# kiva12138/MIMRL

Hardware: AMD Instinct MI355X
Metric: two-stage train iters/sec (higher is better)
Workload: dtype bf16

## Files before the change

### include/mimrl.h

```cpp
#ifndef MIMRL_H_
#define MIMRL_H_

#include <stdint.h>

#ifdef __cplusplus
extern "C" {
#endif

#define MIMRL_ABI_VERSION 6
#define MIMRL_MAX_BLOCKS 4
#define MIMRL_MAX_BATCH 2048
#define MIMRL_MAX_BATCH_CONCAT 1024
#define MIMRL_MAX_CLASSES 8

enum { MIMRL_OK = 0, MIMRL_ERR_ARG = -1, MIMRL_ERR_HIP = -2, MIMRL_ERR_STATE = -3, MIMRL_ERR_NODEVICE = -4 };
enum { MIMRL_GROUP_MAIN = 0, MIMRL_GROUP_CRITIC = 1 };
enum { MIMRL_CRITIC_SEPARATE = 0, MIMRL_CRITIC_CONCAT = 1 };
enum { MIMRL_BOUND_INFONCE = 0, MIMRL_BOUND_NWJ, MIMRL_BOUND_TUBA, MIMRL_BOUND_DV, MIMRL_BOUND_JS_FGAN,
       MIMRL_BOUND_JS, MIMRL_BOUND_SMILE, MIMRL_BOUND_MINE, MIMRL_BOUND_INTERPOLATE };
enum { MIMRL_ACT_NONE = 0, MIMRL_ACT_RELU = 1, MIMRL_ACT_GELU = 2, MIMRL_ACT_TANH = 3 };
enum { MIMRL_PREC_FP32 = 0, MIMRL_PREC_BF16_GEMM_FWD = 1, MIMRL_PREC_BF16_GEMM_BWD = 2, MIMRL_PREC_BF16_GRU_FWD = 4,
       MIMRL_PREC_BF16_GRU_BWD = 8, MIMRL_PREC_BF16 = 15 };

enum { MIMRL_BASELINE_CONSTANT = 0, MIMRL_BASELINE_GAUSSAIN = 1, MIMRL_BASELINE_UNNORMALIZED = 2 };
// ... 115 lines not shown
int mimrl_op_gemm_wgrad_group(void* stream, int n, const float* const* A, const float* const* B, float* const* C, const int32_t* dims,
                              const int64_t* strides, int precision);
int64_t mimrl_op_gru_saved_floats(int B, int T);
int mimrl_op_gru_forward(void* stream, const float* gx_f, const float* gx_r, const float* whh_f, const float* whh_r,
                         const float* bhh_f, const float* bhh_r, const int32_t* lens, float* out, float* saved_f,
                         float* saved_r, int B, int T, int precision);
int mimrl_op_gru_backward(void* stream, const float* whh_f, const float* whh_r, const float* saved_f,
                          const float* saved_r, const int32_t* lens, const float* out, const float* dout, float* dg_f,
                          float* dg_r, float* hprev_f, float* hprev_r, int B, int T, int precision);
int mimrl_op_recur_btv(int B, int nmod);
int mimrl_op_lstm_forward(void* stream, const float* gx_f, const float* gx_r, const float* whh_f, const float* whh_r,
                          const float* bhh_f, const float* bhh_r, const int32_t* lens, float* out, float* saved_f,
                          float* saved_r, int B, int T, int kernel);
int mimrl_op_lstm_backward(void* stream, const float* whh_f, const float* whh_r, const float* saved_f,
                           const float* saved_r, const int32_t* lens, const float* out, const float* dout, float* dg_f,
                           float* dg_r, float* hprev_f, float* hprev_r, int B, int T, int kernel);
int mimrl_op_concat_dw(void* stream, const void* dz2, const void* a1, float* dw2, const void* dz1, const void* a0, float* dw1, int E, int64_t rows,
                       int64_t dw_stride, const float* ds, const void* a2h, float* dw3, const uint32_t* m2, const float* w3, const float* P,
                       const float* Q, int B);
int mimrl_op_gru_wgrad(void* stream, const void* const* dg, const void* const* x, const void* const* hp, float* const* dw_ih,
                       float* const* dw_hh, int64_t rows, int kp);
int mimrl_op_mi_bound(void* stream, const float* scores, float* dscores, float* mi, const float* gscale, int E, int B,
                      int bound);
int mimrl_op_mi_bound_ex(void* stream, const float* scores, float* dscores, float* mi, float* mi_loss, const float* gscale,
                         int E, int B, int bound, uint32_t lossform);
#define MIMRL_NCE_WS_FLOATS 2064
int mimrl_op_mi_infonce_rows(void* stream, const float* scores, float* dscores, float* mi, float* mi_loss, const float* gscale,
                             int E, int B, float* ws);
int mimrl_op_mi_bound_baseline(void* stream, float* scores, float* dscores, float* mi, const float* gscale, const float* lb,
                               float* dlb, int E, int B, int bound);
int mimrl_op_mi_sep_infonce(void* stream, const float* tout, float* dtout, float* mi, float* mi_loss, const float* gscale, int E,
                            int B, int tiled);
int mimrl_op_knn(void* stream, const float* Z, int dz, int N, const int32_t* anchors, int m, int k, int32_t* idx_out);
int mimrl_op_sample_anchors(void* stream, int32_t* anchors_out, int ncall, int m, int N, uint64_t seed, const int32_t* step,
                            uint32_t stream_id, int step_add);
int mimrl_knn_r1_host(const float* z, int N, const int32_t* anchors, int m, int k, int32_t* idx_out);
int mimrl_set_knn_override_mask(mimrl_handle* h, int stage, unsigned call_mask);
int mimrl_op_cmi_loss(void* stream, const float* logits, float* dlogits, float* bce, float* cmi, const float* g_bce,
                      const float* g_cmi, int E, int n, int hardtanh);
int mimrl_op_task_loss(void* stream, int kind, const float* pred, const float* y, float* dpred, float* loss, int B);
int mimrl_op_class_loss(void* stream, int kind, const float* logits, const float* y, float* dlogits, float* loss, int B, int C);
int mimrl_op_mlp_stack_forward(void* stream, int nb, int rows, int brows, int nl, const int32_t* dims, const float* const* W,
                               const float* const* b, int64_t pstride, const float* in, float* const* act, float* out);
int mimrl_op_mlp_stack_backward(void* stream, int nb, int rows, int brows, int nl, const int32_t* dims, const float* const* W,
                                int64_t pstride, const float* const* act, const float* dout, float* const* dz, float* din,
                                float* const* db);
int mimrl_probe_cube(mimrl_handle* h, const float* x, float* out, const float* dout, float* dx);
int mimrl_probe_encoders(mimrl_handle* h, float* cube_x, const float* dcube, const float* dmean);
int mimrl_probe_mi(mimrl_handle* h, int stage, float* mi, float* scores, float* dtin_out);
int mimrl_probe_cmi(mimrl_handle* h, int stage, const float* cmi_in, float* logits, float* vals, float* dcin_out);
int mimrl_probe_knn(mimrl_handle* h, int stage, int32_t* idx_out);
int mimrl_op_adam(void* stream, float* p, float* g, float* m, float* v, int64_t n, const float* lr, const int32_t* step,
                  float beta1, float beta2, float eps, float weight_decay, float clip);

#ifdef __cplusplus
}
#endif
#endif
```

### mimrl_amd/_lib.py

```python
from __future__ import annotations

import ctypes as C
import os
from typing import List, Tuple

_HERE = os.path.dirname(os.path.abspath(__file__))
DETERMINISTIC = os.environ.get("MIMRL_DETERMINISTIC", "0") not in ("", "0")
LIB_PATH = os.environ.get("MIMRL_LIB_PATH") or os.path.join(_HERE, "libmimrl_hip_det.so" if DETERMINISTIC else "libmimrl_hip.so")
MAX_BLOCKS = 4
MAX_BATCH = 2048
MAX_BATCH_CONCAT = 1024
NCE_WS_FLOATS = 2064
NSCALARS = 64
MAX_CLASSES = 8
PHASES = ["gemm_misc", "gru_fwd", "gru_bwd", "cube_fwd", "cube_bwd", "est_fwd", "est_bwd", "opt", "model_misc"]
S1_LOSS, S1_MIS, S1_LOSSES, S2_LOSS, S2_TASK, S2_MIS, S2_LOSSES = 0, 1, 12, 32, 33, 34, 42

BOUNDS = {"infonce": 0, "nwj": 1, "tuba": 2, "dv": 3, "js_fgan": 4, "js": 5, "smile": 6, "mine": 7, "interpolate": 8}
ACTS = {"none": 0, "relu": 1, "gelu": 2, "tanh": 3}
PREC = {"fp32": 0, "bf16": 15, "bf16_gemm_fwd": 1, "bf16_gemm_bwd": 2, "bf16_gemm": 3, "bf16_gru": 12, "bf16_nogemmbwd": 13}


class MimrlError(RuntimeError):
    pass
# ... 29 lines not shown
        "main_p", "main_g", "main_m", "main_v", "crit_p", "crit_g", "crit_m", "crit_v",
        "text", "audio", "video", "labels", "bank_c", "bank_f", "bank_t", "bank_a", "bank_v",
        "anchors", "lr_main", "lr_critic", "pred", "feats", "scalars", "knn_override", "counters")]


_lib = None


def load() -> C.CDLL:
    global _lib
    if _lib is not None:
        return _lib
    if not os.path.exists(LIB_PATH):
        raise MimrlError(f"{LIB_PATH} is missing: build it with `python -c 'import __graft_entry__ as g; g.build()'` "
                         f"or `make -C mimrl_amd/csrc` (hipcc --offload-arch=gfx950). There is no CPU fallback.")
    try:
        import torch
    except ImportError:
        pass
    lib = C.CDLL(LIB_PATH)
    if os.environ.get("MIMRL_LIB_PATH"):
        class _Partial:
            def __init__(self, lib):
                object.__setattr__(self, "_lib", lib)

            def __getattr__(self, name):
                try:
                    return getattr(self._lib, name)
                except AttributeError:
                    return type("_Missing", (), {})()
        real, lib = lib, _Partial(lib)
    lib.mimrl_last_error.restype = C.c_char_p
    lib.mimrl_bucket_floats.restype = C.c_int64
    lib.mimrl_workspace_bytes.restype = C.c_int64
    lib.mimrl_op_gru_saved_floats.restype = C.c_int64
    lib.mimrl_destroy.restype = None
    lib.mimrl_op_gemm.argtypes = [_FP, _FP, _FP, _FP, C.c_int, C.c_int, C.c_int, C.c_int, C.POINTER(C.c_int64), _FP, _FP,
                                  C.c_float, C.c_float, C.c_int, C.c_int]
    lib.mimrl_op_gemm_ex.argtypes = [_FP, _FP, _FP, _FP, C.c_int, C.c_int, C.c_int, C.c_int, C.POINTER(C.c_int64), _FP, _FP, C.c_int,
                                     C.POINTER(C.c_int64), C.c_int, C.c_int, _FP, _FP, _FP, C.c_int, C.c_int]
    lib.mimrl_comm_unique_id.argtypes = [_FP]
    lib.mimrl_set_comm.argtypes = [_FP, _FP, C.c_int, C.c_int]
    lib.mimrl_set_comm_critic_bf16.argtypes = [_FP, C.c_int]
    lib.mimrl_set_task_loss.argtypes = [_FP, C.c_int]
    lib.mimrl_op_task_loss.argtypes = [_FP, C.c_int, _FP, _FP, _FP, _FP, C.c_int]
    lib.mimrl_set_class_loss.argtypes = [_FP, C.c_int]
    lib.mimrl_op_class_loss.argtypes = [_FP, C.c_int, _FP, _FP, _FP, _FP, C.c_int, C.c_int]
    lib.mimrl_main_late_offset.argtypes = [_FP]
    lib.mimrl_main_late_offset.restype = C.c_int64
    lib.mimrl_op_gemm16.argtypes = [_FP, _FP, _FP, _FP, C.c_int, C.c_int, C.c_int, C.c_int, C.POINTER(C.c_int64), _FP, _FP, C.c_int,
                                    C.POINTER(C.c_int64), C.c_int, C.POINTER(C.c_int64), _FP, C.c_int]
    lib.mimrl_op_gemm_wgrad_group.argtypes = [_FP, C.c_int, C.POINTER(C.c_void_p), C.POINTER(C.c_void_p), C.POINTER(C.c_void_p),
                                              C.POINTER(C.c_int32), C.POINTER(C.c_int64), C.c_int]
    lib.mimrl_op_adam.argtypes = [_FP, _FP, _FP, _FP, _FP, C.c_int64, _FP, _FP, C.c_float, C.c_float, C.c_float,
                                  C.c_float, C.c_float]
    lib.mimrl_op_gru_forward.argtypes = [_FP] * 11 + [C.c_int, C.c_int, C.c_int]
    lib.mimrl_op_gru_backward.argtypes = [_FP] * 12 + [C.c_int, C.c_int, C.c_int]
    lib.mimrl_op_lstm_forward.argtypes = [_FP] * 11 + [C.c_int, C.c_int, C.c_int]
    lib.mimrl_op_lstm_backward.argtypes = [_FP] * 12 + [C.c_int, C.c_int, C.c_int]
    lib.mimrl_op_recur_btv.argtypes = [C.c_int, C.c_int]
    lib.mimrl_op_concat_dw.argtypes = [C.c_void_p] * 7 + [C.c_int, C.c_int64, C.c_int64] + [C.c_void_p] * 7 + [C.c_int]
    lib.mimrl_op_gru_wgrad.argtypes = [C.c_void_p] + [C.POINTER(C.c_void_p)] * 5 + [C.c_int64, C.c_int]
    lib.mimrl_op_mi_bound.argtypes = [_FP] * 5 + [C.c_int, C.c_int, C.c_int]
    lib.mimrl_op_mi_bound_ex.argtypes = [_FP] * 6 + [C.c_int, C.c_int, C.c_int, C.c_uint32]
    lib.mimrl_op_mi_infonce_rows.argtypes = [_FP] * 6 + [C.c_int, C.c_int, _FP]
    lib.mimrl_op_mi_sep_infonce.argtypes = [_FP] * 6 + [C.c_int, C.c_int, C.c_int]
    lib.mimrl_op_mi_bound_baseline.argtypes = [_FP] * 7 + [C.c_int, C.c_int, C.c_int]
    lib.mimrl_op_knn.argtypes = [_FP, _FP, C.c_int, C.c_int, _FP, C.c_int, C.c_int, _FP]
    lib.mimrl_op_cmi_loss.argtypes = [_FP] * 7 + [C.c_int, C.c_int, C.c_int]
    lib.mimrl_op_sample_anchors.argtypes = [_FP, _FP, C.c_int, C.c_int, C.c_int, C.c_uint64, _FP, C.c_uint32, C.c_int]
    lib.mimrl_create.argtypes = [C.POINTER(Cfg), _FP, C.POINTER(_FP)]
    lib.mimrl_bind.argtypes = [_FP, C.POINTER(Buffers)]
    lib.mimrl_profile_read.argtypes = [_FP, C.POINTER(C.c_float), C.POINTER(C.c_int32)]
    lib.mimrl_profile_read_gemm.argtypes = [_FP, C.POINTER(C.c_double)]
    for fn in ("mimrl_set_bank_rows", "mimrl_stage_grads", "mimrl_stage_grads_part", "mimrl_stage_apply", "mimrl_estimate", "mimrl_profile_enable", "mimrl_set_stage2_prefetch"):
        getattr(lib, fn).argtypes = [_FP, C.c_int]
    lib.mimrl_set_grad_scale.argtypes = [_FP, C.c_float]
    lib.mimrl_stage_grads_part.argtypes = [_FP, C.c_int, C.c_int]
    lib.mimrl_set_inputs.argtypes = [_FP, C.c_int, _FP, _FP, _FP, _FP]
    lib.mimrl_knn_r1_host.argtypes = [_FP, C.c_int, _FP, C.c_int, C.c_int, _FP]
    lib.mimrl_set_knn_override_mask.argtypes = [_FP, C.c_int, C.c_uint]
    for fn in ("mimrl_stage1_step", "mimrl_stage2_step", "mimrl_two_stage_step", "mimrl_destroy", "mimrl_workspace_bytes", "mimrl_params_changed",
               "mimrl_stage2_forward_tail"):
        getattr(lib, fn).argtypes = [_FP]
    lib.mimrl_forward.argtypes = [_FP, C.c_int, C.c_int]
    lib.mimrl_set_kernel_stamps.argtypes = [_FP, _FP, C.c_int]
    lib.mimrl_probe_cube.argtypes = [_FP] * 5
    lib.mimrl_probe_mi.argtypes = [_FP, C.c_int, _FP, _FP, _FP]
    lib.mimrl_probe_cmi.argtypes = [_FP, C.c_int, _FP, _FP, _FP, _FP]
    lib.mimrl_probe_knn.argtypes = [_FP, C.c_int, _FP]
    lib.mimrl_probe_encoders.argtypes = [_FP] * 4
    lib.mimrl_layout_count.argtypes = [C.POINTER(Cfg)]
    lib.mimrl_layout_entry_dim2.argtypes = [C.POINTER(Cfg), C.c_int]
    lib.mimrl_bucket_floats.argtypes = [C.POINTER(Cfg), C.c_int]
    lib.mimrl_layout_entry.argtypes = [C.POINTER(Cfg), C.c_int, C.c_char_p, C.c_int, C.POINTER(C.c_int),
                                       C.POINTER(C.c_int64), C.POINTER(C.c_int), C.POINTER(C.c_int), C.POINTER(C.c_int)]
    if os.environ.get("MIMRL_LIB_PATH"):
        lib = real
    _lib = lib
    return lib


ENCODERS = {"gru": 0, "conv": 1, "lstm": 2}
BASELINES = {"constant": 0, "gaussain": 1, "unnormalized": 2}

EXPORTS = [
    "mimrl_last_error", "mimrl_abi_version", "mimrl_deterministic", "mimrl_device_check", "mimrl_layout_count", "mimrl_layout_entry", "mimrl_layout_entry_dim2",
    "mimrl_bucket_floats", "mimrl_create", "mimrl_bind", "mimrl_set_bank_rows", "mimrl_set_inputs", "mimrl_stage1_step", "mimrl_stage2_step", "mimrl_two_stage_step",
    "mimrl_stage_grads", "mimrl_stage_grads_part", "mimrl_stage_apply", "mimrl_forward", "mimrl_estimate", "mimrl_profile_enable", "mimrl_profile_read", "mimrl_profile_read_gemm",
    "mimrl_workspace_bytes", "mimrl_params_changed", "mimrl_set_stage2_prefetch", "mimrl_stage2_forward_tail", "mimrl_set_grad_scale", "mimrl_destroy", "mimrl_op_gemm", "mimrl_op_gemm_ex", "mimrl_op_gemm16", "mimrl_op_gemm_wgrad_group",
    "mimrl_op_gru_saved_floats", "mimrl_op_gru_forward", "mimrl_op_gru_backward", "mimrl_op_gru_wgrad", "mimrl_op_concat_dw", "mimrl_op_mi_bound", "mimrl_op_mi_bound_ex", "mimrl_op_mi_bound_baseline", "mimrl_op_mi_sep_infonce", "mimrl_op_knn",
    "mimrl_op_cmi_loss", "mimrl_op_sample_anchors", "mimrl_knn_r1_host", "mimrl_set_knn_override_mask", "mimrl_op_mlp_stack_forward", "mimrl_op_mlp_stack_backward", "mimrl_op_adam",
    "mimrl_probe_cube", "mimrl_probe_mi", "mimrl_probe_cmi", "mimrl_probe_knn", "mimrl_probe_encoders", "mimrl_set_kernel_stamps", "mimrl_comm_unique_id", "mimrl_set_comm", "mimrl_main_late_offset", "mimrl_set_comm_critic_bf16",
    "mimrl_stage1_pipe_prime", "mimrl_stage1_pipe", "mimrl_set_task_loss", "mimrl_op_task_loss", "mimrl_set_class_loss", "mimrl_op_class_loss",
    "mimrl_op_mi_infonce_rows", "mimrl_op_lstm_forward", "mimrl_op_lstm_backward", "mimrl_op_recur_btv",
]

TASK_LOSSES = {"MAE": 0, "MSE": 1, "RMSE": 2, "SIMSE": 3, "CCC": 4}
BATCH_COUPLED_LOSSES = ("RMSE", "SIMSE", "CCC")
CLASS_LOSSES = {"CE": 5, "Focal": 6, "BCE": 7}


def task_loss_code(opt, world: int = 1) -> int:
    loss = getattr(opt, "loss", "MAE")
    task = getattr(opt, "task", "regression")
    ncls = int(getattr(opt, "num_class", 1))
    if loss in CLASS_LOSSES:
        if task != "classification":
            raise NotImplementedError(f"--loss {loss} is a classification loss: it needs --task classification (and --num_class)")
        if loss == "BCE" and ncls not in (1, 2):
            raise NotImplementedError(f"--loss BCE needs --num_class 1 or 2, got {ncls} (Solver.py:327-337)")
        if loss != "BCE" and not 2 <= ncls <= MAX_CLASSES:
            raise NotImplementedError(f"--loss {loss} needs 2 <= --num_class <= {MAX_CLASSES}, got {ncls}")
        if int(world) > 1 and loss == "Focal":
            raise NotImplementedError(f"--loss {loss} couples the whole batch: with {int(world)} ranks each would see only its shard, not the "
                                      f"reference's global batch; run it on one rank, or use CE / BCE")
        return CLASS_LOSSES[loss]
    if loss not in TASK_LOSSES:
        raise NotImplementedError(f"--loss {loss}: unknown task loss (choose one of {', '.join(list(TASK_LOSSES) + list(CLASS_LOSSES))})")
    if task == "classification" or ncls > 1:
        raise NotImplementedError(f"--loss {loss} is a regression loss: --task classification / --num_class {ncls} need one of "
                                  f"{', '.join(CLASS_LOSSES)}")
    if int(world) > 1 and loss in BATCH_COUPLED_LOSSES:
        raise NotImplementedError(f"--loss {loss} couples the whole batch: with {int(world)} ranks each would see only its shard, not the "
                                  f"reference's global batch; run it on one rank, or use MAE / MSE")
    return TASK_LOSSES[loss]


def check(rc: int) -> int:
    if rc < 0:
        raise MimrlError(f"libmimrl_hip error {rc}: {load().mimrl_last_error().decode()}")
    return rc


def make_cfg(opt, d_t: int, d_a: int, d_v: int, seq_len: int = None, bank_capacity: int = 0, precision: str = "fp32",
             use_graph: bool = False, seed: int = 0, device_anchors: bool = False, batch: int = None) -> Cfg:
    c = Cfg()
    c.batch = int(batch if batch is not None else opt.batch_size)
    c.time_len = int(opt.time_len)
    c.seq_len = int(seq_len if seq_len is not None else opt.time_len)
    c.d_t, c.d_a, c.d_v, c.d_common = int(d_t), int(d_a), int(d_v), int(opt.d_common)
    enc = getattr(opt, "encoders", "gru")
    if enc not in ENCODERS:
        raise MimrlError(f"--encoders {enc}: choose gru, conv or lstm (Model.py:237)")
    c.encoder = ENCODERS[enc]
    nb = len(opt.d_hiddens)
    if nb > MAX_BLOCKS or len(opt.d_outs) != nb or len(opt.res_project) != nb:
        raise MimrlError("d_hiddens / d_outs / res_project must have the same length (<= 4)")
# ... 78 lines not shown
```

### mimrl_amd/csrc/cube_bwd_fused.h

```cpp
#pragma once
#include "common.h"
#include "model_ops.h"

namespace mimrl {

struct LAxisBwdArgs {
  const float *dz, *y, *mean, *rstd, *gamma;
  const float* u;
  const float *w2, *w1, *wr;
  float *dy, *du, *dx;
  float *db2, *db1;
  int B, il, hl, ol, C, act;
};
bool laxis_bwd_supported(int il, int hl, int ol, int C);
int laxis_bwd_fused(hipStream_t s, const LAxisBwdArgs& a);

struct DAxisBwdArgs {
  const float *dz, *y, *mean, *rstd, *gamma;
  const float* u;
  const __bf16 *w2t, *w1t, *wrt;
  float *dy, *du, *dx;
  long R;
  int act;
  float *dgamma, *dbeta, *db2, *db1;
};
bool daxis_bwd_supported(int id, int hd, int od);
int daxis_bwd_fused(hipStream_t s, const DAxisBwdArgs& a);

struct WtTransposeArgs { const float* src[12]; __bf16* dst[12]; int n; };
int wt_transpose_bf16(hipStream_t s, const WtTransposeArgs& a);

int daxis_param_grads(hipStream_t s, const float* y, const float* mean, const float* rstd, const float* dz, const float* dy,
                      const float* du, float* dgamma, float* dbeta, float* db2, float* db1, long R);

#ifdef MIMRL_PHASE_PROBE
int cube_bwd_read_phases(long long* out);
#endif

}
```

### mimrl_amd/csrc/cube_bwd_fused.hip

```cpp
#include "cube_bwd_fused.h"
#include "kmix_device.h"

namespace mimrl {

namespace {

#ifdef MIMRL_PHASE_PROBE
__device__ long long g_cbwd_phase[64];
#define BPHASE(base, i) do { if (blockIdx.x == 0 && blockIdx.y == 0 && threadIdx.x == 0) g_cbwd_phase[(base) + (i)] = (long long)wall_clock64(); } while (0)
#else
#define BPHASE(base, i) do { } while (0)
#endif

constexpr int CT = 128;
constexpr int KP = 64 + 8;


template <bool LONG = false>
__global__ __launch_bounds__(256, LONG ? 2 : 1) void laxis_bwd_kernel(LAxisBwdArgs a) {
  __shared__ __attribute__((aligned(16))) __bf16 sdyu[2][CT][KP];
  auto& sdy = sdyu[0];
  auto& sdu = sdyu[1];
  __shared__ __attribute__((aligned(16))) __bf16 wts[3][64][KP];
  float (*red)[2][CT] = reinterpret_cast<float (*)[2][CT]>(&sdu[0][0]);
  __shared__ float acc_l[3][64];
  __shared__ LdsAcc acc_h[64];
  __shared__ float sgam[64];
  const int tid = threadIdx.x, lane = tid & 63, wave = tid >> 6, lr = lane & 31, lh = lane >> 5;
  const int b = blockIdx.y, c0 = blockIdx.x * CT;
  const int il = a.il, hl = a.hl, ol = a.ol, C = a.C;
  const int pb = ol > 32 ? 16 : 0;
  BPHASE(pb, 0);

  float uu[2][16];
  {
    const int ccu = c0 + wave * 32 + lr;
#pragma unroll
    for (int mt = 0; mt < 2; ++mt)
#pragma unroll
      for (int r = 0; r < 16; ++r) {
        const int h = min(mt * 32 + (r & 3) + 8 * (r >> 2) + 4 * lh, hl - 1);
        uu[mt][r] = a.u[((long)b * hl + h) * C + ccu];
      }
  }
  {
    uint4* z = reinterpret_cast<uint4*>(&wts[0][0][0]);
    for (int i = tid; i < 3 * 64 * KP * 2 / 16; i += 256) z[i] = make_uint4(0u, 0u, 0u, 0u);
    if (tid < 64) { acc_l[0][tid] = 0.f; acc_l[1][tid] = 0.f; acc_l[2][tid] = 0.f; acc_h[tid].zero(); sgam[tid] = a.gamma[tid < ol ? tid : ol - 1]; }
  }
  __syncthreads();
  BPHASE(pb, 1);
  {
    const int n2 = ol * hl, n1 = hl * il, nr = ol * il;
    float wv[3][16];
#pragma unroll
    for (int j = 0; j < 16; ++j) {
      const int idx = tid + 256 * j;
      wv[0][j] = a.w2[idx < n2 ? idx : n2 - 1];
      if constexpr (!LONG) {
        wv[1][j] = a.w1[idx < n1 ? idx : n1 - 1];
        wv[2][j] = a.wr[idx < nr ? idx : nr - 1];
      }
    }
#pragma unroll
    for (int j = 0; j < 16; ++j) {
      const int idx = tid + 256 * j;
      if (idx < n2) { const int o = idx / hl, h = idx - o * hl; wts[0][h][o] = to_bf16(wv[0][j]); }
      if constexpr (!LONG) {
        if (idx < n1) { const int h = idx / il, i = idx - h * il; wts[1][i][h] = to_bf16(wv[1][j]); }
        if (idx < nr) { const int o = idx / il, i = idx - o * il; wts[2][i][o] = to_bf16(wv[2][j]); }
      }
    }
  }

  BPHASE(pb, 2);
  const int col = tid & (CT - 1), half = tid >> 7;
  const long cidx = (long)b * C + c0 + col;
  const float mu = a.mean[cidx], rs = a.rstd[cidx];
  const float* __restrict__ dzb = a.dz + (long)b * ol * C + c0 + col;
  const float* __restrict__ yb = a.y + (long)b * ol * C + c0 + col;
  float* __restrict__ dyb = a.dy + (long)b * ol * C + c0 + col;
  float gq[32], xq[32];
#pragma unroll
  for (int j = 0; j < 32; ++j) {
    const int l = min(half + 2 * j, ol - 1);
    gq[j] = dzb[(long)l * C]; xq[j] = yb[(long)l * C];
  }
  float s1 = 0.f, s2 = 0.f;
#pragma unroll
  for (int j = 0; j < 32; ++j) {
    const int l = half + 2 * j;
    xq[j] = (xq[j] - mu) * rs;
    gq[j] = l < ol ? gq[j] * sgam[min(l, 63)] : 0.f;
    s1 += gq[j]; s2 += gq[j] * xq[j];
  }
  BPHASE(pb, 3);
  red[0][half][col] = s1;
  red[1][half][col] = s2;
  __syncthreads();
  s1 = (red[0][0][col] + red[0][1][col]) / ol;
  s2 = (red[1][0][col] + red[1][1][col]) / ol;
#pragma unroll
  for (int j = 0; j < 32; ++j) {
    const int l = half + 2 * j;
    if (l < ol) {
      const float v = rs * (gq[j] - s1 - xq[j] * s2);
      dyb[(long)l * C] = v;
      sdy[col][l] = to_bf16(v);
    }
  }
  for (int l = ol + ((half ^ ol) & 1); l < 64; l += 2) sdy[col][l] = to_bf16(0.f);
  __syncthreads();

  if (a.db2 && tid >= 192 && tid - 192 < ol) {
    float t = 0.f;
    for (int c = 0; c < CT; ++c) t += (float)sdy[(c + tid) & (CT - 1)][tid - 192];
    acc_l[2][tid - 192] = t;
  }
  BPHASE(pb, 4);
  const int nt = wave;
  const int cc = c0 + nt * 32 + lr;
  {
    f32x16 acc0, acc1;
#pragma unroll
    for (int r = 0; r < 16; ++r) { acc0[r] = 0.f; acc1[r] = 0.f; }
#pragma unroll
    for (int ks = 0; ks < 4; ++ks) {
      const bf16x8 bf = *reinterpret_cast<const bf16x8*>(&sdy[nt * 32 + lr][ks * 16 + 8 * lh]);
      const bf16x8 a0 = *reinterpret_cast<const bf16x8*>(&wts[0][lr][ks * 16 + 8 * lh]);
      acc0 = __builtin_amdgcn_mfma_f32_32x32x16_bf16(a0, bf, acc0, 0, 0, 0);
      const bf16x8 a1 = *reinterpret_cast<const bf16x8*>(&wts[0][32 + lr][ks * 16 + 8 * lh]);
      acc1 = __builtin_amdgcn_mfma_f32_32x32x16_bf16(a1, bf, acc1, 0, 0, 0);
    }
    act_dispatch(a.act, [&](auto AT) __attribute__((always_inline)) {
#pragma unroll
    for (int mt = 0; mt < 2; ++mt)
#pragma unroll
      for (int r = 0; r < 16; ++r) {
        const int h = mt * 32 + (r & 3) + 8 * (r >> 2) + 4 * lh;
        float v = 0.f;
        if (h < hl) {
          const long ui = ((long)b * hl + h) * C + cc;
          v = (mt == 0 ? acc0[r] : acc1[r]) * act_grad_c<decltype(AT)::value>(a.act, uu[mt][r]);
          a.du[ui] = v;
        }
        sdu[nt * 32 + lr][h] = to_bf16(v);
        if (a.db1) {
          const float t = half_sum_hi(v);
          if (lr == 16 && h < hl) acc_h[h].add(t);
        }
      }
    });
  }
  __syncthreads();
  BPHASE(pb, 5);
  if constexpr (LONG) {
    float w1v[16], wrv[16];
    auto wreq = [&](int i0) __attribute__((always_inline)) {
      const int i = min(i0 + (tid & 63), il - 1);
#pragma unroll
      for (int j = 0; j < 16; ++j) {
        const int r = 16 * (tid >> 6) + j;
        w1v[j] = a.w1[(long)min(r, hl - 1) * il + i];
        wrv[j] = a.wr[(long)min(r, ol - 1) * il + i];
      }
    };
    wreq(0);
    for (int i0 = 0; i0 < il; i0 += 64) {
      __syncthreads();
      {
        const int ii = tid & 63, r0 = 16 * (tid >> 6);
        const bool iok = i0 + ii < il;
        bf16x8 p1[2], p2[2];
#pragma unroll
        for (int j = 0; j < 16; ++j) {
          p1[j >> 3][j & 7] = to_bf16(iok && r0 + j < hl ? w1v[j] : 0.f);
          p2[j >> 3][j & 7] = to_bf16(iok && r0 + j < ol ? wrv[j] : 0.f);
        }
        *reinterpret_cast<bf16x8*>(&wts[1][ii][r0]) = p1[0]; *reinterpret_cast<bf16x8*>(&wts[1][ii][r0 + 8]) = p1[1];
        *reinterpret_cast<bf16x8*>(&wts[2][ii][r0]) = p2[0]; *reinterpret_cast<bf16x8*>(&wts[2][ii][r0 + 8]) = p2[1];
      }
      __syncthreads();
      wreq(i0 + 64 < il ? i0 + 64 : i0);
      f32x16 acc0, acc1;
#pragma unroll
      for (int r = 0; r < 16; ++r) { acc0[r] = 0.f; acc1[r] = 0.f; }
#pragma unroll
      for (int ks = 0; ks < 8; ++ks) {
        const bool first = ks < 4;
        const int kk = (first ? ks : ks - 4) * 16 + 8 * lh;
        const bf16x8 bf = *reinterpret_cast<const bf16x8*>(first ? &sdu[nt * 32 + lr][kk] : &sdy[nt * 32 + lr][kk]);
        const bf16x8 a0 = *reinterpret_cast<const bf16x8*>(&wts[first ? 1 : 2][lr][kk]);
        acc0 = __builtin_amdgcn_mfma_f32_32x32x16_bf16(a0, bf, acc0, 0, 0, 0);
        const bf16x8 a1 = *reinterpret_cast<const bf16x8*>(&wts[first ? 1 : 2][32 + lr][kk]);
        acc1 = __builtin_amdgcn_mfma_f32_32x32x16_bf16(a1, bf, acc1, 0, 0, 0);
      }
      {
#pragma unroll
        for (int mt = 0; mt < 2; ++mt)
#pragma unroll
          for (int r = 0; r < 16; ++r) {
            const int i = i0 + mt * 32 + (r & 3) + 8 * (r >> 2) + 4 * lh;
            if (i < il) a.dx[((long)b * il + i) * C + cc] = mt == 0 ? acc0[r] : acc1[r];
          }
      }
    }
  } else {
    f32x16 acc0, acc1;
#pragma unroll
    for (int r = 0; r < 16; ++r) { acc0[r] = 0.f; acc1[r] = 0.f; }
#pragma unroll
    for (int ks = 0; ks < 8; ++ks) {
      const bool first = ks < 4;
      const int kk = (first ? ks : ks - 4) * 16 + 8 * lh;
      const bf16x8 bf = *reinterpret_cast<const bf16x8*>(first ? &sdu[nt * 32 + lr][kk] : &sdy[nt * 32 + lr][kk]);
      const bf16x8 a0 = *reinterpret_cast<const bf16x8*>(&wts[first ? 1 : 2][lr][kk]);
      acc0 = __builtin_amdgcn_mfma_f32_32x32x16_bf16(a0, bf, acc0, 0, 0, 0);
      const bf16x8 a1 = *reinterpret_cast<const bf16x8*>(&wts[first ? 1 : 2][32 + lr][kk]);
      acc1 = __builtin_amdgcn_mfma_f32_32x32x16_bf16(a1, bf, acc1, 0, 0, 0);
    }
    {
#pragma unroll
      for (int mt = 0; mt < 2; ++mt)
#pragma unroll
        for (int r = 0; r < 16; ++r) {
          const int i = mt * 32 + (r & 3) + 8 * (r >> 2) + 4 * lh;
          if (i < il) a.dx[((long)b * il + i) * C + cc] = mt == 0 ? acc0[r] : acc1[r];
        }
    }
  }
  __syncthreads();
  BPHASE(pb, 6);
  if (a.db2 && tid < ol) acc_add(&a.db2[tid], acc_l[2][tid]);
  if (a.db1 && tid >= 64 && tid - 64 < hl) acc_add(&a.db1[tid - 64], acc_h[tid - 64].get());
  BPHASE(pb, 7);
}

}

#ifdef MIMRL_PHASE_PROBE
int cube_bwd_read_phases(long long* out) { return hipMemcpyFromSymbol(out, HIP_SYMBOL(g_cbwd_phase), sizeof(long long) * 64) == hipSuccess ? 0 : 1; }
#endif

bool laxis_bwd_supported(int il, int hl, int ol, int C) {
  return il >= 1 && hl >= 1 && ol >= 1 && hl <= 64 && ol <= 64 && C % CT == 0;
}

int laxis_bwd_fused(hipStream_t s, const LAxisBwdArgs& a) {
  if (!laxis_bwd_supported(a.il, a.hl, a.ol, a.C)) return set_error(MIMRL_ERR_ARG, "laxis_bwd_fused: unsupported shape");
  if (!a.wr) return set_error(MIMRL_ERR_ARG, "laxis_bwd_fused: needs the residual projection");
  if (a.il > 64) hipLaunchKernelGGL(laxis_bwd_kernel<true>, dim3(a.C / CT, a.B), dim3(256), 0, s, a);
  else hipLaunchKernelGGL(laxis_bwd_kernel<false>, dim3(a.C / CT, a.B), dim3(256), 0, s, a);
  LAUNCH_CHECK();
  return MIMRL_OK;
}

namespace {

constexpr int DR = 32;
constexpr int DP = 128 + 8;

__global__ __launch_bounds__(256) void daxis_bwd_kernel(DAxisBwdArgs a) {
  __shared__ __attribute__((aligned(16))) __bf16 sdy[DR][DP];
  __shared__ __attribute__((aligned(16))) __bf16 sdu[DR][DP];
  __shared__ LdsAcc spg[3][128];
  const int tid = threadIdx.x, lane = tid & 63, wave = tid >> 6, lr = lane & 31, lh = lane >> 5;
  const long r0 = (long)blockIdx.x * DR;
  const bool pg = a.dgamma != nullptr;
  const int pb = gridDim.x <= 200 ? 32 : 48;
  BPHASE(pb, 0);
  if (pg) for (int i = tid; i < 3 * 128; i += 256) (&spg[0][0])[i].zero();
  const int row1 = tid >> 3, part1 = tid & 7;
  const long r1 = r0 + row1;
  const bool ok1 = r1 < a.R;
  const long rc1 = ok1 ? r1 : a.R - 1;
  const float mu1 = a.mean[rc1], rs1 = a.rstd[rc1];
  float4 gz4[4], yv4[4];
#pragma unroll
  for (int q = 0; q < 4; ++q) {
    gz4[q] = *reinterpret_cast<const float4*>(a.dz + rc1 * 128 + part1 * 16 + q * 4);
    yv4[q] = *reinterpret_cast<const float4*>(a.y + rc1 * 128 + part1 * 16 + q * 4);
  }
  const int n = wave * 32 + lr;
  bf16x8 bw2[8], bw1[8], bwr[8];
#pragma unroll
  for (int ks = 0; ks < 8; ++ks) {
    bw2[ks] = *reinterpret_cast<const bf16x8*>(a.w2t + n * 128 + ks * 16 + 8 * lh);
    bw1[ks] = *reinterpret_cast<const bf16x8*>(a.w1t + n * 128 + ks * 16 + 8 * lh);
    bwr[ks] = *reinterpret_cast<const bf16x8*>(a.wrt + n * 128 + ks * 16 + 8 * lh);
  }
  float uu[16];
#pragma unroll
  for (int r = 0; r < 16; ++r) {
    const long row = min(r0 + (r & 3) + 8 * (r >> 2) + 4 * lh, a.R - 1);
    uu[r] = a.u[row * 128 + n];
  }
  BPHASE(pb, 1);
  {
    const int row = row1, part = part1;
    const long r = r1;
    const bool ok = ok1;
    float g[16], xh[16], dyk[16];
    float s1 = 0.f, s2 = 0.f;
    const float mu = mu1, rs = rs1;
#pragma unroll
    for (int q = 0; q < 4; ++q) {
      const float4 gz = gz4[q];
      const float4 yv = yv4[q];
      const float gg[4] = {gz.x, gz.y, gz.z, gz.w}, yy[4] = {yv.x, yv.y, yv.z, yv.w};
#pragma unroll
      for (int j = 0; j < 4; ++j) {
        g[q * 4 + j] = gg[j];
        xh[q * 4 + j] = (yy[j] - mu) * rs;
        const float dxh = gg[j] * a.gamma[part * 16 + q * 4 + j];
        s1 += dxh; s2 += dxh * xh[q * 4 + j];
      }
    }
    s1 = group_sum<8>(s1); s2 = group_sum<8>(s2);
    s1 *= (1.f / 128.f); s2 *= (1.f / 128.f);
#pragma unroll
    for (int q = 0; q < 4; ++q) {
      float v[4];
#pragma unroll
      for (int j = 0; j < 4; ++j) {
        const int c = part * 16 + q * 4 + j;
        v[j] = rs * (g[q * 4 + j] * a.gamma[c] - s1 - xh[q * 4 + j] * s2);
      }
      if (ok) *reinterpret_cast<float4*>(a.dy + r * 128 + part * 16 + q * 4) = make_float4(v[0], v[1], v[2], v[3]);
      bf16x4 p; p[0] = to_bf16(v[0]); p[1] = to_bf16(v[1]); p[2] = to_bf16(v[2]); p[3] = to_bf16(v[3]);
      *reinterpret_cast<bf16x4*>(&sdy[row][part * 16 + q * 4]) = p;
      if (pg) {
#pragma unroll
        for (int j = 0; j < 4; ++j) { const float gz = ok ? g[q * 4 + j] : 0.f; xh[q * 4 + j] *= gz; g[q * 4 + j] = gz; v[j] = ok ? v[j] : 0.f; }
        dyk[q * 4 + 0] = v[0]; dyk[q * 4 + 1] = v[1]; dyk[q * 4 + 2] = v[2]; dyk[q * 4 + 3] = v[3];
      }
    }
    if (pg) {
      __syncthreads();
#pragma unroll
      for (int j = 0; j < 16; ++j) {
        float sa = xh[j], sb = g[j], sc = dyk[j];
#pragma unroll
        for (int o = 8; o < 64; o <<= 1) { sa += __shfl_xor(sa, o, 64); sb += __shfl_xor(sb, o, 64); sc += __shfl_xor(sc, o, 64); }
        if (lane < 8) { spg[0][part * 16 + j].add(sa); spg[1][part * 16 + j].add(sb); spg[2][part * 16 + j].add(sc); }
      }
    }
  }
  __syncthreads();
  BPHASE(pb, 2);
  {
    f32x16 acc;
#pragma unroll
    for (int r = 0; r < 16; ++r) acc[r] = 0.f;
#pragma unroll
    for (int ks = 0; ks < 8; ++ks) {
      const bf16x8 af = *reinterpret_cast<const bf16x8*>(&sdy[lr][ks * 16 + 8 * lh]);
      acc = __builtin_amdgcn_mfma_f32_32x32x16_bf16(af, bw2[ks], acc, 0, 0, 0);
    }
    float csum = 0.f;
    act_dispatch(a.act, [&](auto AT) __attribute__((always_inline)) {
#pragma unroll
    for (int r = 0; r < 16; ++r) {
      const int m = (r & 3) + 8 * (r >> 2) + 4 * lh;
      const long row = r0 + m;
      float v = 0.f;
      if (row < a.R) {
        v = acc[r] * act_grad_c<decltype(AT)::value>(a.act, uu[r]);
        a.du[row * 128 + n] = v;
      }
      sdu[m][n] = to_bf16(v);
      csum += v;
    }
    });
    if (pg) {
      csum += __shfl_xor(csum, 32, 64);
      if (lh == 0) acc_add(&a.db1[n], csum);
    }
  }
  __syncthreads();
  BPHASE(pb, 3);
  if (pg && tid < 128) {
    acc_add(&a.dgamma[tid], spg[0][tid].get());
    acc_add(&a.dbeta[tid], spg[1][tid].get());
    acc_add(&a.db2[tid], spg[2][tid].get());
  }
  {
    f32x16 acc;
#pragma unroll
    for (int r = 0; r < 16; ++r) acc[r] = 0.f;
#pragma unroll
    for (int ks = 0; ks < 8; ++ks) {
      const bf16x8 a1 = *reinterpret_cast<const bf16x8*>(&sdu[lr][ks * 16 + 8 * lh]);
      acc = __builtin_amdgcn_mfma_f32_32x32x16_bf16(a1, bw1[ks], acc, 0, 0, 0);
      const bf16x8 a2 = *reinterpret_cast<const bf16x8*>(&sdy[lr][ks * 16 + 8 * lh]);
      acc = __builtin_amdgcn_mfma_f32_32x32x16_bf16(a2, bwr[ks], acc, 0, 0, 0);
    }
#pragma unroll
    for (int r = 0; r < 16; ++r) {
      const long row = r0 + (r & 3) + 8 * (r >> 2) + 4 * lh;
      if (row < a.R) a.dx[row * 128 + n] = acc[r];
    }
  }
  BPHASE(pb, 4);
}

__global__ void wt_transpose_kernel(WtTransposeArgs a) {
  __shared__ float t[32][33];
  const float* __restrict__ src = a.src[blockIdx.z];
  __bf16* __restrict__ dst = a.dst[blockIdx.z];
  const int k0 = blockIdx.y * 32, n0 = blockIdx.x * 32, tx = threadIdx.x & 31, ty = threadIdx.x >> 5;
  for (int j = ty; j < 32; j += 8) t[j][tx] = src[(k0 + j) * 128 + n0 + tx];
  __syncthreads();
  for (int j = ty; j < 32; j += 8) dst[(n0 + j) * 128 + k0 + tx] = to_bf16(t[tx][j]);
}

__global__ __launch_bounds__(256) void daxis_param_grads_kernel(const float* __restrict__ y, const float* __restrict__ mean,
                                                                const float* __restrict__ rstd, const float* __restrict__ dz,
                                                                const float* __restrict__ dy, const float* __restrict__ du,
                                                                float* __restrict__ dgamma, float* __restrict__ dbeta,
                                                                float* __restrict__ db2, float* __restrict__ db1, long R) {
  __shared__ float4 red[4][8][32];
  const int cq = threadIdx.x & 31, rl = threadIdx.x >> 5;
  const long r0 = (long)blockIdx.x * 64;
  float4 a0 = make_float4(0.f, 0.f, 0.f, 0.f), a1 = a0, a2 = a0, a3 = a0;
#pragma unroll
  for (int i = 0; i < 8; ++i) {
    const long r = r0 + rl + 8 * i;
    const long rc = r < R ? r : R - 1;
    const float m = r < R ? 1.f : 0.f;
    const float mu = mean[rc], rs = rstd[rc] * m;
    const float4 g = *reinterpret_cast<const float4*>(dz + rc * 128 + cq * 4);
    const float4 yv = *reinterpret_cast<const float4*>(y + rc * 128 + cq * 4);
    const float4 v = *reinterpret_cast<const float4*>(dy + rc * 128 + cq * 4);
    const float4 u = *reinterpret_cast<const float4*>(du + rc * 128 + cq * 4);
    a0.x += g.x * (yv.x - mu) * rs; a0.y += g.y * (yv.y - mu) * rs; a0.z += g.z * (yv.z - mu) * rs; a0.w += g.w * (yv.w - mu) * rs;
    a1.x += g.x * m; a1.y += g.y * m; a1.z += g.z * m; a1.w += g.w * m;
    a2.x += v.x * m; a2.y += v.y * m; a2.z += v.z * m; a2.w += v.w * m;
    a3.x += u.x * m; a3.y += u.y * m; a3.z += u.z * m; a3.w += u.w * m;
  }
  red[0][rl][cq] = a0; red[1][rl][cq] = a1; red[2][rl][cq] = a2; red[3][rl][cq] = a3;
  __syncthreads();
#pragma unroll
  for (int h = 0; h < 2; ++h) {
    const int idx = threadIdx.x + 256 * h, q = idx >> 7, c = idx & 127;
    const float* base = reinterpret_cast<const float*>(&red[q][0][0]);
    float sum = 0.f;
#pragma unroll
    for (int j = 0; j < 8; ++j) sum += base[j * 128 + c];
    float* dst = q == 0 ? dgamma : (q == 1 ? dbeta : (q == 2 ? db2 : db1));
    if (dst) acc_add(&dst[c], sum);
  }
}

}

int daxis_param_grads(hipStream_t s, const float* y, const float* mean, const float* rstd, const float* dz, const float* dy,
                      const float* du, float* dgamma, float* dbeta, float* db2, float* db1, long R) {
  if (R <= 0) return MIMRL_OK;
  hipLaunchKernelGGL(daxis_param_grads_kernel, dim3((unsigned)((R + 63) / 64)), dim3(256), 0, s, y, mean, rstd, dz, dy, du, dgamma, dbeta,
                     db2, db1, R);
  LAUNCH_CHECK();
  return MIMRL_OK;
}

bool daxis_bwd_supported(int id, int hd, int od) { return id == 128 && hd == 128 && od == 128; }

int daxis_bwd_fused(hipStream_t s, const DAxisBwdArgs& a) {
  if (!a.w2t || !a.w1t || !a.wrt) return set_error(MIMRL_ERR_ARG, "daxis_bwd_fused: needs the transposed weight images");
  if ((a.dgamma || a.dbeta || a.db2 || a.db1) && !(a.dgamma && a.dbeta && a.db2 && a.db1))
    return set_error(MIMRL_ERR_ARG, "daxis_bwd_fused: the four parameter-gradient outputs come together");
  hipLaunchKernelGGL(daxis_bwd_kernel, dim3((unsigned)((a.R + DR - 1) / DR)), dim3(256), 0, s, a);
  LAUNCH_CHECK();
  return MIMRL_OK;
}

int wt_transpose_bf16(hipStream_t s, const WtTransposeArgs& a) {
  if (a.n < 1 || a.n > 12) return set_error(MIMRL_ERR_ARG, "wt_transpose_bf16: 1..12 matrices");
  hipLaunchKernelGGL(wt_transpose_kernel, dim3(4, 4, a.n), dim3(256), 0, s, a);
  LAUNCH_CHECK();
  return MIMRL_OK;
}

}
```

### mimrl_amd/csrc/cube_fused.h

```cpp
#pragma once
#include "common.h"
#include "model_ops.h"

namespace mimrl {

struct CubePre {
  const float* tx_raw;
  const float* h2[2];
  const float *gamma[2], *beta[2];
  float p[3];
  float* feats;
  float* cube; float *mean[2], *rstd[2];
  int T;
  RngKey key;
};
struct CubeHead { const float *w, *bias; float *ff, *pred; float scale; int C; };

struct CubeFusedArgs {
  const float* x;
  const float *l_w1, *l_b1, *l_w2, *l_b2, *l_wr, *l_g, *l_be;
  KMixW kw;
  const float *d_w1, *d_b1, *d_w2, *d_b2, *d_wr, *d_g, *d_be;
  float *l_u, *l_h, *l_y, *l_z, *l_mean, *l_rstd;
  float* k_z;
  float *d_u, *d_h, *d_y, *d_mean, *d_rstd;
  float* d_z;
  int B, il, hl, ol, K, act, save;
  int dbg_phase;
  int pre_on, head_on;
  CubePre pre; CubeHead head;
};

bool cube_fused_supported(int il, int hl, int ol, int ik, int hk, int ok, int id, int hd, int od, bool ln_first,
                          bool res_project, bool bias, const float* dropout_mlp);
int cube_block_fwd_fused(hipStream_t s, const CubeFusedArgs& a);

#ifdef MIMRL_PHASE_PROBE
int cube_fwd_read_phases(long long* out);
#endif

}
```

### mimrl_amd/csrc/cube_fused.hip

```cpp
#include "cube_fused.h"

#include "cube_bookends.h"

#include <type_traits>

namespace mimrl {

namespace {

constexpr int D = 128;
constexpr int ILD = 72;
constexpr int IMG = 64 * ILD;
constexpr int CTL = 68, CTD = 132;

typedef _Float16 bf;

#ifdef MIMRL_PHASE_PROBE
__device__ long long g_cube_phase[128];
#define CPHASE(i) do { if (blockIdx.x == 0 && threadIdx.x == 0) g_cube_phase[(SAVE ? 64 : 0) + (NMT - 1) * 16 + (i)] = (long long)wall_clock64(); } while (0)
#else
#define CPHASE(i) do { } while (0)
#endif

__device__ __forceinline__ void mma64(f32x16& acc, const bf* A, const bf* B, int wm, int wn, int lane) {
// ... 32 lines not shown
  *reinterpret_cast<f16x8*>(img + n * ILD + kc + 8) = hi;
}
__device__ __forceinline__ void stage_weight(bf* img, const float* __restrict__ W, int ld, int n0, int k0, int N, int K, int tid) {
  stage_weight_commit(img, stage_weight_request(W, ld, n0, k0, N, K, tid), n0, k0, N, K, tid);
}
struct WImg { float4 q0, q1, q2, q3; };
__device__ __forceinline__ WImg load_weight128(const float* __restrict__ W, int n0, int k0, int tid) {
  const int n = tid >> 2, kc = (tid & 3) * 16;
  const float4* src = reinterpret_cast<const float4*>(W + (long)(n0 + n) * D + k0 + kc);
  return WImg{src[0], src[1], src[2], src[3]};
}
__device__ __forceinline__ void commit_weight128(bf* img, const WImg& w, int tid) {
  const int n = tid >> 2, kc = (tid & 3) * 16;
  f16x8 lo, hi;
  lo[0] = to_f16(w.q0.x); lo[1] = to_f16(w.q0.y); lo[2] = to_f16(w.q0.z); lo[3] = to_f16(w.q0.w);
  lo[4] = to_f16(w.q1.x); lo[5] = to_f16(w.q1.y); lo[6] = to_f16(w.q1.z); lo[7] = to_f16(w.q1.w);
  hi[0] = to_f16(w.q2.x); hi[1] = to_f16(w.q2.y); hi[2] = to_f16(w.q2.z); hi[3] = to_f16(w.q2.w);
  hi[4] = to_f16(w.q3.x); hi[5] = to_f16(w.q3.y); hi[6] = to_f16(w.q3.z); hi[7] = to_f16(w.q3.w);
  *reinterpret_cast<f16x8*>(img + n * ILD + kc) = lo;
  *reinterpret_cast<f16x8*>(img + n * ILD + kc + 8) = hi;
}

struct Carve {
  int xm, aw, bx, bh, ctl, red, ksw, prm;
  int bw, ctd, dprm, az, ah;
  int total;
};
__host__ __device__ inline Carve carve(int K, int nmt, int G) {
  Carve c;
  const int C = K * D, XP = C + 8;
  const int xm_bytes = 64 * XP * 2;
  c.xm = 0;
  c.aw = xm_bytes;
  c.bx = c.aw + 3 * IMG * 2;
  c.bh = c.bx + G * IMG * 2;
  c.ctl = c.bh + G * IMG * 2;
  c.red = c.ctl + G * 64 * CTL * 4;
  c.ksw = c.red + G * 2 * 4 * 64 * 4;
  c.prm = c.ksw + 256 * 4;
  const int l_end = c.prm + 4 * 64 * 4;
  c.bw = 0;
  c.dprm = c.bw + 2 * G * IMG * 2;
  int after = c.dprm + 2 * D * 4;
  if (after < xm_bytes) after = xm_bytes;
  c.az = (after + 15) & ~15;
  c.ah = c.az + nmt * 2 * IMG * 2;
  const int ah_bytes = nmt * 2 * IMG * 2, ctd_bytes = 64 * CTD * 4;
  c.ctd = c.ah;
  const int d_end = c.ah + (ah_bytes > ctd_bytes ? ah_bytes : ctd_bytes);
  c.total = l_end > d_end ? l_end : d_end;
  return c;
}

template <bool SAVE, int NMT, int G, bool PRE, bool HEAD>
__device__ __forceinline__ void cube_fwd_fused_body(const CubeFusedArgs& a) {
  static_assert(!(PRE || HEAD) || G == 2, "PRE / HEAD: 8 waves (12 time-phase streams on 8 waves; head_fwd_kernel's 512-thread shape)");
  static_assert(!HEAD || NMT == 1, "HEAD: every row of the block output in the one LDS tile");
  extern __shared__ __attribute__((aligned(16))) char smem[];
  constexpr int NT = 256 * G;
  const int tid = threadIdx.x, grp = tid >> 8, t = tid & 255, lane = t & 63, wave = t >> 6, wm = wave >> 1, wn = wave & 1;
  const int b = blockIdx.x;
  const int K = a.K, C = K * D, XP = C + 8, il = a.il, hl = a.hl, ol = a.ol;
  const Carve cv = carve(K, NMT, G);
  bf* Xm = reinterpret_cast<bf*>(smem + cv.xm);
  bf* Aw = reinterpret_cast<bf*>(smem + cv.aw);
  bf* Bx = reinterpret_cast<bf*>(smem + cv.bx) + grp * IMG;
  bf* Bh = reinterpret_cast<bf*>(smem + cv.bh) + grp * IMG;
  float* CtL = reinterpret_cast<float*>(smem + cv.ctl) + grp * 64 * CTL;
  float* red = reinterpret_cast<float*>(smem + cv.red) + grp * 2 * 4 * 64;
  float* ksw = reinterpret_cast<float*>(smem + cv.ksw);
  float* prm = reinterpret_cast<float*>(smem + cv.prm);

  CPHASE(0);
  {
    const bool g0 = G == 1 || grp == 0;
    const WReq w0 = stage_weight_request(g0 ? a.l_w1 : a.l_w2, g0 ? il : hl, 0, 0, g0 ? hl : ol, g0 ? il : hl, t);
    const WReq w1 = stage_weight_request(a.l_wr, il, 0, 0, ol, il, t);
    WReq w2;
    if (G == 1) w2 = stage_weight_request(a.l_w2, hl, 0, 0, ol, hl, t);
    float pr[4] = {0.f, 0.f, 0.f, 0.f};
    if (tid < 64) {
      pr[0] = (tid < hl && a.l_b1) ? a.l_b1[tid] : 0.f;
      pr[1] = (tid < ol && a.l_b2) ? a.l_b2[tid] : 0.f;
      pr[2] = tid < ol ? a.l_g[tid] : 0.f;
      pr[3] = tid < ol ? a.l_be[tid] : 0.f;
    }
    CPHASE(13);
    if constexpr (PRE) {
      const CubePre& pp = a.pre;
      const int T = pp.T, w8 = tid >> 6, ph = w8 & 3, ln64 = tid & 63;
      const bool audio = w8 >= 4;
      const int m = audio ? 0 : 1, slot = 1 + m;
      const uint32_t rstep = (uint32_t)(*pp.key.step + pp.key.add);
      const float* __restrict__ txb = pp.tx_raw + (long)b * T * D;
      const float* __restrict__ h2 = (audio ? pp.h2[0] : pp.h2[1]) + (long)b * T * 2 * D;
      const float* __restrict__ gam = audio ? pp.gamma[0] : pp.gamma[1];
      const float* __restrict__ bet = audio ? pp.beta[0] : pp.beta[1];
      float* __restrict__ lmean = audio ? pp.mean[0] : pp.mean[1];
      float* __restrict__ lrstd = audio ? pp.rstd[0] : pp.rstd[1];
      const float ga0 = gam[ln64], ga1 = gam[ln64 + 64], be0 = bet[ln64], be1 = bet[ln64 + 64];
      const float pdrop = audio ? pp.p[1] : pp.p[2];
      const bool wr = pp.cube != nullptr;
      float xt[16][2], v[8][2];
#pragma unroll
      for (int q = 0; q < 16; ++q) {
        const int tt = ph + 4 * q < T ? ph + 4 * q : T - 1;
        xt[q][0] = txb[(long)tt * D + ln64]; xt[q][1] = txb[(long)tt * D + ln64 + 64];
      }
// ... 82 lines not shown
          *reinterpret_cast<f16x4*>(Xm + l * XP + c4) = p;
        }
      }
    }
    }
    CPHASE(14);
    if (tid < 64) { prm[0 * 64 + tid] = pr[0]; prm[1 * 64 + tid] = pr[1]; prm[2 * 64 + tid] = pr[2]; prm[3 * 64 + tid] = pr[3]; }
    stage_weight_commit(g0 ? Aw + 0 * IMG : Aw + 1 * IMG, w0, 0, 0, g0 ? hl : ol, g0 ? il : hl, t);
    if (g0) stage_weight_commit(Aw + 2 * IMG, w1, 0, 0, ol, il, t);
    if (G == 1) stage_weight_commit(Aw + 1 * IMG, w2, 0, 0, ol, hl, t);
  }
  __syncthreads();
  CPHASE(1);
  if constexpr (PRE) {
    if (tid < 3 * D) {
      const float* fp = reinterpret_cast<const float*>(smem + cv.ctl) + (tid >> 7) * 4 * D + (tid & 127);
      a.pre.feats[((long)(tid >> 7) * a.B + b) * D + (tid & 127)] = pre_mean(fp[0], fp[D], fp[2 * D], fp[3 * D], a.pre.T);
    }
  }
  if (a.dbg_phase == 1) return;

  for (int nb = 0; nb < C; nb += 64 * G) {
    const int n0 = nb + 64 * grp;
    const bool on = n0 < C;
    if (on) {
      const int n = t & 63, kg = (t >> 6) * 16;
      f16x8 lo, hi;
#pragma unroll
      for (int j = 0; j < 8; ++j) { lo[j] = Xm[(kg + j) * XP + n0 + n]; hi[j] = Xm[(kg + 8 + j) * XP + n0 + n]; }
      *reinterpret_cast<f16x8*>(Bx + n * ILD + kg) = lo;
      *reinterpret_cast<f16x8*>(Bx + n * ILD + kg + 8) = hi;
    }
    __syncthreads();
    if (nb == 0) CPHASE(8);
    f32x16 acc;
#pragma unroll
    for (int i = 0; i < 16; ++i) acc[i] = 0.f;
    if (on) {
      mma64(acc, Aw + 0 * IMG, Bx, wm, wn, lane);
      const int n = wn * 32 + (lane & 31);
      act_dispatch(a.act, [&](auto AT) __attribute__((always_inline)) {
#pragma unroll
        for (int g = 0; g < 4; ++g) {
          f16x4 p;
#pragma unroll
          for (int q = 0; q < 4; ++q) {
            const int m = acc_row(4 * g + q, wm, lane);
            float h = 0.f;
            if (m < hl) {
              const float u = acc[4 * g + q] + prm[m];
              h = act_apply_c<decltype(AT)::value>(a.act, u);
              if (SAVE) {
                a.l_u[((long)b * hl + m) * C + n0 + n] = u;
                a.l_h[((long)b * hl + m) * C + n0 + n] = h;
              }
            }
            p[q] = to_f16(h);
          }
          *reinterpret_cast<f16x4*>(Bh + n * ILD + wm * 32 + 8 * g + 4 * (lane >> 5)) = p;
        }
      });
    }
    __syncthreads();
    if (nb == 0) CPHASE(9);
    if (on) {
#pragma unroll
      for (int i = 0; i < 16; ++i) acc[i] = 0.f;
      mma64(acc, Aw + 1 * IMG, Bh, wm, wn, lane);
      mma64(acc, Aw + 2 * IMG, Bx, wm, wn, lane);
      const int n = wn * 32 + (lane & 31);
#pragma unroll
      for (int r = 0; r < 16; ++r) {
        const int m = acc_row(r, wm, lane);
        CtL[m * CTL + n] = acc[r] + prm[64 + m];
      }
    }
    __syncthreads();
    if (nb == 0) CPHASE(10);
    {
      const int n = t & 63, q = t >> 6;
      float yv[16];
      float s = 0.f;
      if (on) {
#pragma unroll
        for (int j = 0; j < 16; ++j) {
          const int m = q + 4 * j;
          yv[j] = m < ol ? CtL[m * CTL + n] : 0.f;
          s += yv[j];
        }
        red[q * 64 + n] = s;
      }
      __syncthreads();
      float mu = 0.f;
      if (on) {
        mu = (red[n] + red[64 + n] + red[128 + n] + red[192 + n]) / ol;
        float v = 0.f;
#pragma unroll
        for (int j = 0; j < 16; ++j) { const float c = (q + 4 * j < ol) ? yv[j] - mu : 0.f; v += c * c; }
        red[256 + q * 64 + n] = v;
      }
      __syncthreads();
      if (on) {
        const float rs = rsqrtf((red[256 + n] + red[320 + n] + red[384 + n] + red[448 + n]) / ol + LN_EPS);
#pragma unroll
        for (int j = 0; j < 16; ++j) {
          const int m = q + 4 * j;
          if (m < ol) {
            const float z = (yv[j] - mu) * rs * prm[128 + m] + prm[192 + m];
            const bf zb = to_f16(z);
            Xm[m * XP + n0 + n] = zb;
            if (SAVE) {
              a.l_y[((long)b * ol + m) * C + n0 + n] = yv[j];
              a.l_z[((long)b * ol + m) * C + n0 + n] = (float)zb;
            }
          }
        }
        if (SAVE && q == 0) { a.l_mean[(long)b * C + n0 + n] = mu; a.l_rstd[(long)b * C + n0 + n] = rs; }
      }
    }
    __syncthreads();
    if (nb == 0) CPHASE(11);
  }

  CPHASE(2);
  if (a.dbg_phase == 2) return;
  WImg wnext;
  if constexpr (!SAVE) wnext = load_weight128(a.d_w1, (G == 1 ? 0 : grp) * 64, 0, t);
  kmix_stage_weights(a.kw, ksw);
  {
    auto phase_k = [&](auto NKc) __attribute__((always_inline)) {
      constexpr int NK = decltype(NKc)::value;
      act_dispatch(a.kw.act, [&](auto AT) __attribute__((always_inline)) {
      KMixRegs<NK> kq;
      kq.load(ksw);
#pragma unroll 2
      for (int i = tid; i < ol * D; i += NT) {
        const int l = i >> 7, d = i & 127;
        KMixVals<NK> v;
#pragma unroll
        for (int k = 0; k < NK; ++k) { v.x[k] = (float)Xm[l * XP + k * D + d]; v.sc[k] = 1.f; }
        kmix_forward_regs<NK, decltype(AT)::value>(a.kw, kq, v);
        float out[NK];
        ln_small<NK>(v.y, NK, kq.g, kq.be, out, v.xh, v.mu, v.rs);
#pragma unroll
        for (int o = 0; o < NK; ++o) {
          const bf ob = to_f16(out[o]);
          Xm[l * XP + o * D + d] = ob;
          if (SAVE) a.k_z[(((long)b * ol + l) * NK + o) * D + d] = (float)ob;
        }
      }
      });
    };
    if (K == 3) phase_k(std::integral_constant<int, 3>{});
    else if (K == 1) phase_k(std::integral_constant<int, 1>{});
    else if (K == 2) phase_k(std::integral_constant<int, 2>{});
    else phase_k(std::integral_constant<int, 4>{});
  }
  __syncthreads();

  CPHASE(3);
  if (a.dbg_phase == 3) return;
  const int R = ol * K;
  float* CtD = reinterpret_cast<float*>(smem + cv.ctd);
  float* dgam = reinterpret_cast<float*>(smem + cv.dprm);
  float* dbet = dgam + D;
  bf* Az = reinterpret_cast<bf*>(smem + cv.az);
  bf* Ah = reinterpret_cast<bf*>(smem + cv.ah);
  for (int c = tid; c < NMT * 64 * 16; c += NT) {
    const int r = c >> 4, ch = c & 15;
    f16x8 v;
#pragma unroll
    for (int j = 0; j < 8; ++j) v[j] = to_f16(0.f);
    if (r < R) {
      const int l = r / K, kk = r - l * K;
      v = *reinterpret_cast<const f16x8*>(Xm + l * XP + kk * D + ch * 8);
    }
    *reinterpret_cast<f16x8*>(Az + ((r >> 6) * 2 + (ch >> 3)) * IMG + (r & 63) * ILD + (ch & 7) * 8) = v;
  }
  __syncthreads();
  CPHASE(4);
  if (tid < D) { dgam[tid] = a.d_g[tid]; dbet[tid] = a.d_be[tid]; }
  constexpr int NTW = 2 / G, NI1 = 2 * NTW;
  const int nt0 = G == 1 ? 0 : grp;
  float b1v[NTW], b2v[NTW];
#pragma unroll
  for (int q = 0; q < NTW; ++q) {
    const int col = (nt0 + q) * 64 + wn * 32 + (lane & 31);
    b1v[q] = a.d_b1 ? a.d_b1[col] : 0.f;
    b2v[q] = a.d_b2 ? a.d_b2[col] : 0.f;
  }

  f32x16 acc[NMT][NTW];
#pragma unroll
  for (int mt = 0; mt < NMT; ++mt)
#pragma unroll
    for (int q = 0; q < NTW; ++q)
#pragma unroll
      for (int i = 0; i < 16; ++i) acc[mt][q][i] = 0.f;
  auto wload = [&](int i) -> WImg {
    const float* W = i < NI1 ? a.d_w1 : (i < 2 * NI1 ? a.d_w2 : a.d_wr);
    const int j = i % NI1;
    return load_weight128(W, (nt0 + (j >> 1)) * 64, (j & 1) * 64, t);
  };
  bf* Bw2[2] = {reinterpret_cast<bf*>(smem + cv.bw) + (2 * grp) * IMG, reinterpret_cast<bf*>(smem + cv.bw) + (2 * grp + 1) * IMG};
  if constexpr (SAVE) wnext = wload(0);
#pragma unroll
  for (int i = 0; i < NI1; ++i) {
    const int q = i >> 1, kh = i & 1;
    commit_weight128(Bw2[i & 1], wnext, t);
    wnext = wload(i + 1);
    __syncthreads();
#pragma unroll
    for (int mt = 0; mt < NMT; ++mt) mma64(acc[mt][q], Az + (mt * 2 + kh) * IMG, Bw2[i & 1], wm, wn, lane);
  }
  CPHASE(12);
  act_dispatch(a.act, [&](auto AT) __attribute__((always_inline)) {
#pragma unroll
  for (int mt = 0; mt < NMT; ++mt)
#pragma unroll
    for (int q = 0; q < NTW; ++q) {
      const int nt = nt0 + q, n = wn * 32 + (lane & 31), col = nt * 64 + n;
      const float b1 = b1v[q];
#pragma unroll
      for (int r = 0; r < 16; ++r) {
        const int m = acc_row(r, wm, lane), row = mt * 64 + m;
        float h = 0.f;
        if (row < R) {
          const float u = acc[mt][q][r] + b1;
          h = act_apply_c<decltype(AT)::value>(a.act, u);
          if (SAVE) {
            a.d_u[((long)b * R + row) * D + col] = u;
            a.d_h[((long)b * R + row) * D + col] = h;
          }
        }
        Ah[(mt * 2 + nt) * IMG + m * ILD + n] = to_f16(h);
        acc[mt][q][r] = 0.f;
      }
    }
  });
  __syncthreads();
  CPHASE(5);
  if (a.dbg_phase == 4) return;
#pragma unroll
  for (int i = NI1; i < 3 * NI1; ++i) {
    const int which = i >= 2 * NI1, q = (i % NI1) >> 1, kh = i & 1;
    commit_weight128(Bw2[i & 1], wnext, t);
    if (i + 1 < 3 * NI1) wnext = wload(i + 1);
    __syncthreads();
    const bf* Asrc = which == 0 ? Ah : Az;
#pragma unroll
    for (int mt = 0; mt < NMT; ++mt) mma64(acc[mt][q], Asrc + (mt * 2 + kh) * IMG, Bw2[i & 1], wm, wn, lane);
  }
  __syncthreads();
  CPHASE(6);
  if (a.dbg_phase == 5) return;
#pragma unroll
  for (int mt = 0; mt < NMT; ++mt) {
#pragma unroll
    for (int q = 0; q < NTW; ++q) {
      const int n = wn * 32 + (lane & 31), col = (nt0 + q) * 64 + n;
      const float b2 = b2v[q];
#pragma unroll
      for (int r = 0; r < 16; ++r) CtD[acc_row(r, wm, lane) * CTD + col] = acc[mt][q][r] + b2;
    }
    __syncthreads();
    {
      constexpr int TPR = 4 * G, CW = 32 / G;
      const int m = tid / TPR, part = tid % TPR, row = mt * 64 + m;
      float yv[CW];
      float s0 = 0.f;
#pragma unroll
      for (int j = 0; j < CW / 4; ++j) {
        const float4 q = *reinterpret_cast<const float4*>(&CtD[m * CTD + part * CW + 4 * j]);
        yv[4 * j] = q.x; yv[4 * j + 1] = q.y; yv[4 * j + 2] = q.z; yv[4 * j + 3] = q.w;
        s0 += (q.x + q.y) + (q.z + q.w);
      }
      s0 = group_sum<TPR>(s0);
      const float mu = s0 * (1.f / D);
      float v0 = 0.f;
#pragma unroll
      for (int j = 0; j < CW; ++j) { const float c = yv[j] - mu; v0 += c * c; }
      v0 = group_sum<TPR>(v0);
      const float rs = rsqrtf(v0 * (1.f / D) + LN_EPS);
      if (row < R) {
        const long o = ((long)b * R + row) * D + part * CW;
#pragma unroll
        for (int j = 0; j < CW / 4; ++j) {
          const int c = part * CW + 4 * j;
          float4 z;
          z.x = (yv[4 * j] - mu) * rs * dgam[c] + dbet[c];
          z.y = (yv[4 * j + 1] - mu) * rs * dgam[c + 1] + dbet[c + 1];
          z.z = (yv[4 * j + 2] - mu) * rs * dgam[c + 2] + dbet[c + 2];
          z.w = (yv[4 * j + 3] - mu) * rs * dgam[c + 3] + dbet[c + 3];
          *reinterpret_cast<float4*>(a.d_z + o + 4 * j) = z;
          if constexpr (HEAD) *reinterpret_cast<float4*>(&CtD[m * CTD + c]) = z;
          if (SAVE) *reinterpret_cast<float4*>(a.d_y + o + 4 * j) = make_float4(yv[4 * j], yv[4 * j + 1], yv[4 * j + 2], yv[4 * j + 3]);
        }
        if (SAVE && part == 0) { a.d_mean[(long)b * R + row] = mu; a.d_rstd[(long)b * R + row] = rs; }
      }
    }
    __syncthreads();
  }
  if constexpr (HEAD) {
    float (*hph)[128] = reinterpret_cast<float (*)[128]>(smem + cv.bw);
    float* hred = reinterpret_cast<float*>(smem + cv.bw) + 4 * 128;
    hph[tid >> 7][tid & 127] = head_phase_sum(CtD + (tid & 127), CTD, tid >> 7, R);
    __syncthreads();
    head_finish(hph, a.head.w, a.head.bias, a.head.ff + (long)b * D, a.head.pred + (long)b * a.head.C, a.head.scale, hred, a.head.C);
  }
  CPHASE(7);
}

template <bool SAVE, int NMT, int G>
__global__ __launch_bounds__(256 * G) void cube_fwd_fused_kernel(CubeFusedArgs a) { cube_fwd_fused_body<SAVE, NMT, G, false, false>(a); }
template <bool SAVE, int NMT, bool PRE, bool HEAD>
__global__ __launch_bounds__(512) void cube_fwd_bookends_kernel(CubeFusedArgs a) { cube_fwd_fused_body<SAVE, NMT, 2, PRE, HEAD>(a); }

}

#ifdef MIMRL_PHASE_PROBE
int cube_fwd_read_phases(long long* out) { return hipMemcpyFromSymbol(out, HIP_SYMBOL(g_cube_phase), sizeof(long long) * 128) == hipSuccess ? 0 : 1; }
#endif

bool cube_fused_supported(int il, int hl, int ol, int ik, int hk, int ok, int id, int hd, int od, bool ln_first,
                          bool res_project, bool bias, const float* dropout_mlp) {
  (void)bias;
  if (ln_first || !res_project) return false;
  if (dropout_mlp[0] > 0.f || dropout_mlp[1] > 0.f || dropout_mlp[2] > 0.f) return false;
  if (id != D || hd != D || od != D) return false;
  if (il > 64 || hl > 64 || ol > 64 || il < 1 || hl < 1 || ol < 1) return false;
  if (ik != hk || ik != ok || ik < 1 || ik > 4) return false;
  if (ol * ok > 192) return false;
  return true;
}

int cube_block_fwd_fused(hipStream_t s, const CubeFusedArgs& a) {
  const int R = a.ol * a.K;
  const int nmt = (R + 63) / 64;
  if (nmt < 1 || nmt > 3) return set_error(MIMRL_ERR_ARG, "cube_fused: unsupported row count %d", R);
  constexpr int groups = 2;
  const int G = groups == 1 ? 1 : 2;
  const Carve cv = carve(a.K, nmt, G);
  if (cv.total > 160 * 1024) return set_error(MIMRL_ERR_ARG, "cube_fused: LDS budget exceeded (%d B)", cv.total);
  if ((a.pre_on || a.head_on) && G != 2) return set_error(MIMRL_ERR_ARG, "cube_fused: the PRE / HEAD modes need two wave groups");
  if (a.pre_on && (a.K != 3 || a.pre.T < 1 || a.pre.T > a.il)) return set_error(MIMRL_ERR_ARG, "cube_fused: PRE mode needs K = 3 and 1 <= T <= il (T %d, il %d, K %d)", a.pre.T, a.il, a.K);
  if (a.head_on && nmt != 1) return set_error(MIMRL_ERR_ARG, "cube_fused: HEAD mode needs ol * K <= 64 (got %d)", R);
#define LAUNCH_KERN(KERN, GG)                                                                                      \
  do {                                                                                                             \
    auto kern = KERN;                                                                                              \
    HIPX(hipFuncSetAttribute(reinterpret_cast<const void*>(kern), hipFuncAttributeMaxDynamicSharedMemorySize, cv.total)); \
    hipLaunchKernelGGL(kern, dim3(a.B), dim3(256 * GG), cv.total, s, a);                                           \
  } while (0)
#define LAUNCH_PLAIN(SAVE, GG)                                                                                     \
  do {                                                                                                             \
    if (nmt == 1) LAUNCH_KERN((cube_fwd_fused_kernel<SAVE, 1, GG>), GG);                                           \
    else if (nmt == 2) LAUNCH_KERN((cube_fwd_fused_kernel<SAVE, 2, GG>), GG);                                      \
    else LAUNCH_KERN((cube_fwd_fused_kernel<SAVE, 3, GG>), GG);                                                    \
  } while (0)
#define LAUNCH_PRE(SAVE)                                                                                           \
  do {                                                                                                             \
    if (nmt == 1) LAUNCH_KERN((cube_fwd_bookends_kernel<SAVE, 1, true, false>), 2);                                \
    else if (nmt == 2) LAUNCH_KERN((cube_fwd_bookends_kernel<SAVE, 2, true, false>), 2);                           \
    else LAUNCH_KERN((cube_fwd_bookends_kernel<SAVE, 3, true, false>), 2);                                         \
  } while (0)
#define LAUNCH_MODE(SAVE)                                                                                          \
  do {                                                                                                             \
    if (G == 1) LAUNCH_PLAIN(SAVE, 1);                                                                             \
    else if (a.head_on && a.pre_on) LAUNCH_KERN((cube_fwd_bookends_kernel<SAVE, 1, true, true>), 2);               \
    else if (a.head_on) LAUNCH_KERN((cube_fwd_bookends_kernel<SAVE, 1, false, true>), 2);                          \
    else if (a.pre_on) LAUNCH_PRE(SAVE);                                                                           \
    else LAUNCH_PLAIN(SAVE, 2);                                                                                    \
  } while (0)
  if (a.save) LAUNCH_MODE(true); else LAUNCH_MODE(false);
#undef LAUNCH_MODE
#undef LAUNCH_PRE
#undef LAUNCH_PLAIN
#undef LAUNCH_KERN
  LAUNCH_CHECK();
  return MIMRL_OK;
}

}
```

### mimrl_amd/csrc/engine.h

```cpp
#pragma once
#include <cstdio>
#include <cstdlib>
#include <cstring>
#include <algorithm>
#include <vector>
#include <dlfcn.h>

#include "cube_fused.h"
#include "mlp_fused.h"
#include "concat_fused.h"
#include "cube_bwd_fused.h"
#include "cube_long.h"
#include "estimator_ops.h"
#include "gemm.h"
#include "gru.h"
#include "gru_wgrad.h"
#include "concat_dw.h"
#include "lstm.h"
#include "layout.h"
#include "comm.h"
#include "model_ops.h"
#include "scoped.h"

namespace mimrl {
// ... 342 lines not shown
  void retire(hipGraphExec_t& ex) { if (ex) { retired.push_back(ex); ex = nullptr; } }
  void drop_graphs(int set = -1) {
    for (int q = 0; q < 2; ++q)
      if (set < 0 || q == set)
        for (CachedGraph& c : gsets[q].all) retire(c.exec);
  }
  template <typename Body>
  int replay_or_capture(CachedGraph& slot, Body&& body, bool postprocess = false);
  float* P(long off) const { return bufs.main_p + off; }
  float* Gm(long off) const { return bufs.main_g + off; }
  float* CP(long off) const { return bufs.crit_p + off; }
  float* CG(long off) const { return bufs.crit_g + off; }
  long conv_w[2] = {0, 0}, conv_b[2] = {0, 0};
  int encoders_forward(bool save, int knn_stage);
  int conv_forward(int knn_stage);
  int conv_backward();
  int lstm_encoders_forward(bool save, int knn_stage);
  int lstm_encoders_backward();
  int rng_add = 0;
  RngKey key() const { return RngKey{(uint32_t)cfg.seed, (uint32_t)(cfg.seed >> 32), d_ints, rng_add}; }
  const float* coef1() const { return d_consts; }
  const float* coef2() const { return d_consts + 11; }
  const float* gs_mi(int stage) const { return d_consts + 19 + (stage - 1) * 5; }
  const float* g_bce(int stage) const { return d_consts + 29 + (stage - 1) * 6; }
  const float* g_cmi(int stage) const { return d_consts + 41 + (stage - 1) * 6; }
  int nprod() const { return (cfg.batch / cfg.k_neighbor) * cfg.k_neighbor; }
  int m_anchor() const { return cfg.batch / cfg.k_neighbor; }

  int resolve();
  int alloc_workspace();
  template <typename T>
  int take(T** p, size_t count) {
    const size_t bytes = (count * sizeof(T) + 255) / 256 * 256;
    if (ws) {
      if (ws_used + bytes > ws_bytes) return set_error(MIMRL_ERR_STATE, "workspace overflow");
      *p = reinterpret_cast<T*>(ws + ws_used);
    }
    ws_used += bytes;
    return MIMRL_OK;
  }
  int carve();

  int G_(const GemmDesc& d) { return G_on(stream, d); }
  struct Deferred { int kind; int side; GemmDesc g; const float* src; long n0, n1, n2, n3; float* dst;
                    const float *p1 = nullptr, *p2 = nullptr, *p3 = nullptr; float* dst2 = nullptr; KMixW kw = KMixW();
                    const float *p4 = nullptr, *p5 = nullptr; float *dst3 = nullptr, *dst4 = nullptr; };
  std::vector<Deferred> deferred;
  int flush_deferred(int only_side = 0);
  int wg_helper = -1;
  int dbg_delay(hipStream_t st, int tag);
  int model_forward(bool train, bool save, int knn_stage = 0, int part = 0);
  int cube_forward(bool train, bool save, const CubePre* pre = nullptr, const CubeHead* head = nullptr);
  bool cube_block_fused(int i, bool train) const;
  int cube_backward(int cur_in, int* cur_out);
  int wt_images(hipStream_t st, bool bwd_bf16, bool launch, bool* d_fused);
  int model_backward();
  int encoders_backward(float* dcube);
  int gru_layer_backward(int l);
  int knn_launch(int stage, hipStream_t st);
  bool pipe_primed = false; int fwd_parity = 0, pipe_set = 0;
  int pipe_forward_body(bool other_inputs);
  int run_stage1_pipe_prime();
  int run_stage1_pipe(bool next_valid);
  int mi_forward(int stage, bool want_grad);
  int cmi_forward(int stage, bool want_grad);
  int mi_backward(int stage);
  int cmi_backward(int stage);
  int route_feature_grads();
  GatherSum head_gather;
  bool head_gather_on = false;
  hipEvent_t ev_dmean = nullptr;
  int estimators_all(int stage, bool want_grad, bool backward);
  int mlp_stack_forward(int nb, int rows, int brows, long p0, long pstride, int nl, const long (*l_off)[2], const int* dims,
                        const float* in, float* const* act, float* out);
  int mlp_stack_backward(int nb, int rows, int brows, long p0, long pstride, int nl, const long (*l_off)[2],
                         const int* dims, const float* in, float* const* act, float* dout, float* const* dtmp, float* din,
                         bool wgrad);
  int enqueue_grads(int stage, bool skip_zero = false);
  int enqueue_apply(int stage);
  int run(int stage, int kind);
  int run_step();
  bool keep_events = false;
  bool fuse_boundary = false;
  bool imgT_valid = false;
  bool skip_imgT_refresh = false;
  bool wtT_prebuilt = false;
  bool wtT_built = false;
};
```

### mimrl_amd/csrc/engine_abi.hip

```cpp
#include "engine.h"

extern "C" {

const char* mimrl_last_error(void) { return mimrl::last_error_slot().c_str(); }
#ifdef MIMRL_PHASE_PROBE
int mimrl_dbg_cube_phases(long long* out) { return mimrl::cube_fwd_read_phases(out); }
int mimrl_dbg_cube_bwd_phases(long long* out) { return mimrl::cube_bwd_read_phases(out); }
int mimrl_dbg_kmix_phases(long long* out) { return mimrl::kmix_bwd_read_phases(out); }
int mimrl_dbg_nce_phases(long long* out) { return mimrl::nce_read_phases(out); }
int mimrl_dbg_model_ops_phases(long long* out) { return mimrl::model_ops_read_phases(out); }
int mimrl_dbg_gru_bwd_phases(long long* out) { return mimrl::gru_bwd_read_phases(out); }
int mimrl_dbg_concat_bwd_phases(long long* out) { return mimrl::concat_bwd_read_phases(out); }
#endif
int mimrl_abi_version(void) { return MIMRL_ABI_VERSION; }

int mimrl_device_check(void) {
  int n = 0;
  if (hipGetDeviceCount(&n) != hipSuccess || n <= 0) return set_error(MIMRL_ERR_NODEVICE, "no HIP device visible");
  int dev = 0;
  if (hipGetDevice(&dev) != hipSuccess) return set_error(MIMRL_ERR_NODEVICE, "hipGetDevice failed");
  hipDeviceProp_t p;
  if (hipGetDeviceProperties(&p, dev) != hipSuccess) return set_error(MIMRL_ERR_NODEVICE, "hipGetDeviceProperties failed");
  if (std::strncmp(p.gcnArchName, "gfx950", 6) != 0)
    return set_error(MIMRL_ERR_NODEVICE, "device %d is %s; this library is built for gfx950 (MI355X) only", dev, p.gcnArchName);
// ... 513 lines not shown
                     const float* A2, const float* B2, int K2, const int64_t st2[6], int a_gap_at, int a_gap_rows, const float* bias_n,
                     const float* gradact_u, float* colsum, int act, int precision) {
  if (!st || (A2 && !st2)) return set_error(MIMRL_ERR_ARG, "null strides");
  GemmDesc d;
  d.A = A; d.B = B; d.C = C; d.M = M; d.N = N; d.K = K; d.batch = batch;
  d.sa_m = st[0]; d.sa_k = st[1]; d.sa_b = st[2]; d.sb_k = st[3]; d.sb_n = st[4]; d.sb_b = st[5];
  d.sc_m = st[6]; d.sc_n = st[7]; d.sc_b = st[8];
  if (A2) {
    d.A2 = A2; d.B2 = B2; d.K2 = K2;
    d.sa2_m = st2[0]; d.sa2_k = st2[1]; d.sa2_b = st2[2]; d.sb2_k = st2[3]; d.sb2_n = st2[4]; d.sb2_b = st2[5];
  }
  d.a_gap_at = a_gap_at; d.a_gap_rows = a_gap_rows;
  d.bias_n = bias_n; d.gradact_u = gradact_u; d.colsum = colsum; d.act = act & 0xff; d.atomic = (act >> 8) & 1;
  return gemm(reinterpret_cast<hipStream_t>(stream), d, (precision & 1) != 0);
}

int mimrl_op_gemm16(void* stream, const void* A, const void* B, void* C, int M, int N, int K, int batch, const int64_t st[9],
                    const void* A2, const void* B2, int K2, const int64_t st2[6], int batch_in, const int64_t st_bo[5],
                    const float* bias_n, int flags) {
  if (!st || (A2 && !st2) || (batch_in > 0 && !st_bo)) return set_error(MIMRL_ERR_ARG, "null strides");
  if (batch_in < 0 || (batch_in > 0 && batch % batch_in != 0)) return set_error(MIMRL_ERR_ARG, "batch_in must divide batch");
  GemmDesc d;
  d.A = static_cast<const float*>(A); d.B = static_cast<const float*>(B); d.C = static_cast<float*>(C);
  d.M = M; d.N = N; d.K = K; d.batch = batch;
  d.sa_m = st[0]; d.sa_k = st[1]; d.sa_b = st[2]; d.sb_k = st[3]; d.sb_n = st[4]; d.sb_b = st[5];
  d.sc_m = st[6]; d.sc_n = st[7]; d.sc_b = st[8];
  if (A2) {
    d.A2 = static_cast<const float*>(A2); d.B2 = static_cast<const float*>(B2); d.K2 = K2;
    d.sa2_m = st2[0]; d.sa2_k = st2[1]; d.sa2_b = st2[2]; d.sb2_k = st2[3]; d.sb2_n = st2[4]; d.sb2_b = st2[5];
  }
  if (batch_in > 0) { d.batch_in = batch_in; d.sa_bo = st_bo[0]; d.sb_bo = st_bo[1]; d.sc_bo = st_bo[2]; d.bias_n_bo = st_bo[3]; }
  if (st_bo) d.bias_n_b = st_bo[4];
  d.bias_n = bias_n;
  d.a_bf16 = flags & 1; d.b_bf16 = (flags >> 1) & 1; d.f16 = (flags >> 2) & 1; d.c_f16 = (flags >> 3) & 1; d.atomic = (flags >> 4) & 1;
  if (flags >> 8) { d.a_gap_at = (flags >> 8) & 0xfff; d.a_gap_rows = (flags >> 20) & 0xfff; }
  return gemm(reinterpret_cast<hipStream_t>(stream), d, true);
}

int mimrl_op_gemm_wgrad_group(void* stream, int n, const float* const* A, const float* const* B, float* const* C, const int32_t* dims,
                              const int64_t* st, int precision) {
  if (n <= 0 || n > 12 || !A || !B || !C || !dims || !st) return set_error(MIMRL_ERR_ARG, "gemm_wgrad_group: 1..12 problems");
  GemmDesc d[12];
  for (int i = 0; i < n; ++i) {
    d[i].A = A[i]; d[i].B = B[i]; d[i].C = C[i];
    d[i].M = dims[4 * i]; d[i].N = dims[4 * i + 1]; d[i].K = dims[4 * i + 2]; d[i].batch = dims[4 * i + 3];
    const int64_t* q = st + 9 * i;
    d[i].sa_m = q[0]; d[i].sa_k = q[1]; d[i].sa_b = q[2]; d[i].sb_k = q[3]; d[i].sb_n = q[4]; d[i].sb_b = q[5];
    d[i].sc_m = q[6]; d[i].sc_n = q[7]; d[i].sc_b = q[8];
    d[i].atomic = 1;
  }
  return gemm_group_splitk(reinterpret_cast<hipStream_t>(stream), d, n, (precision & 1) != 0);
}

int64_t mimrl_op_gru_saved_floats(int B, int T) { return gru_saved_floats(B, T); }

int mimrl_op_gru_forward(void* stream, const float* gx_f, const float* gx_r, const float* whh_f, const float* whh_r,
                         const float* bhh_f, const float* bhh_r, const int32_t* lens, float* out, float* saved_f,
                         float* saved_r, int B, int T, int precision) {
  GruFwdArgs a;
  std::memset(&a, 0, sizeof a);
  a.B = B; a.T = T; a.out_ld = 2 * H; a.nmod = 1; a.btv = gru_pick_btv(B, 1);
  a.lens[0] = lens; a.lens[1] = lens;
  a.seq[0][0] = GruSeq{gx_f, whh_f, bhh_f, out, saved_f};
  a.seq[0][1] = GruSeq{gx_r, whh_r, bhh_r, out, saved_r};
  return gru_forward(reinterpret_cast<hipStream_t>(stream), a, (precision & 1) != 0);
}

int mimrl_op_gru_backward(void* stream, const float* whh_f, const float* whh_r, const float* saved_f,
                          const float* saved_r, const int32_t* lens, const float* out, const float* dout, float* dg_f,
                          float* dg_r, float* hprev_f, float* hprev_r, int B, int T, int precision) {
  GruBwdArgs a;
  std::memset(&a, 0, sizeof a);
  a.B = B; a.T = T; a.out_ld = 2 * H; a.dout_ld = 2 * H; a.dout_off = H; a.nmod = 1; a.btv = gru_pick_btv(B, 1);
  a.lens[0] = lens; a.lens[1] = lens;
  a.seq[0][0] = GruSeqBwd{whh_f, saved_f, out, dout, dg_f, hprev_f, nullptr, nullptr};
  a.seq[0][1] = GruSeqBwd{whh_r, saved_r, out, dout, dg_r, hprev_r, nullptr, nullptr};
  return gru_backward(reinterpret_cast<hipStream_t>(stream), a, (precision & 1) != 0);
}

int mimrl_op_recur_btv(int B, int nmod) {
  if (B < 1 || nmod < 1 || nmod > 2) return set_error(MIMRL_ERR_ARG, "mimrl_op_recur_btv: B >= 1, nmod 1 or 2");
  const int g = gru_pick_btv(B, nmod), l = lstm_btv(B, nmod);
  if (g != l) return set_error(MIMRL_ERR_STATE, "mimrl_op_recur_btv: the GRU (%d) and LSTM (%d) picks differ: give this entry point an encoder argument", g, l);
  return g;
}

int mimrl_op_lstm_forward(void* stream, const float* gx_f, const float* gx_r, const float* whh_f, const float* whh_r,
                          const float* bhh_f, const float* bhh_r, const int32_t* lens, float* out, float* saved_f,
                          float* saved_r, int B, int T, int kernel) {
  if (!gx_f || !gx_r || !whh_f || !whh_r || !bhh_f || !bhh_r || !lens || !out) return set_error(MIMRL_ERR_ARG, "mimrl_op_lstm_forward: null argument");
  if ((saved_f != nullptr) != (saved_r != nullptr)) return set_error(MIMRL_ERR_ARG, "mimrl_op_lstm_forward: both saved records or neither");
  LstmFwdArgs a;
  std::memset(&a, 0, sizeof a);
  a.B = B; a.T = T; a.out_ld = 2 * H; a.nmod = 1;
  a.lens[0] = lens; a.lens[1] = lens;
  a.seq[0][0] = LstmSeq{gx_f, whh_f, bhh_f, out, saved_f};
  a.seq[0][1] = LstmSeq{gx_r, whh_r, bhh_r, out, saved_r};
  return lstm_forward_kernels(reinterpret_cast<hipStream_t>(stream), a, kernel);
}

int mimrl_op_lstm_backward(void* stream, const float* whh_f, const float* whh_r, const float* saved_f,
                           const float* saved_r, const int32_t* lens, const float* out, const float* dout, float* dg_f,
                           float* dg_r, float* hprev_f, float* hprev_r, int B, int T, int kernel) {
  if (!whh_f || !whh_r || !saved_f || !saved_r || !lens || !out || !dout || !dg_f || !dg_r || !hprev_f || !hprev_r)
    return set_error(MIMRL_ERR_ARG, "mimrl_op_lstm_backward: null argument");
  LstmBwdArgs a;
// ... 152 lines not shown
```

### mimrl_amd/csrc/engine_backward.hip

```cpp
#include "engine.h"

int mimrl_handle::cube_backward(int cur_in, int* cur_out) {
  const int B = cfg.batch;
  int dims[MIMRL_MAX_BLOCKS + 1][3];
  dims[0][0] = cfg.time_len; dims[0][1] = 3; dims[0][2] = cfg.d_common;
  for (int i = 0; i < cfg.n_blocks; ++i)
    for (int ax = 0; ax < 3; ++ax) dims[i + 1][ax] = cfg.d_outs[i][ax];
  const int per_block = 7 + (cfg.dropout_mlp[0] > 0.f) + (cfg.dropout_mlp[2] > 0.f);
  const bool defer = multi_stream && !cfg.ln_first && per_block * cfg.n_blocks + 1 <= NGBUF;
  const int npool = defer ? NGBUF : 4;
  int used[NGBUF] = {0};
  used[cur_in] = 1;
  int cur = cur_in;
  auto grab = [&]() { for (int q = 0; q < npool; ++q) if (!used[q]) { used[q] = 1; return q; } return -1; };
  auto release = [&](int q) { if (!defer) used[q] = 0; };
  auto W_gemm = [&](int sd, const GemmDesc& g) -> int {
    if (defer) { deferred.push_back(Deferred{0, sd, g, nullptr, 0, 0, 0, 0, nullptr}); return MIMRL_OK; }
    return G_on(S(sd), g);
  };
  auto W_colsum = [&](int sd, const float* src, long rows, int cols, int ld, float* dst) -> int {
    if (defer) { deferred.push_back(Deferred{1, sd, GemmDesc(), src, rows, cols, ld, 0, dst}); return MIMRL_OK; }
    return colsum(S(sd), src, rows, cols, ld, dst);
  };
  auto W_rowsum = [&](int sd, const float* src, int nb, int rows, int cols, float* dst) -> int {
    if (defer) { deferred.push_back(Deferred{2, sd, GemmDesc(), src, nb, rows, cols, 0, dst}); return MIMRL_OK; }
    return rowsum_batched(S(sd), src, nb, rows, cols, dst);
  };
  auto W_lnpar = [&](int sd, const float* y, const float* mean, const float* rstd, const float* dz, float* dgam, float* dbet,
                     int nb, int n, int cols) -> int {
    if (defer) {
      Deferred d{3, sd, GemmDesc(), y, nb, n, cols, 0, dgam};
      d.p1 = mean; d.p2 = rstd; d.p3 = dz; d.dst2 = dbet;
      deferred.push_back(d);
      return MIMRL_OK;
    }
    return colln_param_grads(S(sd), y, mean, rstd, dz, dgam, dbet, nb, n, cols);
  };
  auto W_dpg = [&](int sd, const float* y, const float* mean, const float* rstd, const float* dz, const float* dy, const float* du,
                   float* dgam, float* dbet, float* db2, float* db1, long rows) -> int {
    if (defer) {
      Deferred d{6, sd, GemmDesc(), y, rows, 0, 0, 0, dgam};
      d.p1 = mean; d.p2 = rstd; d.p3 = dz; d.p4 = dy; d.p5 = du; d.dst2 = dbet; d.dst3 = db2; d.dst4 = db1;
      deferred.push_back(d);
      return MIMRL_OK;
    }
    return daxis_param_grads(S(sd), y, mean, rstd, dz, dy, du, dgam, dbet, db2, db1, rows);
  };
  auto W_fork = [&](int lo, int hi) -> int { return defer ? MIMRL_OK : fork(lo, hi); };
  bool d_fused[MIMRL_MAX_BLOCKS] = {};
  MX(wt_images(stream, bf16, !(wtT_prebuilt && wtT_built), d_fused));
  auto W_join = [&](int lo, int hi) -> int { return defer ? MIMRL_OK : join(lo, hi); };
#define GRAB(var)                                                                                   \
  const int var = grab();                                                                           \
  if (var < 0) return set_error(MIMRL_ERR_STATE, "cube_backward: out of gradient buffers (line %d)", __LINE__)

  for (int i = cfg.n_blocks - 1; i >= 0; --i) {
    const BlockW& w = blk[i];
    BlockBuf& b = bb[i];
    const int il = dims[i][0], ik = dims[i][1], id = dims[i][2];
    const int hl = w.ax[0].hid, ol = w.ax[0].out, hk = w.ax[1].hid, ok = w.ax[1].out, hd = w.ax[2].hid, od = w.ax[2].out;
    const float* xblk = i == 0 ? cube0 : bb[i - 1].d.z;
    const float pl = cfg.dropout_mlp[0], pk = cfg.dropout_mlp[1], pd = cfg.dropout_mlp[2];
    if (d_fused[i]) {
      const AxisW& a = w.ax[2];
      const long R2 = (long)B * ol * ok;
      GRAB(i_dy); GRAB(i_du); GRAB(i_dx);
      DAxisBwdArgs fa;
      fa.dz = gbuf[cur]; fa.y = b.d.y; fa.mean = b.d.mean; fa.rstd = b.d.rstd; fa.gamma = P(a.ln_g); fa.u = b.d.u;
      fa.w2t = wtT[i][0]; fa.w1t = wtT[i][1]; fa.wrt = wtT[i][2];
      fa.dy = gbuf[i_dy]; fa.du = gbuf[i_du]; fa.dx = gbuf[i_dx];
      fa.R = R2; fa.act = cfg.activation;
      fa.dgamma = fa.dbeta = fa.db2 = fa.db1 = nullptr;
      MX(daxis_bwd_fused(stream, fa));
      MX(W_fork(1, 3));
      MX(W_dpg(2, b.d.y, b.d.mean, b.d.rstd, gbuf[cur], gbuf[i_dy], gbuf[i_du], Gm(a.ln_g), Gm(a.ln_b),
               a.fc2.b >= 0 ? Gm(a.fc2.b) : nullptr, a.fc1.b >= 0 ? Gm(a.fc1.b) : nullptr, R2));
      { GemmDesc g = gemm_tn(gbuf[i_dy], od, b.d.h, hd, Gm(a.fc2.w), hd, od, hd, (int)R2); g.atomic = 1; MX(W_gemm(1, g)); }
      { GemmDesc g = gemm_tn(gbuf[i_dy], od, b.k.z, id, Gm(a.res), id, od, id, (int)R2); g.atomic = 1; MX(W_gemm(2, g)); }
      { GemmDesc g = gemm_tn(gbuf[i_du], hd, b.k.z, id, Gm(a.fc1.w), id, hd, id, (int)R2); g.atomic = 1; MX(W_gemm(3, g)); }
      MX(W_join(1, 3));
      release(cur); release(i_dy); release(i_du);
      cur = i_dx;
    } else {
      const AxisW& a = w.ax[2];
      const long R2 = (long)B * ol * ok;
      const float* xin = b.k.z;
      const float* xmlp = cfg.ln_first ? b.d.xn : b.k.z;
      int i_dy = cur;
      if (!cfg.ln_first) {
        GRAB(q);
        MX(rowln_bwd(stream, b.d.y, P(a.ln_g), b.d.mean, b.d.rstd, gbuf[cur], gbuf[q], Gm(a.ln_g), Gm(a.ln_b), R2, od));
        release(cur);
        i_dy = q;
      }
      const float* dy = gbuf[i_dy];
      int i_dym = i_dy;
      if (pd > 0.f) {
        GRAB(q);
        HIPX(hipMemcpyAsync(gbuf[q], dy, sizeof(float) * R2 * od, hipMemcpyDeviceToDevice, stream));
        MX(dropout_inplace(stream, gbuf[q], R2 * od, pd, key(), 12 + 3 * i));
        i_dym = q;
      }
      const float* dym = gbuf[i_dym];
      MX(W_fork(1, 2));
      { GemmDesc g = gemm_tn(dym, od, b.d.h, hd, Gm(a.fc2.w), hd, od, hd, (int)R2); g.atomic = 1; MX(W_gemm(1, g)); }
      if (a.fc2.b >= 0) MX(W_colsum(1, dym, R2, od, od, Gm(a.fc2.b)));
      if (a.res >= 0) { GemmDesc g = gemm_tn(dy, od, xin, id, Gm(a.res), id, od, id, (int)R2); g.atomic = 1; MX(W_gemm(2, g)); }
      GRAB(i_du);
      { GemmDesc g = gemm_nn(dym, od, P(a.fc2.w), hd, gbuf[i_du], hd, (int)R2, hd, od); g.act = cfg.activation; g.gradact_u = b.d.u;
        if (a.fc1.b >= 0) g.colsum = Gm(a.fc1.b);
        MX(G_(g)); }
      MX(W_fork(3, 3));
      { GemmDesc g = gemm_tn(gbuf[i_du], hd, xmlp, id, Gm(a.fc1.w), id, hd, id, (int)R2); g.atomic = 1; MX(W_gemm(3, g)); }
      GRAB(i_dx0);
      int i_dx = i_dx0;
      const bool fuse_dx = a.res >= 0 && !cfg.ln_first;
      { GemmDesc g = gemm_nn(gbuf[i_du], hd, P(a.fc1.w), id, gbuf[i_dx], id, (int)R2, id, hd);
        if (fuse_dx) { g.A2 = dy; g.sa2_m = od; g.sa2_k = 1; g.B2 = P(a.res); g.sb2_k = id; g.sb2_n = 1; g.K2 = od; }
        MX(G_(g)); }
      if (cfg.ln_first) {
        MX(join(3, 3));
        MX(rowln_bwd(stream, b.k.z, P(a.ln_g), b.d.xn_mean, b.d.xn_rstd, gbuf[i_dx], gbuf[i_du], Gm(a.ln_g), Gm(a.ln_b), R2, id));
        release(i_dx);
        i_dx = i_du;
      } else {
        release(i_du);
      }
      if (!fuse_dx) {
        if (a.res >= 0) { GemmDesc g = gemm_nn(dy, od, P(a.res), id, gbuf[i_dx], id, (int)R2, id, od); g.beta = 1.f; MX(G_(g)); }
        else MX(add_inplace(stream, gbuf[i_dx], dy, R2 * id));
      }
      MX(W_join(1, 3));
      if (i_dym != i_dy) release(i_dym);
      release(i_dy);
      cur = i_dx;
    }
    {
      const AxisW& a = w.ax[1];
      KMixW kw;
      std::memset(&kw, 0, sizeof kw);
      kw.w1 = P(a.fc1.w); kw.b1 = a.fc1.b >= 0 ? P(a.fc1.b) : nullptr;
      kw.w2 = P(a.fc2.w); kw.b2 = a.fc2.b >= 0 ? P(a.fc2.b) : nullptr;
      kw.wr = a.res >= 0 ? P(a.res) : nullptr; kw.g = P(a.ln_g); kw.be = P(a.ln_b);
      kw.dw1 = Gm(a.fc1.w); kw.db1 = a.fc1.b >= 0 ? Gm(a.fc1.b) : nullptr;
      kw.dw2 = Gm(a.fc2.w); kw.db2 = a.fc2.b >= 0 ? Gm(a.fc2.b) : nullptr;
      kw.dwr = a.res >= 0 ? Gm(a.res) : nullptr; kw.dg = Gm(a.ln_g); kw.dbe = Gm(a.ln_b);
      kw.ik = ik; kw.hk = hk; kw.ok = ok; kw.act = cfg.activation; kw.ln_first = cfg.ln_first;
      kw.drop_p = pk; kw.key = key(); kw.stream_id = 11 + 3 * i;
      GRAB(q);
      static const int kmix_inchain = dbg_env("MIMRL_KMIX_PG_INCHAIN") ? atoi(dbg_env("MIMRL_KMIX_PG_INCHAIN")) : 1;
      if (defer && kmix_inchain) {
        MX(kmix_bwd(stream, b.l.z, gbuf[cur], gbuf[q], kw, (long)B * ol, id));
      } else if (defer) {
        MX(kmix_bwd_part(stream, b.l.z, gbuf[cur], gbuf[q], kw, (long)B * ol, id, 1));
        static const int kdbg = dbg_env("MIMRL_DBG_KMIX") ? atoi(dbg_env("MIMRL_DBG_KMIX")) : 0;
        static const bool kmix_park = dbg_env("MIMRL_KMIX_PG_PARKED") != nullptr;
        if (kmix_park) {
          Deferred d{5, 2, GemmDesc(), b.l.z, (long)B * ol, id, 0, 0, nullptr};
          d.p3 = gbuf[cur]; d.kw = kw; d.kw.dbg = kdbg;
          deferred.push_back(d);
        } else {
          KMixW kp = kw; kp.dbg = kdbg;
          MX(fork(3, 3));
          MX(kmix_bwd_part(S(3), b.l.z, gbuf[cur], nullptr, kp, (long)B * ol, id, 2));
          kmix_pg_on_side3 = true;
        }
      } else {
        MX(kmix_bwd(stream, b.l.z, gbuf[cur], gbuf[q], kw, (long)B * ol, id));
      }
      release(cur);
      cur = q;
    }
    if (bf16 && fused_cube_bwd && !cfg.ln_first && pl <= 0.f && w.ax[0].res >= 0 && laxis_bwd_supported(il, hl, ol, ik * id) &&
        (il <= 64 || laxis_bwd_long_on)) {
      const AxisW& a = w.ax[0];
      const long C = (long)ik * id;
      GRAB(i_dy); GRAB(i_du); GRAB(i_dx);
      LAxisBwdArgs fa;
      fa.dz = gbuf[cur]; fa.y = b.l.y; fa.mean = b.l.mean; fa.rstd = b.l.rstd; fa.gamma = P(a.ln_g); fa.u = b.l.u;
      fa.w2 = P(a.fc2.w); fa.w1 = P(a.fc1.w); fa.wr = P(a.res);
      fa.dy = gbuf[i_dy]; fa.du = gbuf[i_du]; fa.dx = gbuf[i_dx];
      fa.db2 = a.fc2.b >= 0 ? Gm(a.fc2.b) : nullptr; fa.db1 = a.fc1.b >= 0 ? Gm(a.fc1.b) : nullptr;
      fa.B = B; fa.il = il; fa.hl = hl; fa.ol = ol; fa.C = (int)C; fa.act = cfg.activation;
      MX(laxis_bwd_fused(stream, fa));
      MX(W_fork(1, 3));
      MX(W_lnpar(1, b.l.y, b.l.mean, b.l.rstd, gbuf[cur], Gm(a.ln_g), Gm(a.ln_b), B, ol, (int)C));
      release(cur);
      { GemmDesc g; g.A = gbuf[i_dy]; g.sa_m = C; g.sa_k = 1; g.sa_b = (long)ol * C;
        g.B = b.l.h; g.sb_k = 1; g.sb_n = C; g.sb_b = (long)hl * C;
        g.C = Gm(a.fc2.w); g.sc_m = hl; g.sc_n = 1; g.sc_b = 0; g.M = ol; g.N = hl; g.K = (int)C; g.batch = B; g.atomic = 1;
        MX(W_gemm(1, g)); }
      { GemmDesc g; g.A = gbuf[i_dy]; g.sa_m = C; g.sa_k = 1; g.sa_b = (long)ol * C;
        g.B = xblk; g.sb_k = 1; g.sb_n = C; g.sb_b = (long)il * C;
        g.C = Gm(a.res); g.sc_m = il; g.sc_n = 1; g.sc_b = 0; g.M = ol; g.N = il; g.K = (int)C; g.batch = B; g.atomic = 1;
        MX(W_gemm(2, g)); }
      { GemmDesc g; g.A = gbuf[i_du]; g.sa_m = C; g.sa_k = 1; g.sa_b = (long)hl * C;
        g.B = xblk; g.sb_k = 1; g.sb_n = C; g.sb_b = (long)il * C;
        g.C = Gm(a.fc1.w); g.sc_m = il; g.sc_n = 1; g.sc_b = 0; g.M = hl; g.N = il; g.K = (int)C; g.batch = B; g.atomic = 1;
        MX(W_gemm(3, g)); }
      MX(W_join(1, 3));
      release(i_dy); release(i_du);
      cur = i_dx;
    } else {
      const AxisW& a = w.ax[0];
      const long C = (long)ik * id;
      const float* xmlp = cfg.ln_first ? b.l.xn : xblk;
      int i_dy = cur;
      if (!cfg.ln_first) {
        GRAB(q);
        MX(colln_bwd(stream, b.l.y, P(a.ln_g), b.l.mean, b.l.rstd, gbuf[cur], gbuf[q], Gm(a.ln_g), Gm(a.ln_b), B, ol, (int)C));
        release(cur);
        i_dy = q;
      }
      const float* dy = gbuf[i_dy];
      int i_dym = i_dy;
      if (pl > 0.f) {
        GRAB(q);
        HIPX(hipMemcpyAsync(gbuf[q], dy, sizeof(float) * B * ol * C, hipMemcpyDeviceToDevice, stream));
        MX(dropout_inplace(stream, gbuf[q], (long)B * ol * C, pl, key(), 10 + 3 * i));
        i_dym = q;
      }
      const float* dym = gbuf[i_dym];
      MX(W_fork(1, 2));
      { GemmDesc g; g.A = dym; g.sa_m = C; g.sa_k = 1; g.sa_b = (long)ol * C;
        g.B = b.l.h; g.sb_k = 1; g.sb_n = C; g.sb_b = (long)hl * C;
        g.C = Gm(a.fc2.w); g.sc_m = hl; g.sc_n = 1; g.sc_b = 0; g.M = ol; g.N = hl; g.K = (int)C; g.batch = B; g.atomic = 1;
        MX(W_gemm(1, g)); }
      if (a.fc2.b >= 0) MX(W_rowsum(1, dym, B, ol, (int)C, Gm(a.fc2.b)));
      if (a.res >= 0) {
        GemmDesc g; g.A = dy; g.sa_m = C; g.sa_k = 1; g.sa_b = (long)ol * C;
        g.B = xblk; g.sb_k = 1; g.sb_n = C; g.sb_b = (long)il * C;
        g.C = Gm(a.res); g.sc_m = il; g.sc_n = 1; g.sc_b = 0; g.M = ol; g.N = il; g.K = (int)C; g.batch = B; g.atomic = 1;
        MX(W_gemm(2, g));
      }
      GRAB(i_du);
      { GemmDesc g; g.A = P(a.fc2.w); g.sa_m = 1; g.sa_k = hl; g.sa_b = 0;
        if (bf16 && w2p[i] && w2p_valid[i] && hl % 4 != 0) { g.A = w2p[i]; g.sa_k = (hl + 3) & ~3; g.a_pad4 = 1; }
        g.B = dym; g.sb_k = C; g.sb_n = 1; g.sb_b = (long)ol * C;
        g.C = gbuf[i_du]; g.sc_m = C; g.sc_n = 1; g.sc_b = (long)hl * C; g.M = hl; g.N = (int)C; g.K = ol; g.batch = B;
        g.act = cfg.activation; g.gradact_u = b.l.u;
        MX(G_(g)); }
      MX(W_fork(3, 3));
      { GemmDesc g; g.A = gbuf[i_du]; g.sa_m = C; g.sa_k = 1; g.sa_b = (long)hl * C;
        g.B = xmlp; g.sb_k = 1; g.sb_n = C; g.sb_b = (long)il * C;
        g.C = Gm(a.fc1.w); g.sc_m = il; g.sc_n = 1; g.sc_b = 0; g.M = hl; g.N = il; g.K = (int)C; g.batch = B; g.atomic = 1;
        MX(W_gemm(3, g)); }
      if (a.fc1.b >= 0) MX(W_rowsum(3, gbuf[i_du], B, hl, (int)C, Gm(a.fc1.b)));
      GRAB(i_dx0);
      int i_dx = i_dx0;
      { GemmDesc g; g.A = P(a.fc1.w); g.sa_m = 1; g.sa_k = il; g.sa_b = 0;
        g.B = gbuf[i_du]; g.sb_k = C; g.sb_n = 1; g.sb_b = (long)hl * C;
        g.C = gbuf[i_dx]; g.sc_m = C; g.sc_n = 1; g.sc_b = (long)il * C; g.M = il; g.N = (int)C; g.K = hl; g.batch = B;
        if (a.res >= 0 && !cfg.ln_first) {
          g.A2 = P(a.res); g.sa2_m = 1; g.sa2_k = il; g.sa2_b = 0;
          g.B2 = dy; g.sb2_k = C; g.sb2_n = 1; g.sb2_b = (long)ol * C; g.K2 = ol;
        }
        MX(G_(g)); }
      if (cfg.ln_first) {
        MX(join(3, 3));
        MX(colln_bwd(stream, xblk, P(a.ln_g), b.l.xn_mean, b.l.xn_rstd, gbuf[i_dx], gbuf[i_du], Gm(a.ln_g), Gm(a.ln_b), B, il, (int)C));
        release(i_dx);
        i_dx = i_du;
      } else {
        release(i_du);
      }
      if (a.res >= 0 && !cfg.ln_first) {
      } else if (a.res >= 0) {
        GemmDesc g; g.A = P(a.res); g.sa_m = 1; g.sa_k = il; g.sa_b = 0;
        g.B = dy; g.sb_k = C; g.sb_n = 1; g.sb_b = (long)ol * C;
        g.C = gbuf[i_dx]; g.sc_m = C; g.sc_n = 1; g.sc_b = (long)il * C; g.M = il; g.N = (int)C; g.K = ol; g.batch = B; g.beta = 1.f;
        MX(G_(g));
      } else {
        MX(add_inplace(stream, gbuf[i_dx], dy, (long)B * il * C));
      }
      MX(W_join(1, 3));
      if (i_dym != i_dy) release(i_dym);
      release(i_dy);
      cur = i_dx;
    }
    static const int early = dbg_env("MIMRL_EARLY_FLUSH") ? atoi(dbg_env("MIMRL_EARLY_FLUSH")) : 2;
    if (defer && (early == 2 || (early == 1 && i == cfg.n_blocks - 1))) MX(flush_deferred(1));
  }
#undef GRAB
  *cur_out = cur;
  return MIMRL_OK;
}

__global__ void dbg_spin_kernel(long ticks) {
  const long t0 = wall_clock64();
  while (wall_clock64() - t0 < ticks) __builtin_amdgcn_s_sleep(16);
}
int mimrl_handle::dbg_delay(hipStream_t st, int tag) {
  static const char* spec = knob("MIMRL_DBG_DELAY_TAG");
  static const int want = spec ? atoi(spec) : -1;
  static const int us = spec && strchr(spec, ':') ? atoi(strchr(spec, ':') + 1) : 50;
  if (tag != want) return MIMRL_OK;
  hipLaunchKernelGGL(dbg_spin_kernel, dim3(1), dim3(64), 0, st, (long)us * 100);
  LAUNCH_CHECK();
  return MIMRL_OK;
}

int mimrl_handle::flush_deferred(int only_side) {
  if (deferred.empty()) return MIMRL_OK;
  if (only_side > 0) MX(fork(only_side, only_side)); else MX(fork(1, 3));
  for (int q = 1; q <= 3; ++q) MX(dbg_delay(S(q), 9));
  constexpr int wg_sides = 3;
  static const int dbg_skip_kinds = dbg_env("MIMRL_DBG_SKIP_DEFERRED") ? atoi(dbg_env("MIMRL_DBG_SKIP_DEFERRED")) : 0;
  const bool groupk = !prof_on && bf16 && !((dbg_skip_kinds >> 0) & 1) && cfg.seq_len <= 128;
  if (groupk) {
    std::vector<GemmDesc> cls[2];
    for (const Deferred& d : deferred) if (d.kind == 0) cls[d.g.sa_k == 1 ? 0 : 1].push_back(d.g);
    for (int c = 0; c < 2; ++c) {
      hipStream_t st = only_side > 0 ? S(only_side) : S(1 + c % wg_sides);
      for (size_t i = 0; i < cls[c].size(); i += 12) MX(gemm_group_splitk(st, cls[c].data() + i, (int)std::min<size_t>(12, cls[c].size() - i), bf16));
    }
  }
  int rr = 2;
  for (const Deferred& d : deferred) {
    if ((dbg_skip_kinds >> d.kind) & 1) continue;
    if (groupk && d.kind == 0) continue;
    static const bool dbg_defer_main = dbg_env("MIMRL_DBG_DEFER_MAIN") != nullptr;
    hipStream_t st = dbg_defer_main ? stream : only_side > 0 ? S(only_side) : S(1 + (groupk ? rr++ : d.side - 1) % wg_sides);
    if (d.kind == 0) MX(G_on(st, d.g));
    else if (d.kind == 1) MX(colsum(st, d.src, d.n0, (int)d.n1, (int)d.n2, d.dst));
    else if (d.kind == 2) MX(rowsum_batched(st, d.src, (int)d.n0, (int)d.n1, (int)d.n2, d.dst));
    else if (d.kind == 3) MX(colln_param_grads(st, d.src, d.p1, d.p2, d.p3, d.dst, d.dst2, (int)d.n0, (int)d.n1, (int)d.n2));
    else if (d.kind == 6) MX(daxis_param_grads(st, d.src, d.p1, d.p2, d.p3, d.p4, d.p5, d.dst, d.dst2, d.dst3, d.dst4, d.n0));
    else MX(kmix_bwd_part(st, d.src, d.p3, nullptr, d.kw, d.n0, (int)d.n1, 2));
  }
  deferred.clear();
  return MIMRL_OK;
}

int mimrl_handle::model_backward() {
  Range rg("mimrl.model_backward");
  DetDefer det_defer(stream, &det_ranges);
  const int B = cfg.batch, T = cfg.seq_len, L = cfg.time_len, D = cfg.d_common;
  const long BT_ = (long)B * T;
  const int nb = cfg.n_blocks;
  const int ol = cfg.d_outs[nb - 1][0], ok = cfg.d_outs[nb - 1][1], od = cfg.d_outs[nb - 1][2];
  MX(head_bwd(stream, dfeat, dpred, P(cls_w), bufs.feats, gbuf[0], Gm(cls_w), Gm(cls_b), B, ol, ok, od,
              cfg.compose_t_sum, cfg.compose_k_sum, head_gather_on ? &head_gather : nullptr, ncls()));
  int ci = 0;
  deferred.clear();
  { Scope sc(this, MIMRL_PH_CUBE_BWD); MX(cube_backward(0, &ci)); }
  MX(dbg_delay(stream, 7));
  return encoders_backward(gbuf[ci]);
}

int mimrl_handle::encoders_backward(float* dcube) {
  const int B = cfg.batch, T = cfg.seq_len, L = cfg.time_len, D = cfg.d_common;
  const long BT_ = (long)B * T;
  const float* dmean = dfeat + (size_t)B * D;
  if (head_gather_on && ev_dmean) { HIPX(hipStreamWaitEvent(stream, ev_dmean, 0)); ev_dmean = nullptr; }
  {
    LnSide2 sd[2];
    for (int m = 0; m < 2; ++m)
      sd[m] = LnSide2{h1[m], P(ln_g[m]), P(ln_b[m]), ln_mean[m], ln_rstd[m], ds[m], Gm(ln_g[m]), Gm(ln_b[m]), 1 + m,
                      cfg.dropout[1 + m], (uint32_t)(1 + m)};
    ds_bf16_live = rec16_on && cfg.encoder == MIMRL_ENCODER_GRU && dg_bf16 && (prec & MIMRL_PREC_BF16_GRU_BWD) != 0 && gru_bwd_io16_ok(0);
    MX(ln_relu_drop_bwd2(stream, sd[0], sd[1], dcube, B, T, L, 3, D, key(), dmean + (size_t)B * D, dmean + 2 * (size_t)B * D, ds_bf16_live ? 1 : 0));
  }
  MX(fork(0, 0));
  MX(text_post_bwd(S(0), dcube, dtx, B, T, L, 3, D, 0, cfg.dropout[0], key(), 0, dmean));
  { GemmDesc g = gemm_tn(dtx, D, bufs.text, cfg.d_t, Gm(w_t), cfg.d_t, D, cfg.d_t, (int)BT_); g.atomic = 1; MX(G_on(S(0), g)); }
  static const int dbg_join_at = dbg_env("MIMRL_DBG_JOIN_AT") ? atoi(dbg_env("MIMRL_DBG_JOIN_AT")) : 0;
  MX(flush_deferred());
  if (dbg_join_at == 1) MX(join(1, 3));
  if (cfg.encoder != MIMRL_ENCODER_GRU) kmix_pg_on_side3 = false;
  if (cfg.encoder == MIMRL_ENCODER_CONV) {
    MX(conv_backward());
    MX(join(0, 5));
    return MIMRL_OK;
  }
  if (cfg.encoder == MIMRL_ENCODER_LSTM) {
    MX(lstm_encoders_backward());
    MX(join(0, 5));
    return MIMRL_OK;
  }
  if (kmix_pg_on_side3) { MX(join(3, 3)); kmix_pg_on_side3 = false; }
// ... 158 lines not shown
```

### mimrl_amd/csrc/engine_forward.hip

```cpp
#include "engine.h"

int mimrl_handle::encoders_forward(bool save, int knn_stage) {
  if (cfg.encoder == MIMRL_ENCODER_CONV) return conv_forward(knn_stage);
  if (cfg.encoder == MIMRL_ENCODER_LSTM) return lstm_encoders_forward(save, knn_stage);
  const int B = cfg.batch, T = cfg.seq_len;
  const long BT_ = (long)B * T;
  const float* xin[2] = {bufs.audio, bufs.video};
  const int dmod[2] = {cfg.d_a, cfg.d_v};
  if (!ev_lens) MX(seq_lengths2(S(4), xin[0], dmod[0], lens[0], xin[1], dmod[1], lens[1], B, T));
  const bool use_h16 = h16_on && l0_packed && bf16 && fwd_f16 && (prec & MIMRL_PREC_BF16_GRU_FWD) && h0h[0] && w1h;
  if (save) { h16_live = use_h16; hp16_live = false; }
  for (int l = 0; l < 2; ++l) {
    GruFwdArgs a;
    a.B = B; a.T = T; a.out_ld = 2 * H; a.nmod = 2;
    a.btv = gru_pick_btv(B, 2);
    a.gx_f16 = gx_f16 ? 1 : 0;
    a.stamp = kstamp; a.stamp.id = l;
    if (l == 1) MX(fork(1, 3));
    if (l == 0 && !l0_packed && l0_bwd_pack && save) {
      L0Pack pk;
      for (int m = 0; m < 2; ++m) { pk.x[m] = xin[m]; pk.d[m] = dmod[m]; for (int d = 0; d < 2; ++d) { pk.w_ih[m][d] = nullptr; pk.b_ih[m][d] = nullptr; } }
      pk.xpack = xpack; pk.wpack = wpack; pk.bpack = bpack; pk.rows = BT_; pk.KP = KP();
      MX(l0_pack(S(0), pk, true, false));
    }
// ... 198 lines not shown
    if (save || keep_cube0) {
      cpre.cube = cube0;
      for (int m = 0; m < 2; ++m) { cpre.mean[m] = ln_mean[m]; cpre.rstd[m] = ln_rstd[m]; }
    }
  } else if (!pre_done) {
    LnSide2 sd[2];
    for (int m = 0; m < 2; ++m)
      sd[m] = LnSide2{h1[m], P(ln_g[m]), P(ln_b[m]), ln_mean[m], ln_rstd[m], nullptr, nullptr, nullptr, 1 + m, pdrop[1 + m],
                      (uint32_t)(1 + m)};
    if (fused_pre) {
      MX(tail_pre_fwd(stream, tx_raw, pdrop[0], sd[0], sd[1], cube0, bufs.feats + (size_t)B * D, B, T, L, 3, D, key()));
    } else {
      MX(ln_relu_drop_fwd2(stream, sd[0], sd[1], cube0, B, T, L, 3, D, key()));
      MX(feat_mean_fwd(stream, cube0, bufs.feats + (size_t)B * D, B, T, L, 3, D));
    }
  }
  const BlockBuf& last = bb[cfg.n_blocks - 1];
  const int ol = cfg.d_outs[cfg.n_blocks - 1][0], ok = cfg.d_outs[cfg.n_blocks - 1][1], od = cfg.d_outs[cfg.n_blocks - 1][2];
  if (od != D) return set_error(MIMRL_ERR_ARG, "last block d_out must equal d_common (features feed 128-wide estimators)");
  CubeHead chead;
  chead.w = P(cls_w); chead.bias = P(cls_b); chead.ff = bufs.feats; chead.pred = bufs.pred; chead.C = ncls();
  chead.scale = (cfg.compose_t_sum ? 1.f : 1.f / ol) * (cfg.compose_k_sum ? 1.f : 1.f / ok);
  { Scope sc(this, MIMRL_PH_CUBE_FWD); MX(cube_forward(train, save, fold_pre ? &cpre : nullptr, fold_head ? &chead : nullptr)); }
  MX(dbg_delay(stream, save ? 2 : 13));
  if (!fold_head)
    MX(head_fwd(stream, last.d.z, P(cls_w), P(cls_b), bufs.feats, bufs.pred, B, ol, ok, od, cfg.compose_t_sum,
                cfg.compose_k_sum, ncls()));
  (void)ff;
  return MIMRL_OK;
}

int mimrl_handle::dual_tail_pre() {
  const int B = cfg.batch, T = cfg.seq_len, L = cfg.time_len, D = cfg.d_common;
  float* const cubes[2] = {cube0, alt.cube0};
  float* const feats[2] = {bufs.feats + (size_t)B * D, alt.feats + (size_t)B * D};
  const int add[2] = {1, 0};
  if (T < L)
    for (int o = 0; o < 2; ++o) HIPX(hipMemsetAsync(cubes[o], 0, sizeof(float) * (size_t)B * L * 3 * D, stream));
  LnSide2 sd[2];
  for (int m = 0; m < 2; ++m)
    sd[m] = LnSide2{h1[m], P(ln_g[m]), P(ln_b[m]), ln_mean[m], ln_rstd[m], nullptr, nullptr, nullptr, 1 + m, cfg.dropout[1 + m], (uint32_t)(1 + m)};
  MX(tail_pre2_fwd(stream, tx_raw, cfg.dropout[0], sd[0], sd[1], cubes, feats, add, tailp_part, B, T, L, 3, D, key()));
  return MIMRL_OK;
}

bool mimrl_handle::cube_block_fused(int i, bool train) const {
  if (!bf16 || !fused_cube || i < 0 || i >= cfg.n_blocks) return false;
  int il = cfg.time_len, ik = 3, id = cfg.d_common;
  for (int j = 0; j < i; ++j) { il = blk[j].ax[0].out; ik = blk[j].ax[1].out; id = blk[j].ax[2].out; }
  const BlockW& w = blk[i];
  const float pmlp[3] = {train ? cfg.dropout_mlp[0] : 0.f, train ? cfg.dropout_mlp[1] : 0.f, train ? cfg.dropout_mlp[2] : 0.f};
  return cube_fused_supported(il, w.ax[0].hid, w.ax[0].out, ik, w.ax[1].hid, w.ax[1].out, id, w.ax[2].hid, w.ax[2].out, cfg.ln_first != 0,
                              cfg.res_project[i] != 0, cfg.bias != 0, pmlp);
}

int mimrl_handle::cube_forward(bool train, bool save, const CubePre* pre, const CubeHead* head) {
  const int B = cfg.batch;
  const float* x = cube0;
  int il = cfg.time_len, ik = 3, id = cfg.d_common;
  const bool no_fused = !fused_cube;
  for (int i = 0; i < cfg.n_blocks; ++i) {
    const BlockW& w = blk[i];
    BlockBuf& b = bb[i];
    const int hl = w.ax[0].hid, ol = w.ax[0].out, hk = w.ax[1].hid, ok = w.ax[1].out, hd = w.ax[2].hid, od = w.ax[2].out;
    const float pl = train ? cfg.dropout_mlp[0] : 0.f, pk = train ? cfg.dropout_mlp[1] : 0.f,
                pd = train ? cfg.dropout_mlp[2] : 0.f;
    const float pmlp[3] = {pl, pk, pd};
    if (bf16 && !no_fused &&
        cube_fused_supported(il, hl, ol, ik, hk, ok, id, hd, od, cfg.ln_first != 0, cfg.res_project[i] != 0, cfg.bias != 0, pmlp)) {
      CubeFusedArgs fa;
      std::memset(&fa, 0, sizeof fa);
      auto PB = [&](long off) -> const float* { return off >= 0 ? P(off) : nullptr; };
      fa.x = x;
      fa.l_w1 = P(w.ax[0].fc1.w); fa.l_b1 = PB(w.ax[0].fc1.b); fa.l_w2 = P(w.ax[0].fc2.w); fa.l_b2 = PB(w.ax[0].fc2.b);
      fa.l_wr = P(w.ax[0].res); fa.l_g = P(w.ax[0].ln_g); fa.l_be = P(w.ax[0].ln_b);
      fa.kw.w1 = P(w.ax[1].fc1.w); fa.kw.b1 = PB(w.ax[1].fc1.b); fa.kw.w2 = P(w.ax[1].fc2.w); fa.kw.b2 = PB(w.ax[1].fc2.b);
      fa.kw.wr = P(w.ax[1].res); fa.kw.g = P(w.ax[1].ln_g); fa.kw.be = P(w.ax[1].ln_b);
      fa.kw.ik = ik; fa.kw.hk = hk; fa.kw.ok = ok; fa.kw.act = cfg.activation; fa.kw.ln_first = 0; fa.kw.drop_p = 0.f;
      fa.kw.key = key(); fa.kw.stream_id = 0;
      fa.d_w1 = P(w.ax[2].fc1.w); fa.d_b1 = PB(w.ax[2].fc1.b); fa.d_w2 = P(w.ax[2].fc2.w); fa.d_b2 = PB(w.ax[2].fc2.b);
      fa.d_wr = P(w.ax[2].res); fa.d_g = P(w.ax[2].ln_g); fa.d_be = P(w.ax[2].ln_b);
      if (save) {
        fa.l_u = b.l.u; fa.l_h = b.l.h; fa.l_y = b.l.y; fa.l_z = b.l.z; fa.l_mean = b.l.mean; fa.l_rstd = b.l.rstd;
        fa.k_z = b.k.z;
        fa.d_u = b.d.u; fa.d_h = b.d.h; fa.d_y = b.d.y; fa.d_mean = b.d.mean; fa.d_rstd = b.d.rstd;
      }
      fa.d_z = b.d.z;
      fa.dbg_phase = dbg_env("MIMRL_CUBE_PHASE") ? atoi(dbg_env("MIMRL_CUBE_PHASE")) : 0;
      fa.B = B; fa.il = il; fa.hl = hl; fa.ol = ol; fa.K = ik; fa.act = cfg.activation; fa.save = save ? 1 : 0;
      if (fa.dbg_phase == 100) { fa.save = 0; fa.dbg_phase = 0; }
      if (pre && i == 0) { fa.pre_on = 1; fa.pre = *pre; }
      if (head && i == cfg.n_blocks - 1) { fa.head_on = 1; fa.head = *head; }
      MX(cube_block_fwd_fused(stream, fa));
      x = b.d.z;
      il = ol; ik = ok; id = od;
      continue;
    }
    {
      const AxisW& a = w.ax[0];
      const long C = (long)ik * id;
      const float* xi = x;
      const bool long_l = bf16 && laxis_long_on && !cfg.ln_first && pl <= 0.f && a.res >= 0 && laxis_fwd_long_supported(il, hl, ol, (int)C);
      if (long_l) {
        if (w2p[i] && hl % 4 != 0) {
          MX(pad_rows(stream, P(a.fc2.w), w2p[i], ol, hl, (hl + 3) & ~3));
          w2p_valid[i] = true;
        }
        LAxisLongArgs la;
        la.x = x; la.w1 = P(a.fc1.w); la.b1 = a.fc1.b >= 0 ? P(a.fc1.b) : nullptr; la.w2 = P(a.fc2.w); la.b2 = a.fc2.b >= 0 ? P(a.fc2.b) : nullptr;
        la.wr = P(a.res); la.g = P(a.ln_g); la.be = P(a.ln_b);
        la.u = b.l.u; la.h = b.l.h; la.y = b.l.y; la.z = b.l.z; la.mean = b.l.mean; la.rstd = b.l.rstd;
        la.B = B; la.il = il; la.hl = hl; la.ol = ol; la.C = (int)C; la.act = cfg.activation;
        MX(laxis_fwd_long(stream, la, fwd_f16));
      } else {
      if (cfg.ln_first) { MX(colln_fwd(stream, x, P(a.ln_g), P(a.ln_b), b.l.xn, b.l.xn_mean, b.l.xn_rstd, B, il, (int)C)); xi = b.l.xn; }
      GemmDesc g1;
      g1.A = P(a.fc1.w); g1.sa_m = il; g1.sa_k = 1; g1.sa_b = 0;
      g1.B = xi; g1.sb_k = C; g1.sb_n = 1; g1.sb_b = (long)il * C;
      g1.C = b.l.h; g1.sc_m = C; g1.sc_n = 1; g1.sc_b = (long)hl * C;
      g1.M = hl; g1.N = (int)C; g1.K = il; g1.batch = B;
      g1.bias_m = a.fc1.b >= 0 ? P(a.fc1.b) : nullptr; g1.act = cfg.activation; g1.pre = b.l.u;
      g1.f16 = fwd_f16;
      MX(G_(g1));
      GemmDesc g2;
      g2.A = P(a.fc2.w); g2.sa_m = hl; g2.sa_k = 1;
      if (bf16 && w2p[i] && hl % 4 != 0) {
        const int hp = (hl + 3) & ~3;
        MX(pad_rows(stream, P(a.fc2.w), w2p[i], ol, hl, hp));
        w2p_valid[i] = true;
        g2.A = w2p[i]; g2.sa_m = hp; g2.a_pad4 = 1;
      }
      g2.B = b.l.h; g2.sb_k = C; g2.sb_n = 1; g2.sb_b = (long)hl * C;
      g2.C = b.l.y; g2.sc_m = C; g2.sc_n = 1; g2.sc_b = (long)ol * C;
      g2.M = ol; g2.N = (int)C; g2.K = hl; g2.batch = B;
      g2.bias_m = a.fc2.b >= 0 ? P(a.fc2.b) : nullptr;
      const bool fuse_res = a.res >= 0 && pl <= 0.f;
      if (fuse_res) {
        g2.A2 = P(a.res); g2.sa2_m = il; g2.sa2_k = 1; g2.sa2_b = 0;
        g2.B2 = x; g2.sb2_k = C; g2.sb2_n = 1; g2.sb2_b = (long)il * C; g2.K2 = il;
      }
      MX(G_(g2));
      if (!fuse_res) {
        MX(dropout_inplace(stream, b.l.y, (long)B * ol * C, pl, key(), 10 + 3 * i));
// ... 2 lines not shown
          g3.A = P(a.res); g3.sa_m = il; g3.B = x; g3.sb_b = (long)il * C; g3.K = il; g3.bias_m = nullptr; g3.beta = 1.f;
          MX(G_(g3));
        } else {
          MX(add_inplace(stream, b.l.y, x, (long)B * ol * C));
        }
      }
      if (!cfg.ln_first) MX(colln_fwd(stream, b.l.y, P(a.ln_g), P(a.ln_b), b.l.z, b.l.mean, b.l.rstd, B, ol, (int)C));
      }
    }
    {
      const AxisW& a = w.ax[1];
      KMixW kw;
      std::memset(&kw, 0, sizeof kw);
      kw.w1 = P(a.fc1.w); kw.b1 = a.fc1.b >= 0 ? P(a.fc1.b) : nullptr;
      kw.w2 = P(a.fc2.w); kw.b2 = a.fc2.b >= 0 ? P(a.fc2.b) : nullptr;
      kw.wr = a.res >= 0 ? P(a.res) : nullptr; kw.g = P(a.ln_g); kw.be = P(a.ln_b);
      kw.ik = ik; kw.hk = hk; kw.ok = ok; kw.act = cfg.activation; kw.ln_first = cfg.ln_first;
      kw.drop_p = pk; kw.key = key(); kw.stream_id = 11 + 3 * i;
      MX(kmix_fwd(stream, b.l.z, b.k.z, kw, (long)B * ol, id));
    }
    {
      const AxisW& a = w.ax[2];
      const long R2 = (long)B * ol * ok;
      const float* xi = b.k.z;
      if (cfg.ln_first) { MX(rowln_fwd(stream, b.k.z, P(a.ln_g), P(a.ln_b), b.d.xn, b.d.xn_mean, b.d.xn_rstd, R2, id)); xi = b.d.xn; }
      GemmDesc g1 = gemm_nt(xi, id, P(a.fc1.w), id, b.d.h, hd, (int)R2, hd, id);
      g1.bias_n = a.fc1.b >= 0 ? P(a.fc1.b) : nullptr; g1.act = cfg.activation; g1.pre = b.d.u;
      MX(G_(g1));
      GemmDesc g2 = gemm_nt(b.d.h, hd, P(a.fc2.w), hd, b.d.y, od, (int)R2, od, hd);
      g2.bias_n = a.fc2.b >= 0 ? P(a.fc2.b) : nullptr;
      const bool fuse_res = a.res >= 0 && pd <= 0.f;
      if (fuse_res) {
        g2.A2 = b.k.z; g2.sa2_m = id; g2.sa2_k = 1; g2.B2 = P(a.res); g2.sb2_k = 1; g2.sb2_n = id; g2.K2 = id;
      }
      MX(G_(g2));
      if (!fuse_res) {
        MX(dropout_inplace(stream, b.d.y, R2 * od, pd, key(), 12 + 3 * i));
        if (a.res >= 0) {
          GemmDesc g3 = gemm_nt(b.k.z, id, P(a.res), id, b.d.y, od, (int)R2, od, id);
          g3.beta = 1.f;
          MX(G_(g3));
        } else {
          MX(add_inplace(stream, b.d.y, b.k.z, R2 * od));
        }
      }
      if (!cfg.ln_first) MX(rowln_fwd(stream, b.d.y, P(a.ln_g), P(a.ln_b), b.d.z, b.d.mean, b.d.rstd, R2, od));
    }
    x = b.d.z;
    il = ol; ik = ok; id = od;
  }
  return MIMRL_OK;
}

int mimrl_handle::wt_images(hipStream_t st, bool bwd_bf16, bool launch, bool* d_fused) {
  int din2 = cfg.d_common;
  WtTransposeArgs ta;
  ta.n = 0;
  for (int i = 0; i < cfg.n_blocks; ++i) {
    const AxisW& a = blk[i].ax[2];
    d_fused[i] = bwd_bf16 && fused_cube_bwd && !cfg.ln_first && cfg.dropout_mlp[2] <= 0.f && a.res >= 0 &&
                 daxis_bwd_supported(din2, a.hid, a.out) && ta.n + 3 <= 12;
    din2 = cfg.d_outs[i][2];
    if (!d_fused[i]) continue;
    const long srcs[3] = {a.fc2.w, a.fc1.w, a.res};
    for (int q = 0; q < 3; ++q) { ta.src[ta.n] = P(srcs[q]); ta.dst[ta.n] = wtT[i][q]; ++ta.n; }
  }
  if (launch && ta.n > 0) MX(wt_transpose_bf16(st, ta));
  return MIMRL_OK;
}
```

### mimrl_amd/csrc/gemm.hip

```cpp
#include <cstdio>
#include "gemm.h"

#include <type_traits>

#include <cstdlib>

namespace mimrl {

namespace {

constexpr int BM = 64, BN = 64;

inline bool aligned16(const void* p) { return (reinterpret_cast<uintptr_t>(p) & 15) == 0; }

template <bool BF16, int BK>
struct Smem;
template <int BK>
struct Smem<false, BK> {
  float a[BK][BM + 4];
  float b[BK][BN + 4];
};
template <int BK>
struct Smem<true, BK> {
  __bf16 a[BM][BK + 8];
// ... 439 lines not shown
template <int T, bool KC, bool BF, bool F16 = false>
__device__ __forceinline__ void fast_store(const f32x4* v, __bf16* __restrict__ img, int tid) {
  if constexpr (BF) {
    if constexpr (KC) {
#pragma unroll
      for (int h = 0; h < T; ++h) {
        const int idx = h * 256 + tid;
        *reinterpret_cast<f32x4*>(img + (idx >> 2) * FT<T>::KCP + (idx & 3) * 8) = v[h];
      }
    } else {
      const int rq = tid & (8 * T - 1), kq = tid / (8 * T);
#pragma unroll
      for (int j = 0; j < T; ++j) *reinterpret_cast<f32x4*>(img + (kq * T + j) * FT<T>::RCP + rq * 8) = v[j];
    }
  } else if constexpr (KC) {
#pragma unroll
    for (int h = 0; h < FT<T>::NV; ++h) {
      const int idx = h * 256 + tid;
      *reinterpret_cast<bf16x4*>(img + (idx >> 3) * FT<T>::KCP + (idx & 7) * 4) = cvt4<F16>(v[h]);
    }
  } else {
    constexpr int KB = FT<T>::KB;
    const int rq = tid & (16 * T - 1), kq = tid / (16 * T);
#pragma unroll
    for (int j = 0; j < KB; ++j) *reinterpret_cast<bf16x4*>(img + (kq * KB + j) * FT<T>::RCP + rq * 4) = cvt4<F16>(v[j]);
  }
}

template <int T, bool KC>
__device__ __forceinline__ bf16x8 fast_frag(const __bf16* __restrict__ img, int rb, int s, int lane) {
  if constexpr (KC) {
    return *reinterpret_cast<const bf16x8*>(img + (rb + (lane & 31)) * FT<T>::KCP + s * 16 + 8 * (lane >> 5));
  } else {
    typedef __attribute__((address_space(3))) bf16x4 lds4;
    const int j = lane & 15, q = j >> 2, p = j & 3;
    const __bf16* a = img + (s * 16 + 8 * (lane >> 5) + q) * FT<T>::RCP + rb + 16 * ((lane >> 4) & 1) + 4 * p;
    const bf16x4 lo = __builtin_amdgcn_ds_read_tr16_b64_v4bf16((lds4*)(a));
    const bf16x4 hi = __builtin_amdgcn_ds_read_tr16_b64_v4bf16((lds4*)(a + 4 * FT<T>::RCP));
    bf16x8 r;
    r[0] = lo[0]; r[1] = lo[1]; r[2] = lo[2]; r[3] = lo[3]; r[4] = hi[0]; r[5] = hi[1]; r[6] = hi[2]; r[7] = hi[3];
    return r;
  }
}

__device__ __forceinline__ void h8_to_bf8(f32x4& v) {
  const f16x8 h = __builtin_bit_cast(f16x8, v);
  bf16x8 o;
#pragma unroll
  for (int i = 0; i < 8; ++i) o[i] = to_bf16((float)h[i]);
  v = __builtin_bit_cast(f32x4, o);
}

template <int TM, int TN, bool AKC, bool BKC, bool GEN, bool ABF = false, bool BBF = false, bool F16 = false, bool BH = false>
__device__ __forceinline__ void fast_body(const GemmDesc& d, int ksplit, int kt_per, int dbg, unsigned bx, unsigned by, unsigned bzr) {
  constexpr int BMf = 64 * TM, BNf = 64 * TN;
  __shared__ __attribute__((aligned(16))) __bf16 sA[2][FT<TM>::ELEMS];
  __shared__ __attribute__((aligned(16))) __bf16 sB[2][FT<TN>::ELEMS];
  const int tid = threadIdx.x, lane = tid & 63, wave = tid >> 6;
  const int wm = wave >> 1, wn = wave & 1;
  const int bz = bzr / ksplit, ks = bzr - bz * ksplit;
  long oa = (long)bz * d.sa_b, ob = (long)bz * d.sb_b, oc = (long)bz * d.sc_b, obn = (long)bz * d.bias_n_b;
  if (d.batch_in > 0) {
    const int bo = bz / d.batch_in, bi = bz - bo * d.batch_in;
    oa = (long)bo * d.sa_bo + (long)bi * d.sa_b; ob = (long)bo * d.sb_bo + (long)bi * d.sb_b;
    oc = (long)bo * d.sc_bo + (long)bi * d.sc_b; obn = (long)bo * d.bias_n_bo + (long)bi * d.bias_n_b;
  }
  const int m0 = by * BMf, n0 = bx * BNf;
  f32x16 acc[TM][TN];
#pragma unroll
  for (int i = 0; i < TM; ++i)
#pragma unroll
    for (int j = 0; j < TN; ++j)
#pragma unroll
      for (int r = 0; r < 16; ++r) acc[i][j][r] = 0.f;
  float bn_pre[TN];
#pragma unroll
  for (int j = 0; j < TN; ++j) {
    const int n = n0 + wn * 32 * TN + j * 32 + (lane & 31);
    bn_pre[j] = d.bias_n ? d.bias_n[obn + (n < d.N ? n : d.N - 1)] : 0.f;
  }

  auto segment = [&](const float* __restrict__ Ap, long sa, const float* __restrict__ Bp, long sb, int K, int kt0, int kt1, int ga_at, int ga) {
    constexpr int LA = FL<TM, ABF>::N, LB = FL<TN, BBF>::N;
    f32x4 ra[FPF][LA], rb[FPF][LB];
    if (kt0 >= kt1) return;
    const int last = kt1 - 1;
    auto request = [&](auto J, int kt) __attribute__((always_inline)) {
      constexpr int j = decltype(J)::value;
      const int t = kt < last ? kt : last;
      fast_load<TM, AKC, ABF>(Ap, sa, m0, d.M, ga_at, ga, K, t * FBK, tid, ra[j]);
      fast_load<TN, BKC, BBF>(Bp, sb, n0, d.N, 0x7fffffff, 0, K, t * FBK, tid, rb[j]);
    };
    auto publish = [&](auto J, int buf, int kt) __attribute__((always_inline)) {
      constexpr int j = decltype(J)::value;
      const int t = kt < last ? kt : last;
      fast_wait<LA, (FPF - 1) * (LA + LB) + LB>(ra[j]);
      fast_wait<LB, (FPF - 1) * (LA + LB)>(rb[j]);
      fast_fix<TM, AKC, ABF>(m0, d.M, K, t * FBK, tid, ra[j]);
      fast_fix<TN, BKC, BBF>(n0, d.N, K, t * FBK, tid, rb[j]);
      if constexpr (BH) {
#pragma unroll
        for (int h = 0; h < LB; ++h) h8_to_bf8(rb[j][h]);
      }
      fast_store<TM, AKC, ABF, F16>(ra[j], sA[buf], tid);
      fast_store<TN, BKC, BBF, F16>(rb[j], sB[buf], tid);
    };
    gemm_static_for<0, FPF>([&](auto J) __attribute__((always_inline)) { request(J, kt0 + decltype(J)::value); });
    publish(std::integral_constant<int, 0>{}, 0, kt0);
    __syncthreads();
    int cur = 0;
// ... 6 lines not shown
        request(J, kt + FPF);
#pragma unroll
        for (int s = 0; s < FBK / 16; ++s) {
          bf16x8 af[TM], bfr[TN];
#pragma unroll
          for (int i = 0; i < TM; ++i) af[i] = fast_frag<TM, AKC>(sA[cur], wm * 32 * TM + i * 32, s, lane);
#pragma unroll
          for (int jn = 0; jn < TN; ++jn) bfr[jn] = fast_frag<TN, BKC>(sB[cur], wn * 32 * TN + jn * 32, s, lane);
#pragma unroll
          for (int i = 0; i < TM; ++i)
#pragma unroll
            for (int jn = 0; jn < TN; ++jn) {
              if constexpr (F16) acc[i][jn] = __builtin_amdgcn_mfma_f32_32x32x16_f16(__builtin_bit_cast(f16x8, af[i]), __builtin_bit_cast(f16x8, bfr[jn]), acc[i][jn], 0, 0, 0);
              else acc[i][jn] = __builtin_amdgcn_mfma_f32_32x32x16_bf16(af[i], bfr[jn], acc[i][jn], 0, 0, 0);
            }
        }
        publish(std::integral_constant<int, (j + 1) % FPF>{}, cur ^ 1, kt + 1);
        __syncthreads();
        cur ^= 1;
      });
    }
    asm volatile("s_waitcnt vmcnt(0)" : : : "memory");
  };
  {
    const int ktiles = (d.K + FBK - 1) / FBK;
    const int kt0 = ks * kt_per;
    const int kt1 = dbg == 2 ? kt0 : (kt0 + kt_per < ktiles ? kt0 + kt_per : ktiles);
    const float* Ab = ABF ? reinterpret_cast<const float*>(reinterpret_cast<const __bf16*>(d.A) + oa) : d.A + oa;
    const float* Bb = BBF ? reinterpret_cast<const float*>(reinterpret_cast<const __bf16*>(d.B) + ob) : d.B + ob;
    segment(Ab, AKC ? d.sa_m : d.sa_k, Bb, BKC ? d.sb_n : d.sb_k, d.K, kt0, kt1, d.a_gap_rows ? d.a_gap_at : 0x7fffffff, d.a_gap_rows);
  }
  if (d.A2) {
    const long oa2 = (long)bz * d.sa2_b, ob2 = (long)bz * d.sb2_b;
    const float* Ab = ABF ? reinterpret_cast<const float*>(reinterpret_cast<const __bf16*>(d.A2) + oa2) : d.A2 + oa2;
    const float* Bb = BBF ? reinterpret_cast<const float*>(reinterpret_cast<const __bf16*>(d.B2) + ob2) : d.B2 + ob2;
    segment(Ab, AKC ? d.sa2_m : d.sa2_k, Bb, BKC ? d.sb2_n : d.sb2_k, d.K2, 0, (d.K2 + FBK - 1) / FBK, 0x7fffffff, 0);
  }
  if (dbg == 1) { if (acc[0][0][0] == 123.456f) d.C[0] = 1.f; return; }
  if constexpr (!GEN && TN == 2) {
    if (d.c_f16 && d.sc_n == 1 && d.N % 64 == 0) {
#pragma unroll
      for (int i = 0; i < TM; ++i)
        epilogue_f16_pair(d, oc, bn_pre[0], bn_pre[1], acc[i][0], acc[i][1], m0 + wm * 32 * TM + i * 32, n0 + wn * 64, lane);
      return;
    }
  }
#pragma unroll
  for (int i = 0; i < TM; ++i)
#pragma unroll
    for (int j = 0; j < TN; ++j)
      epilogue<GEN>(d, d.atomic || ksplit > 1, bz, oc, bn_pre[j], acc[i][j], m0 + wm * 32 * TM + i * 32, n0 + wn * 32 * TN + j * 32 + (lane & 31), lane);
}

template <int TM, int TN, bool AKC, bool BKC, bool GEN>
__global__ __launch_bounds__(256) void gemm_fast_kernel(KernelArgs ka) {
  unsigned bx, by, bzr;
  tile_ids(ka.xcd_remap, bx, by, bzr);
  fast_body<TM, TN, AKC, BKC, GEN>(ka.d, ka.ksplit, ka.kt_per, ka.dbg, bx, by, bzr);
}
template <int TM, int TN, bool GEN>
__global__ __launch_bounds__(256) void gemm_fast_f16_kernel(KernelArgs ka) {
  unsigned bx, by, bzr;
  tile_ids(ka.xcd_remap, bx, by, bzr);
  fast_body<TM, TN, true, true, GEN, false, false, true>(ka.d, ka.ksplit, ka.kt_per, ka.dbg, bx, by, bzr);
}
template <int TM, int TN>
__global__ __launch_bounds__(256) void gemm_fast_f16s_kernel(KernelArgs ka) {
  unsigned bx, by, bzr;
  tile_ids(ka.xcd_remap, bx, by, bzr);
  fast_body<TM, TN, true, true, false, true, true, true>(ka.d, ka.ksplit, ka.kt_per, ka.dbg, bx, by, bzr);
}
template <int TM, int TN, bool AKC, bool BKC, bool BBF>
__global__ __launch_bounds__(256) void gemm_fast_bf_kernel(KernelArgs ka) {
  unsigned bx, by, bzr;
  tile_ids(ka.xcd_remap, bx, by, bzr);
  fast_body<TM, TN, AKC, BKC, false, true, BBF>(ka.d, ka.ksplit, ka.kt_per, ka.dbg, bx, by, bzr);
}

template <int TM, int TN>
__global__ __launch_bounds__(256) void gemm_fast_bfh_kernel(KernelArgs ka) {
  unsigned bx, by, bzr;
  tile_ids(ka.xcd_remap, bx, by, bzr);
  fast_body<TM, TN, false, false, false, true, true, false, true>(ka.d, ka.ksplit, ka.kt_per, ka.dbg, bx, by, bzr);
}

struct GroupArgs {
  GemmDesc d[GEMM_GROUP_MAX];
  int start[GEMM_GROUP_MAX + 1];
  int n;
};
template <bool AKC, bool BKC>
__global__ __launch_bounds__(256) void gemm_group_kernel(GroupArgs ga) {
  int p = 0;
#pragma unroll
  for (int q = 1; q < GEMM_GROUP_MAX; ++q)
    if (q < ga.n && (int)blockIdx.x >= ga.start[q]) p = q;
  const GemmDesc& d = ga.d[p];
  const unsigned t = blockIdx.x - ga.start[p];
  const unsigned nx = (d.N + 63) / 64, ny = (d.M + 63) / 64;
  fast_body<1, 1, AKC, BKC, false>(d, 1, (d.K + FBK - 1) / FBK, 0, t % nx, (t / nx) % ny, t / (nx * ny));
}

constexpr int GEMM_GROUPK_MAX = 12;
struct GroupKProb {
  const float* A; const float* B; float* C;
  int M, N, K, batch;
  long sa, sa_b, sb, sb_b, sc_m, sc_b;
  int nsplit, kt_per;
};
struct GroupKArgs {
  GroupKProb p[GEMM_GROUPK_MAX];
  int start[GEMM_GROUPK_MAX];
  int n;
};
template <bool AKC, bool BKC>
__global__ __launch_bounds__(256) void gemm_groupk_kernel(GroupKArgs ga) {
  int p = 0;
#pragma unroll
  for (int q = 1; q < GEMM_GROUPK_MAX; ++q)
    if (q < ga.n && (int)blockIdx.x >= ga.start[q]) p = q;
  const GroupKProb& g = ga.p[p];
  GemmDesc d;
  d.A = g.A; d.B = g.B; d.C = g.C; d.M = g.M; d.N = g.N; d.K = g.K; d.batch = g.batch;
  d.sa_m = AKC ? g.sa : 1; d.sa_k = AKC ? 1 : g.sa; d.sa_b = g.sa_b;
  d.sb_n = BKC ? g.sb : 1; d.sb_k = BKC ? 1 : g.sb; d.sb_b = g.sb_b;
  d.sc_m = g.sc_m; d.sc_n = 1; d.sc_b = g.sc_b; d.atomic = 1;
  const unsigned t = blockIdx.x - ga.start[p];
  const unsigned nx = (g.N + 63) / 64, ny = (g.M + 63) / 64;
  fast_body<1, 1, AKC, BKC, false>(d, g.nsplit, g.kt_per, 0, t % nx, (t / nx) % ny, t / (nx * ny));
}

inline int fast_class(const float* P, long s_r, long s_k, long s_b, long s_bo, int R, int K, int bf = 0, int pad4 = 0) {
  const int q = bf ? 8 : 4;
  if (!aligned16(P) || s_b % q != 0 || s_bo % q != 0) return 0;
  const bool pad = pad4 && !bf;
  if (s_k == 1 && s_r % q == 0 && (K % q == 0 || pad) && K >= q && s_r != 1) return 1;
  if (s_r == 1 && s_k % q == 0 && (R % q == 0 || pad) && R >= q) return 2;
  return 0;
}

inline bool vec_ok_a(const float* P, long s_m, long s_k, long s_b) {
  return aligned16(P) && s_b % 4 == 0 && ((s_k == 1 && s_m % 4 == 0) || (s_m == 1 && s_k != 1 && s_k % 4 == 0));
}
inline bool vec_ok_b(const float* P, long s_k, long s_n, long s_b) {
  return aligned16(P) && s_b % 4 == 0 && ((s_k == 1 && s_n != 1 && s_n % 4 == 0) || (s_n == 1 && s_k % 4 == 0));
}

}

static bool plain_accumulate(const GemmDesc& d) {
  return !d.A2 && d.atomic && d.beta == 0.f && !d.bias_n && !d.bias_m && !d.pre && !d.gradact_u && !d.colsum && d.act == ACT_NONE;
}

static bool fast_plan(const GemmDesc& d, bool bf16, GemmPlan* p) {
  if (!bf16) return false;
  const int ca = fast_class(d.A, d.sa_m, d.sa_k, d.sa_b, d.sa_bo, d.M, d.K, d.a_bf16, d.a_pad4), cb = fast_class(d.B, d.sb_n, d.sb_k, d.sb_b, d.sb_bo, d.N, d.K, d.b_bf16);
  if (!ca || !cb || (ca == 2 && cb == 1)) return false;
  if (d.A2 && (fast_class(d.A2, d.sa2_m, d.sa2_k, d.sa2_b, 0, d.M, d.K2, d.a_bf16) != ca || fast_class(d.B2, d.sb2_n, d.sb2_k, d.sb2_b, 0, d.N, d.K2, d.b_bf16) != cb))
    return false;
  if (d.a_bf16 || d.b_bf16) {
    if (!d.a_bf16 || (ca == 1 && cb == 1 && !(d.f16 && d.b_bf16)) || d.bias_m || d.beta != 0.f || d.pre || d.gradact_u) return false;
    if (d.f16 && !(ca == 1 && cb == 1 && d.b_bf16)) return false;
    if (d.a_gap_rows && (d.a_gap_at % 8 != 0 || d.a_gap_rows % 8 != 0)) return false;
    if (d.b_f16cvt && !(ca == 2 && cb == 2 && d.b_bf16 && !d.A2)) return false;
  }
  const int ktiles = (d.K + FBK - 1) / FBK;
  const bool acc = plain_accumulate(d) && ktiles >= 32;
  auto tiles = [&](int tm, int tn) { return (long)((d.M + 64 * tm - 1) / (64 * tm)) * ((d.N + 64 * tn - 1) / (64 * tn)) * d.batch; };
  auto split = [&](long t) {
    if (!acc) return 1;
    long ks = (512 + t - 1) / t;
    if (ks > ktiles / 16) ks = ktiles / 16;
    return (int)(ks < 1 ? 1 : ks);
  };
  const int cand[3][2] = {{2, 2}, {2, 1}, {1, 1}};
  int pick = 2;
  for (int c = 0; c < 3; ++c) {
    const int tm = cand[c][0], tn = cand[c][1];
    if (d.M < 64 * tm || d.N < 64 * tn) continue;
    const long t = tiles(tm, tn);
    constexpr long min_wgs = 700;
    if (t * split(t) >= ((acc && ktiles > 1024) ? 224 : min_wgs) || c == 2) { pick = c; break; }
  }
  p->fast = 1; p->tm = cand[pick][0]; p->tn = cand[pick][1]; p->ca = ca; p->cb = cb;
  p->tiles = tiles(p->tm, p->tn);
  p->nsplit = split(p->tiles);
  p->kt_per = (ktiles + p->nsplit - 1) / p->nsplit;
  p->variant = 10 + 4 * pick + (ca == 1 ? (cb == 1 ? 0 : 1) : 2);
  return true;
}

void gemm_plan(const GemmDesc& d, bool bf16, GemmPlan* p) {
  p->fast = 0; p->tm = p->tn = 1; p->ca = p->cb = 0;
  if (fast_plan(d, bf16, p)) return;
  const bool va = vec_ok_a(d.A, d.sa_m, d.sa_k, d.sa_b) && d.sa_bo % 4 == 0, vb = vec_ok_b(d.B, d.sb_k, d.sb_n, d.sb_b) && d.sb_bo % 4 == 0;
  const bool va2 = d.A2 ? vec_ok_a(d.A2, d.sa2_m, d.sa2_k, d.sa2_b) : true, vb2 = d.B2 ? vec_ok_b(d.B2, d.sb2_k, d.sb2_n, d.sb2_b) : true;
  const bool a_kfast = d.sa_k == 1 && (!d.A2 || d.sa2_k == 1), b_kfast = d.sb_k == 1 && d.sb_n != 1 && (!d.B2 || (d.sb2_k == 1 && d.sb2_n != 1));
  const bool lean = bf16 && (d.M % BM == 0 || a_kfast) && (d.N % BN == 0 || b_kfast) &&
                    va && vb && va2 && vb2 && d.K >= 64;
  const long tiles = (long)((d.N + BN - 1) / BN) * ((d.M + BM - 1) / BM) * d.batch;
  const bool lean128 = lean && tiles <= 256 && d.K >= 128 && (!d.A2 || d.K2 >= 64);
  p->variant = !bf16 ? 0 : lean128 ? 3 : lean ? 2 : 1;
  const int BKh = lean128 ? 128 : (lean ? 64 : 32);
  const int ktiles = (d.K + BKh - 1) / BKh;
  p->nsplit = 1; p->kt_per = ktiles; p->tiles = tiles;
  if (plain_accumulate(d) && ktiles >= 8) {
    int ksplit = (int)((512 + tiles - 1) / tiles);
    if (ksplit > ktiles / 4) ksplit = ktiles / 4;
    if (ksplit < 1) ksplit = 1;
    p->nsplit = ksplit;
    p->kt_per = (ktiles + ksplit - 1) / ksplit;
  }
}

int gemm_group(hipStream_t s, const GemmDesc* ds, int n, bool bf16) {
  bool ok = bf16 && n >= 2 && n <= GEMM_GROUP_MAX;
  int ca = 0, cb = 0;
  long total = 0;
  for (int i = 0; ok && i < n; ++i) {
    const GemmDesc& d = ds[i];
    if (d.M <= 0 || d.N <= 0 || d.batch <= 0 || !d.A || !d.B || !d.C) { ok = false; break; }
    const int a = fast_class(d.A, d.sa_m, d.sa_k, d.sa_b, d.sa_bo, d.M, d.K), b = fast_class(d.B, d.sb_n, d.sb_k, d.sb_b, d.sb_bo, d.N, d.K);
    if (!a || !b || (a == 2 && b == 1) || (i > 0 && (a != ca || b != cb))) { ok = false; break; }
    ca = a; cb = b;
    if (d.A2 || d.bias_m || d.beta != 0.f || d.pre || d.gradact_u || d.a_gap_rows || d.a_bf16 || d.b_bf16) { ok = false; break; }
    total += (long)((d.M + 63) / 64) * ((d.N + 63) / 64) * d.batch;
  }
  if (!ok || total > 65535L * 16) {
    for (int i = 0; i < n; ++i) MX(gemm(s, ds[i], bf16));
    return MIMRL_OK;
  }
  GroupArgs ga;
  ga.n = n;
  int acc = 0;
  for (int i = 0; i < GEMM_GROUP_MAX; ++i) {
    if (i < n) { ga.d[i] = ds[i]; ga.start[i] = acc; acc += ((ds[i].M + 63) / 64) * ((ds[i].N + 63) / 64) * ds[i].batch; }
    else { ga.d[i] = GemmDesc(); ga.start[i] = 0x7fffffff; }
  }
  ga.start[GEMM_GROUP_MAX] = acc;
  if (ca == 1 && cb == 1) hipLaunchKernelGGL((gemm_group_kernel<true, true>), dim3(acc), dim3(256), 0, s, ga);
  else if (ca == 1) hipLaunchKernelGGL((gemm_group_kernel<true, false>), dim3(acc), dim3(256), 0, s, ga);
  else hipLaunchKernelGGL((gemm_group_kernel<false, false>), dim3(acc), dim3(256), 0, s, ga);
  LAUNCH_CHECK();
  return MIMRL_OK;
}

int gemm_group_splitk(hipStream_t s, const GemmDesc* ds, int n, bool bf16) {
  bool ok = bf16 && n >= 2 && n <= GEMM_GROUPK_MAX;
  int ca = 0, cb = 0;
  long tiles = 0;
  double macs = 0;
  for (int i = 0; ok && i < n; ++i) {
    const GemmDesc& d = ds[i];
    if (d.M <= 0 || d.N <= 0 || d.batch <= 0 || !d.A || !d.B || !d.C) { ok = false; break; }
    const int a = fast_class(d.A, d.sa_m, d.sa_k, d.sa_b, d.sa_bo, d.M, d.K), b = fast_class(d.B, d.sb_n, d.sb_k, d.sb_b, d.sb_bo, d.N, d.K);
    if (!a || !b || a != b || (i > 0 && a != ca)) { ok = false; break; }
    ca = a; cb = b;
    if (!plain_accumulate(d) || d.alpha != 1.f || d.sc_n != 1 || d.batch_in > 0 || d.a_gap_rows || d.a_bf16 || d.b_bf16) { ok = false; break; }
    tiles += (long)((d.M + 63) / 64) * ((d.N + 63) / 64) * d.batch;
    macs += (double)d.M * d.N * d.K * d.batch;
  }
  if (macs > 3e9) ok = false;
  if (!ok) {
    for (int i = 0; i < n; ++i) MX(gemm(s, ds[i], bf16));
    return MIMRL_OK;
  }
  (void)cb;
  GroupKArgs ga;
  ga.n = n;
  const long want = (768 + tiles - 1) / tiles;
  long acc = 0;
  for (int i = 0; i < GEMM_GROUPK_MAX; ++i) {
    if (i >= n) { ga.p[i] = GroupKProb(); ga.start[i] = 0x7fffffff; continue; }
    const GemmDesc& d = ds[i];
    GroupKProb& g = ga.p[i];
    g.A = d.A; g.B = d.B; g.C = d.C; g.M = d.M; g.N = d.N; g.K = d.K; g.batch = d.batch;
    g.sa = ca == 1 ? d.sa_m : d.sa_k; g.sa_b = d.sa_b; g.sb = ca == 1 ? d.sb_n : d.sb_k; g.sb_b = d.sb_b;
    g.sc_m = d.sc_m; g.sc_b = d.sc_b;
    const int ktiles = (d.K + FBK - 1) / FBK;
    long ks = want < 1 ? 1 : want;
    if (ks > ktiles / 8) ks = ktiles / 8;
    if (ks < 1) ks = 1;
    g.kt_per = (int)((ktiles + ks - 1) / ks);
    g.nsplit = (ktiles + g.kt_per - 1) / g.kt_per;
    ga.start[i] = (int)acc;
    acc += (long)((d.M + 63) / 64) * ((d.N + 63) / 64) * d.batch * g.nsplit;
  }
  if (acc > 0x7fffffffL) return set_error(MIMRL_ERR_ARG, "gemm_group_splitk: grid too large");
  if (ca == 1) hipLaunchKernelGGL((gemm_groupk_kernel<true, true>), dim3((unsigned)acc), dim3(256), 0, s, ga);
  else hipLaunchKernelGGL((gemm_groupk_kernel<false, false>), dim3((unsigned)acc), dim3(256), 0, s, ga);
  LAUNCH_CHECK();
  return MIMRL_OK;
}

int gemm(hipStream_t s, const GemmDesc& d, bool bf16) {
  if (d.M <= 0 || d.N <= 0 || d.batch <= 0) return MIMRL_OK;
  static const int dbg_skip = dbg_env("MIMRL_DBG_SKIP_WGRAD") ? atoi(dbg_env("MIMRL_DBG_SKIP_WGRAD")) : 0;
  if (dbg_skip && d.atomic && (dbg_skip == 1 || (dbg_skip == 2 && d.batch > 1 && d.sc_b == 0))) return MIMRL_OK;
  if (!d.A || !d.B || !d.C) return set_error(MIMRL_ERR_ARG, "gemm: null operand");
  if ((d.A2 != nullptr) != (d.B2 != nullptr)) return set_error(MIMRL_ERR_ARG, "gemm: second product needs both operands");
  if (d.a_gap_rows && (d.a_gap_at % 4 != 0 || d.a_gap_rows % 4 != 0 || d.A2))
    return set_error(MIMRL_ERR_ARG, "gemm: the A-row gap must be a multiple of 4 rows (single product only)");
  if (d.batch_in > 0 && (d.A2 || d.bias_m || d.colsum || d.batch % d.batch_in != 0))
    return set_error(MIMRL_ERR_ARG, "gemm: two-level batch supports A, B, C, bias_n only");
  if (bf16 && gemm_tall_ok(d)) return gemm_tall(s, d);
  if (d.c_bf16) return set_error(MIMRL_ERR_ARG, "gemm: a bf16-stored output exists in the tall LDS-DMA kernel only (gemm_tall_ok)");
  GemmPlan pl;
  gemm_plan(d, bf16, &pl);
#ifdef MIMRL_GEMM_TRACE_BUILD
  constexpr bool trace = true;
#else
  constexpr bool trace = false;
#endif
  if (trace && bf16 && !pl.fast)
    fprintf(stderr, "[gemm] generic: M %d N %d K %d batch %d | A %p sa %ld %ld %ld cls %d | B %p sb %ld %ld %ld cls %d | A2 %d K2 %d bias_m %d beta %g pre %d gu %d atomic %d\n",
            d.M, d.N, d.K, d.batch, (const void*)d.A, d.sa_m, d.sa_k, d.sa_b, fast_class(d.A, d.sa_m, d.sa_k, d.sa_b, d.sa_bo, d.M, d.K, d.a_bf16),
            (const void*)d.B, d.sb_k, d.sb_n, d.sb_b, fast_class(d.B, d.sb_n, d.sb_k, d.sb_b, d.sb_bo, d.N, d.K, d.b_bf16), d.A2 != nullptr, d.K2,
            d.bias_m != nullptr, (double)d.beta, d.pre != nullptr, d.gradact_u != nullptr, d.atomic);
  if (d.c_f16 && (d.atomic || pl.nsplit > 1 || d.bias_m || d.beta != 0.f || d.pre || d.gradact_u || d.colsum))
    return set_error(MIMRL_ERR_ARG, "gemm: an fp16-stored output takes the plain store only (no atomic / split-K / beta / pre / column sums)");
  DetNoFlush det_nf(!(d.atomic || pl.nsplit > 1 || d.colsum));
  DetGemmTarget det_gt(d.colsum ? nullptr : d.C);
  KernelArgs ka;
  ka.d = d;
  ka.vec_a = vec_ok_a(d.A, d.sa_m, d.sa_k, d.sa_b) && d.sa_bo % 4 == 0;
  ka.vec_b = vec_ok_b(d.B, d.sb_k, d.sb_n, d.sb_b) && d.sb_bo % 4 == 0;
  ka.vec_a2 = d.A2 ? vec_ok_a(d.A2, d.sa2_m, d.sa2_k, d.sa2_b) : 1;
  ka.vec_b2 = d.B2 ? vec_ok_b(d.B2, d.sb2_k, d.sb2_n, d.sb2_b) : 1;
  ka.xcd_remap = 1;
  static const int dbg_gemm = dbg_env("MIMRL_DBG_GEMM") ? atoi(dbg_env("MIMRL_DBG_GEMM")) : 0;
  ka.dbg = dbg_gemm;
  ka.ksplit = pl.nsplit;
  ka.kt_per = pl.kt_per;
  const int bm = 64 * pl.tm, bn = 64 * pl.tn;
  dim3 grid((d.N + bn - 1) / bn, (d.M + bm - 1) / bm, d.batch * pl.nsplit);
  if (grid.y > 65535 || grid.z > 65535) return set_error(MIMRL_ERR_ARG, "gemm: grid too large (M=%d batch=%d)", d.M, d.batch);
  const bool gen = d.bias_m || d.beta != 0.f || d.pre || d.gradact_u;
  if ((d.a_bf16 || d.b_bf16) && !pl.fast)
    return set_error(MIMRL_ERR_ARG, "gemm: bf16-stored operands need the fast path (bf16 mode, 8-element alignment, A bf16, layouts KC/RC or RC/RC, plain epilogue)");
  if (d.b_f16cvt && !(d.a_bf16 && d.b_bf16)) return set_error(MIMRL_ERR_ARG, "gemm: b_f16cvt needs a_bf16 = b_bf16 = 1");
#define FASTK(TM_, TN_, A_, B_)                                                                               \
  if (d.f16 && d.a_bf16) hipLaunchKernelGGL((gemm_fast_f16s_kernel<TM_, TN_>), grid, dim3(256), 0, s, ka);    \
  else if (d.f16 && gen) hipLaunchKernelGGL((gemm_fast_f16_kernel<TM_, TN_, true>), grid, dim3(256), 0, s, ka);    \
  else if (d.f16) hipLaunchKernelGGL((gemm_fast_f16_kernel<TM_, TN_, false>), grid, dim3(256), 0, s, ka);     \
  else if (gen) hipLaunchKernelGGL((gemm_fast_kernel<TM_, TN_, A_, B_, true>), grid, dim3(256), 0, s, ka);    \
  else hipLaunchKernelGGL((gemm_fast_kernel<TM_, TN_, A_, B_, false>), grid, dim3(256), 0, s, ka);            \
  break
#define FASTB(TM_, TN_, A_, B_)                                                                               \
  if (d.b_f16cvt) { if constexpr (!(A_) && !(B_)) hipLaunchKernelGGL((gemm_fast_bfh_kernel<TM_, TN_>), grid, dim3(256), 0, s, ka); } \
  else if (d.a_bf16 && d.b_bf16) hipLaunchKernelGGL((gemm_fast_bf_kernel<TM_, TN_, A_, B_, true>), grid, dim3(256), 0, s, ka);   \
  else if (d.a_bf16) hipLaunchKernelGGL((gemm_fast_bf_kernel<TM_, TN_, A_, B_, false>), grid, dim3(256), 0, s, ka);         \
  else if (gen) hipLaunchKernelGGL((gemm_fast_kernel<TM_, TN_, A_, B_, true>), grid, dim3(256), 0, s, ka);    \
  else hipLaunchKernelGGL((gemm_fast_kernel<TM_, TN_, A_, B_, false>), grid, dim3(256), 0, s, ka);            \
  break
#define GENK(BF_, BK_, LEAN_)                                                                                 \
  if (gen) hipLaunchKernelGGL((gemm_kernel<BF_, BK_, LEAN_, true>), grid, dim3(256), 0, s, ka);               \
  else hipLaunchKernelGGL((gemm_kernel<BF_, BK_, LEAN_, false>), grid, dim3(256), 0, s, ka);                  \
  break
  switch (pl.variant) {
    case 10: FASTK(2, 2, true, true);
    case 11: FASTB(2, 2, true, false);
    case 12: FASTB(2, 2, false, false);
    case 14: FASTK(2, 1, true, true);
    case 15: FASTB(2, 1, true, false);
    case 16: FASTB(2, 1, false, false);
    case 18: FASTK(1, 1, true, true);
    case 19: FASTB(1, 1, true, false);
    case 20: FASTB(1, 1, false, false);
    case 0: GENK(false, 32, false);
    case 3: GENK(true, 128, true);
    case 2: GENK(true, 64, true);
    default: GENK(true, 32, false);
  }
#undef FASTB
#undef GENK
#undef FASTK
  LAUNCH_CHECK();
  return MIMRL_OK;
}

}
```

Baseline: 1233.

## Save cube activations and backward gradients in bf16 and consume them in wgrad GEMMs

Adds a 16-bit save mode to the fused cube forward, which writes the saved hidden activations and outputs as bf16, and a bf16 output mode to the L-axis and D-axis backward kernels for dY and dU. The grouped split-K weight-gradient GEMM and the K-contiguous fast path are extended to read bf16 A and B operands directly. The aim is to halve activation and gradient memory traffic and skip fp32 round-trips between stages. It adds precision loss on the saved tensors and more template variants.

```diff
diff --git a/include/mimrl.h b/include/mimrl.h
--- a/include/mimrl.h
+++ b/include/mimrl.h
@@ -191,6 +191,8 @@
 int mimrl_probe_knn(mimrl_handle* h, int stage, int32_t* idx_out);
 int mimrl_op_adam(void* stream, float* p, float* g, float* m, float* v, int64_t n, const float* lr, const int32_t* step,
                   float beta1, float beta2, float eps, float weight_decay, float clip);
+int mimrl_op_gemm_wgrad_group16(void* stream, int n, const void* const* A, const void* const* B, float* const* C, const int32_t* dims,
+                                const int64_t* strides, const int32_t* storage, int grouped);
 
 #ifdef __cplusplus
 }
diff --git a/mimrl_amd/_lib.py b/mimrl_amd/_lib.py
--- a/mimrl_amd/_lib.py
+++ b/mimrl_amd/_lib.py
@@ -105,6 +105,8 @@
                                     C.POINTER(C.c_int64), C.c_int, C.POINTER(C.c_int64), _FP, C.c_int]
     lib.mimrl_op_gemm_wgrad_group.argtypes = [_FP, C.c_int, C.POINTER(C.c_void_p), C.POINTER(C.c_void_p), C.POINTER(C.c_void_p),
                                               C.POINTER(C.c_int32), C.POINTER(C.c_int64), C.c_int]
+    lib.mimrl_op_gemm_wgrad_group16.argtypes = [_FP, C.c_int, C.POINTER(C.c_void_p), C.POINTER(C.c_void_p), C.POINTER(C.c_void_p),
+                                                C.POINTER(C.c_int32), C.POINTER(C.c_int64), C.POINTER(C.c_int32), C.c_int]
     lib.mimrl_op_adam.argtypes = [_FP, _FP, _FP, _FP, _FP, C.c_int64, _FP, _FP, C.c_float, C.c_float, C.c_float,
                                   C.c_float, C.c_float]
     lib.mimrl_op_gru_forward.argtypes = [_FP] * 11 + [C.c_int, C.c_int, C.c_int]
@@ -166,7 +168,7 @@
     "mimrl_op_cmi_loss", "mimrl_op_sample_anchors", "mimrl_knn_r1_host", "mimrl_set_knn_override_mask", "mimrl_op_mlp_stack_forward", "mimrl_op_mlp_stack_backward", "mimrl_op_adam",
     "mimrl_probe_cube", "mimrl_probe_mi", "mimrl_probe_cmi", "mimrl_probe_knn", "mimrl_probe_encoders", "mimrl_set_kernel_stamps", "mimrl_comm_unique_id", "mimrl_set_comm", "mimrl_main_late_offset", "mimrl_set_comm_critic_bf16",
     "mimrl_stage1_pipe_prime", "mimrl_stage1_pipe", "mimrl_set_task_loss", "mimrl_op_task_loss", "mimrl_set_class_loss", "mimrl_op_class_loss",
-    "mimrl_op_mi_infonce_rows", "mimrl_op_lstm_forward", "mimrl_op_lstm_backward", "mimrl_op_recur_btv",
+    "mimrl_op_mi_infonce_rows", "mimrl_op_lstm_forward", "mimrl_op_lstm_backward", "mimrl_op_recur_btv", "mimrl_op_gemm_wgrad_group16",
 ]
 
 TASK_LOSSES = {"MAE": 0, "MSE": 1, "RMSE": 2, "SIMSE": 3, "CCC": 4}
diff --git a/mimrl_amd/csrc/cube_bwd_fused.h b/mimrl_amd/csrc/cube_bwd_fused.h
--- a/mimrl_amd/csrc/cube_bwd_fused.h
+++ b/mimrl_amd/csrc/cube_bwd_fused.h
@@ -11,6 +11,7 @@
   float *dy, *du, *dx;
   float *db2, *db1;
   int B, il, hl, ol, C, act;
+  int out16 = 0;
 };
 bool laxis_bwd_supported(int il, int hl, int ol, int C);
 int laxis_bwd_fused(hipStream_t s, const LAxisBwdArgs& a);
@@ -23,6 +24,7 @@
   long R;
   int act;
   float *dgamma, *dbeta, *db2, *db1;
+  int out16 = 0;
 };
 bool daxis_bwd_supported(int id, int hd, int od);
 int daxis_bwd_fused(hipStream_t s, const DAxisBwdArgs& a);
@@ -31,7 +33,7 @@
 int wt_transpose_bf16(hipStream_t s, const WtTransposeArgs& a);
 
 int daxis_param_grads(hipStream_t s, const float* y, const float* mean, const float* rstd, const float* dz, const float* dy,
-                      const float* du, float* dgamma, float* dbeta, float* db2, float* db1, long R);
+                      const float* du, float* dgamma, float* dbeta, float* db2, float* db1, long R, bool in16 = false);
 
 #ifdef MIMRL_PHASE_PROBE
 int cube_bwd_read_phases(long long* out);
diff --git a/mimrl_amd/csrc/cube_bwd_fused.hip b/mimrl_amd/csrc/cube_bwd_fused.hip
--- a/mimrl_amd/csrc/cube_bwd_fused.hip
+++ b/mimrl_amd/csrc/cube_bwd_fused.hip
@@ -16,7 +16,7 @@
 constexpr int KP = 64 + 8;
 
 
-template <bool LONG = false>
+template <bool LONG = false, bool O16 = false>
 __global__ __launch_bounds__(256, LONG ? 2 : 1) void laxis_bwd_kernel(LAxisBwdArgs a) {
   __shared__ __attribute__((aligned(16))) __bf16 sdyu[2][CT][KP];
   auto& sdy = sdyu[0];
@@ -80,6 +80,7 @@
   const float* __restrict__ dzb = a.dz + (long)b * ol * C + c0 + col;
   const float* __restrict__ yb = a.y + (long)b * ol * C + c0 + col;
   float* __restrict__ dyb = a.dy + (long)b * ol * C + c0 + col;
+  __bf16* __restrict__ dyb16 = reinterpret_cast<__bf16*>(a.dy) + (long)b * ol * C + c0 + col;
   float gq[32], xq[32];
 #pragma unroll
   for (int j = 0; j < 32; ++j) {
@@ -105,8 +106,9 @@
     const int l = half + 2 * j;
     if (l < ol) {
       const float v = rs * (gq[j] - s1 - xq[j] * s2);
-      dyb[(long)l * C] = v;
-      sdy[col][l] = to_bf16(v);
+      const __bf16 vb = to_bf16(v);
+      if constexpr (O16) dyb16[(long)l * C] = vb; else dyb[(long)l * C] = v;
+      sdy[col][l] = vb;
     }
   }
   for (int l = ol + ((half ^ ol) & 1); l < 64; l += 2) sdy[col][l] = to_bf16(0.f);
@@ -142,7 +144,7 @@
         if (h < hl) {
           const long ui = ((long)b * hl + h) * C + cc;
           v = (mt == 0 ? acc0[r] : acc1[r]) * act_grad_c<decltype(AT)::value>(a.act, uu[mt][r]);
-          a.du[ui] = v;
+          if constexpr (O16) reinterpret_cast<__bf16*>(a.du)[ui] = to_bf16(v); else a.du[ui] = v;
         }
         sdu[nt * 32 + lr][h] = to_bf16(v);
         if (a.db1) {
@@ -249,7 +251,9 @@
 int laxis_bwd_fused(hipStream_t s, const LAxisBwdArgs& a) {
   if (!laxis_bwd_supported(a.il, a.hl, a.ol, a.C)) return set_error(MIMRL_ERR_ARG, "laxis_bwd_fused: unsupported shape");
   if (!a.wr) return set_error(MIMRL_ERR_ARG, "laxis_bwd_fused: needs the residual projection");
+  if (a.out16 && a.il > 64) return set_error(MIMRL_ERR_ARG, "laxis_bwd_fused: bf16 dY / dU exist for il <= 64 only");
   if (a.il > 64) hipLaunchKernelGGL(laxis_bwd_kernel<true>, dim3(a.C / CT, a.B), dim3(256), 0, s, a);
+  else if (a.out16) hipLaunchKernelGGL((laxis_bwd_kernel<false, true>), dim3(a.C / CT, a.B), dim3(256), 0, s, a);
   else hipLaunchKernelGGL(laxis_bwd_kernel<false>, dim3(a.C / CT, a.B), dim3(256), 0, s, a);
   LAUNCH_CHECK();
   return MIMRL_OK;
@@ -260,6 +264,7 @@
 constexpr int DR = 32;
 constexpr int DP = 128 + 8;
 
+template <bool O16>
 __global__ __launch_bounds__(256) void daxis_bwd_kernel(DAxisBwdArgs a) {
   __shared__ __attribute__((aligned(16))) __bf16 sdy[DR][DP];
   __shared__ __attribute__((aligned(16))) __bf16 sdu[DR][DP];
@@ -326,8 +331,9 @@
         const int c = part * 16 + q * 4 + j;
         v[j] = rs * (g[q * 4 + j] * a.gamma[c] - s1 - xh[q * 4 + j] * s2);
       }
-      if (ok) *reinterpret_cast<float4*>(a.dy + r * 128 + part * 16 + q * 4) = make_float4(v[0], v[1], v[2], v[3]);
       bf16x4 p; p[0] = to_bf16(v[0]); p[1] = to_bf16(v[1]); p[2] = to_bf16(v[2]); p[3] = to_bf16(v[3]);
+      if constexpr (O16) { if (ok) *reinterpret_cast<bf16x4*>(reinterpret_cast<__bf16*>(a.dy) + r * 128 + part * 16 + q * 4) = p; }
+      else { if (ok) *reinterpret_cast<float4*>(a.dy + r * 128 + part * 16 + q * 4) = make_float4(v[0], v[1], v[2], v[3]); }
       *reinterpret_cast<bf16x4*>(&sdy[row][part * 16 + q * 4]) = p;
       if (pg) {
 #pragma unroll
@@ -366,7 +372,7 @@
       float v = 0.f;
       if (row < a.R) {
         v = acc[r] * act_grad_c<decltype(AT)::value>(a.act, uu[r]);
-        a.du[row * 128 + n] = v;
+        if constexpr (!O16) a.du[row * 128 + n] = v;
       }
       sdu[m][n] = to_bf16(v);
       csum += v;
@@ -379,6 +385,13 @@
   }
   __syncthreads();
   BPHASE(pb, 3);
+  if constexpr (O16) {
+#pragma unroll
+    for (int h = 0; h < 2; ++h) {
+      const int c = tid + 256 * h, m = c >> 4, ch = c & 15;
+      if (r0 + m < a.R) *reinterpret_cast<bf16x8*>(reinterpret_cast<__bf16*>(a.du) + (r0 + m) * 128 + ch * 8) = *reinterpret_cast<const bf16x8*>(&sdu[m][ch * 8]);
+    }
+  }
   if (pg && tid < 128) {
     acc_add(&a.dgamma[tid], spg[0][tid].get());
     acc_add(&a.dbeta[tid], spg[1][tid].get());
@@ -414,6 +427,7 @@
   for (int j = ty; j < 32; j += 8) dst[(n0 + j) * 128 + k0 + tx] = to_bf16(t[tx][j]);
 }
 
+template <bool I16>
 __global__ __launch_bounds__(256) void daxis_param_grads_kernel(const float* __restrict__ y, const float* __restrict__ mean,
                                                                 const float* __restrict__ rstd, const float* __restrict__ dz,
                                                                 const float* __restrict__ dy, const float* __restrict__ du,
@@ -431,8 +445,16 @@
     const float mu = mean[rc], rs = rstd[rc] * m;
     const float4 g = *reinterpret_cast<const float4*>(dz + rc * 128 + cq * 4);
     const float4 yv = *reinterpret_cast<const float4*>(y + rc * 128 + cq * 4);
-    const float4 v = *reinterpret_cast<const float4*>(dy + rc * 128 + cq * 4);
-    const float4 u = *reinterpret_cast<const float4*>(du + rc * 128 + cq * 4);
+    float4 v, u;
+    if constexpr (I16) {
+      const bf16x4 vb = *reinterpret_cast<const bf16x4*>(reinterpret_cast<const __bf16*>(dy) + rc * 128 + cq * 4);
+      const bf16x4 ub = *reinterpret_cast<const bf16x4*>(reinterpret_cast<const __bf16*>(du) + rc * 128 + cq * 4);
+      v = make_float4((float)vb[0], (float)vb[1], (float)vb[2], (float)vb[3]);
+      u = make_float4((float)ub[0], (float)ub[1], (float)ub[2], (float)ub[3]);
+    } else {
+      v = *reinterpret_cast<const float4*>(dy + rc * 128 + cq * 4);
+      u = *reinterpret_cast<const float4*>(du + rc * 128 + cq * 4);
+    }
     a0.x += g.x * (yv.x - mu) * rs; a0.y += g.y * (yv.y - mu) * rs; a0.z += g.z * (yv.z - mu) * rs; a0.w += g.w * (yv.w - mu) * rs;
     a1.x += g.x * m; a1.y += g.y * m; a1.z += g.z * m; a1.w += g.w * m;
     a2.x += v.x * m; a2.y += v.y * m; a2.z += v.z * m; a2.w += v.w * m;
@@ -455,9 +477,11 @@
 }
 
 int daxis_param_grads(hipStream_t s, const float* y, const float* mean, const float* rstd, const float* dz, const float* dy,
-                      const float* du, float* dgamma, float* dbeta, float* db2, float* db1, long R) {
+                      const float* du, float* dgamma, float* dbeta, float* db2, float* db1, long R, bool in16) {
   if (R <= 0) return MIMRL_OK;
-  hipLaunchKernelGGL(daxis_param_grads_kernel, dim3((unsigned)((R + 63) / 64)), dim3(256), 0, s, y, mean, rstd, dz, dy, du, dgamma, dbeta,
+  if (in16) hipLaunchKernelGGL(daxis_param_grads_kernel<true>, dim3((unsigned)((R + 63) / 64)), dim3(256), 0, s, y, mean, rstd, dz, dy, du, dgamma, dbeta,
+                               db2, db1, R);
+  else hipLaunchKernelGGL(daxis_param_grads_kernel<false>, dim3((unsigned)((R + 63) / 64)), dim3(256), 0, s, y, mean, rstd, dz, dy, du, dgamma, dbeta,
                      db2, db1, R);
   LAUNCH_CHECK();
   return MIMRL_OK;
@@ -469,7 +493,8 @@
   if (!a.w2t || !a.w1t || !a.wrt) return set_error(MIMRL_ERR_ARG, "daxis_bwd_fused: needs the transposed weight images");
   if ((a.dgamma || a.dbeta || a.db2 || a.db1) && !(a.dgamma && a.dbeta && a.db2 && a.db1))
     return set_error(MIMRL_ERR_ARG, "daxis_bwd_fused: the four parameter-gradient outputs come together");
-  hipLaunchKernelGGL(daxis_bwd_kernel, dim3((unsigned)((a.R + DR - 1) / DR)), dim3(256), 0, s, a);
+  if (a.out16) hipLaunchKernelGGL(daxis_bwd_kernel<true>, dim3((unsigned)((a.R + DR - 1) / DR)), dim3(256), 0, s, a);
+  else hipLaunchKernelGGL(daxis_bwd_kernel<false>, dim3((unsigned)((a.R + DR - 1) / DR)), dim3(256), 0, s, a);
   LAUNCH_CHECK();
   return MIMRL_OK;
 }
diff --git a/mimrl_amd/csrc/cube_fused.h b/mimrl_amd/csrc/cube_fused.h
--- a/mimrl_amd/csrc/cube_fused.h
+++ b/mimrl_amd/csrc/cube_fused.h
@@ -28,6 +28,7 @@
   int B, il, hl, ol, K, act, save;
   int dbg_phase;
   int pre_on, head_on;
+  int save16;
   CubePre pre; CubeHead head;
 };
 
diff --git a/mimrl_amd/csrc/cube_fused.hip b/mimrl_amd/csrc/cube_fused.hip
--- a/mimrl_amd/csrc/cube_fused.hip
+++ b/mimrl_amd/csrc/cube_fused.hip
@@ -108,8 +108,9 @@
   return c;
 }
 
-template <bool SAVE, int NMT, int G, bool PRE, bool HEAD>
+template <bool SAVE, int NMT, int G, bool PRE, bool HEAD, bool S16 = false>
 __device__ __forceinline__ void cube_fwd_fused_body(const CubeFusedArgs& a) {
+  static_assert(SAVE || !S16, "S16 is a format of the saved activations");
   static_assert(!(PRE || HEAD) || G == 2, "PRE / HEAD: 8 waves (12 time-phase streams on 8 waves; head_fwd_kernel's 512-thread shape)");
   static_assert(!HEAD || NMT == 1, "HEAD: every row of the block output in the one LDS tile");
   extern __shared__ __attribute__((aligned(16))) char smem[];
@@ -298,7 +299,8 @@
               h = act_apply_c<decltype(AT)::value>(a.act, u);
               if (SAVE) {
                 a.l_u[((long)b * hl + m) * C + n0 + n] = u;
-                a.l_h[((long)b * hl + m) * C + n0 + n] = h;
+                if constexpr (S16) reinterpret_cast<bf*>(a.l_h)[((long)b * hl + m) * C + n0 + n] = to_f16(h);
+                else a.l_h[((long)b * hl + m) * C + n0 + n] = h;
               }
             }
             p[q] = to_f16(h);
@@ -392,7 +394,7 @@
         for (int o = 0; o < NK; ++o) {
           const bf ob = to_f16(out[o]);
           Xm[l * XP + o * D + d] = ob;
-          if (SAVE) a.k_z[(((long)b * ol + l) * NK + o) * D + d] = (float)ob;
+          if (SAVE && !S16) a.k_z[(((long)b * ol + l) * NK + o) * D + d] = (float)ob;
         }
       }
       });
@@ -420,6 +422,7 @@
     if (r < R) {
       const int l = r / K, kk = r - l * K;
       v = *reinterpret_cast<const f16x8*>(Xm + l * XP + kk * D + ch * 8);
+      if constexpr (S16) *reinterpret_cast<f16x8*>(reinterpret_cast<bf*>(a.k_z) + ((long)b * ol * K + r) * D + ch * 8) = v;
     }
     *reinterpret_cast<f16x8*>(Az + ((r >> 6) * 2 + (ch >> 3)) * IMG + (r & 63) * ILD + (ch & 7) * 8) = v;
   }
@@ -476,7 +479,7 @@
           h = act_apply_c<decltype(AT)::value>(a.act, u);
           if (SAVE) {
             a.d_u[((long)b * R + row) * D + col] = u;
-            a.d_h[((long)b * R + row) * D + col] = h;
+            if constexpr (!S16) a.d_h[((long)b * R + row) * D + col] = h;
           }
         }
         Ah[(mt * 2 + nt) * IMG + m * ILD + n] = to_f16(h);
@@ -486,6 +489,14 @@
   });
   __syncthreads();
   CPHASE(5);
+  if constexpr (S16) {
+    for (int c = tid; c < NMT * 64 * 16; c += NT) {
+      const int r = c >> 4, ch = c & 15;
+      if (r < R)
+        *reinterpret_cast<f16x8*>(reinterpret_cast<bf*>(a.d_h) + ((long)b * R + r) * D + ch * 8) =
+            *reinterpret_cast<const f16x8*>(Ah + ((r >> 6) * 2 + (ch >> 3)) * IMG + (r & 63) * ILD + (ch & 7) * 8);
+    }
+  }
   if (a.dbg_phase == 4) return;
 #pragma unroll
   for (int i = NI1; i < 3 * NI1; ++i) {
@@ -561,6 +572,8 @@
 __global__ __launch_bounds__(256 * G) void cube_fwd_fused_kernel(CubeFusedArgs a) { cube_fwd_fused_body<SAVE, NMT, G, false, false>(a); }
 template <bool SAVE, int NMT, bool PRE, bool HEAD>
 __global__ __launch_bounds__(512) void cube_fwd_bookends_kernel(CubeFusedArgs a) { cube_fwd_fused_body<SAVE, NMT, 2, PRE, HEAD>(a); }
+template <int NMT, bool PRE, bool HEAD>
+__global__ __launch_bounds__(512) void cube_fwd_save16_kernel(CubeFusedArgs a) { cube_fwd_fused_body<true, NMT, 2, PRE, HEAD, true>(a); }
 
 }
 
@@ -609,6 +622,17 @@
     else if (nmt == 2) LAUNCH_KERN((cube_fwd_bookends_kernel<SAVE, 2, true, false>), 2);                           \
     else LAUNCH_KERN((cube_fwd_bookends_kernel<SAVE, 3, true, false>), 2);                                         \
   } while (0)
+#define LAUNCH_MODE16()                                                                                            \
+  do {                                                                                                             \
+    if (a.head_on && a.pre_on) LAUNCH_KERN((cube_fwd_save16_kernel<1, true, true>), 2);                            \
+    else if (a.head_on) LAUNCH_KERN((cube_fwd_save16_kernel<1, false, true>), 2);                                  \
+    else if (a.pre_on && nmt == 1) LAUNCH_KERN((cube_fwd_save16_kernel<1, true, false>), 2);                       \
+    else if (a.pre_on && nmt == 2) LAUNCH_KERN((cube_fwd_save16_kernel<2, true, false>), 2);                       \
+    else if (a.pre_on) LAUNCH_KERN((cube_fwd_save16_kernel<3, true, false>), 2);                                   \
+    else if (nmt == 1) LAUNCH_KERN((cube_fwd_save16_kernel<1, false, false>), 2);                                  \
+    else if (nmt == 2) LAUNCH_KERN((cube_fwd_save16_kernel<2, false, false>), 2);                                  \
+    else LAUNCH_KERN((cube_fwd_save16_kernel<3, false, false>), 2);                                                \
+  } while (0)
 #define LAUNCH_MODE(SAVE)                                                                                          \
   do {                                                                                                             \
     if (G == 1) LAUNCH_PLAIN(SAVE, 1);                                                                             \
@@ -617,7 +641,10 @@
     else if (a.pre_on) LAUNCH_PRE(SAVE);                                                                           \
     else LAUNCH_PLAIN(SAVE, 2);                                                                                    \
   } while (0)
-  if (a.save) LAUNCH_MODE(true); else LAUNCH_MODE(false);
+  if (a.save16 && !(a.save && G == 2)) return set_error(MIMRL_ERR_ARG, "cube_fused: 16-bit saves are a format of the two-group saving forward");
+  if (a.save16) LAUNCH_MODE16();
+  else if (a.save) LAUNCH_MODE(true); else LAUNCH_MODE(false);
+#undef LAUNCH_MODE16
 #undef LAUNCH_MODE
 #undef LAUNCH_PRE
 #undef LAUNCH_PLAIN
diff --git a/mimrl_amd/csrc/engine.h b/mimrl_amd/csrc/engine.h
--- a/mimrl_amd/csrc/engine.h
+++ b/mimrl_amd/csrc/engine.h
@@ -418,6 +418,8 @@
   int model_forward(bool train, bool save, int knn_stage = 0, int part = 0);
   int cube_forward(bool train, bool save, const CubePre* pre = nullptr, const CubeHead* head = nullptr);
   bool cube_block_fused(int i, bool train) const;
+  bool cube_block_16bit_saves(int i) const;
+  void daxis_fused_blocks(bool bwd_bf16, bool* d_fused) const;
   int cube_backward(int cur_in, int* cur_out);
   int wt_images(hipStream_t st, bool bwd_bf16, bool launch, bool* d_fused);
   int model_backward();
diff --git a/mimrl_amd/csrc/engine_abi.hip b/mimrl_amd/csrc/engine_abi.hip
--- a/mimrl_amd/csrc/engine_abi.hip
+++ b/mimrl_amd/csrc/engine_abi.hip
@@ -589,6 +589,24 @@
   return gemm_group_splitk(reinterpret_cast<hipStream_t>(stream), d, n, (precision & 1) != 0);
 }
 
+int mimrl_op_gemm_wgrad_group16(void* stream, int n, const void* const* A, const void* const* B, float* const* C, const int32_t* dims,
+                                const int64_t* st, const int32_t* storage, int grouped) {
+  if (n <= 0 || n > 12 || !A || !B || !C || !dims || !st || !storage) return set_error(MIMRL_ERR_ARG, "gemm_wgrad_group16: 1..12 problems");
+  GemmDesc d[12];
+  for (int i = 0; i < n; ++i) {
+    d[i].A = static_cast<const float*>(A[i]); d[i].B = static_cast<const float*>(B[i]); d[i].C = C[i];
+    d[i].M = dims[4 * i]; d[i].N = dims[4 * i + 1]; d[i].K = dims[4 * i + 2]; d[i].batch = dims[4 * i + 3];
+    const int64_t* q = st + 9 * i;
+    d[i].sa_m = q[0]; d[i].sa_k = q[1]; d[i].sa_b = q[2]; d[i].sb_k = q[3]; d[i].sb_n = q[4]; d[i].sb_b = q[5];
+    d[i].sc_m = q[6]; d[i].sc_n = q[7]; d[i].sc_b = q[8];
+    d[i].atomic = 1;
+    d[i].a_bf16 = storage[i] & 1; d[i].b_bf16 = d[i].b_f16cvt = (storage[i] >> 1) & 1;
+  }
+  if (grouped) return gemm_group_splitk(reinterpret_cast<hipStream_t>(stream), d, n, true);
+  for (int i = 0; i < n; ++i) MX(gemm(reinterpret_cast<hipStream_t>(stream), d[i], true));
+  return MIMRL_OK;
+}
+
 int64_t mimrl_op_gru_saved_floats(int B, int T) { return gru_saved_floats(B, T); }
 
 int mimrl_op_gru_forward(void* stream, const float* gx_f, const float* gx_r, const float* whh_f, const float* whh_r,
diff --git a/mimrl_amd/csrc/engine_backward.hip b/mimrl_amd/csrc/engine_backward.hip
--- a/mimrl_amd/csrc/engine_backward.hip
+++ b/mimrl_amd/csrc/engine_backward.hip
@@ -37,14 +37,14 @@
     return colln_param_grads(S(sd), y, mean, rstd, dz, dgam, dbet, nb, n, cols);
   };
   auto W_dpg = [&](int sd, const float* y, const float* mean, const float* rstd, const float* dz, const float* dy, const float* du,
-                   float* dgam, float* dbet, float* db2, float* db1, long rows) -> int {
+                   float* dgam, float* dbet, float* db2, float* db1, long rows, bool in16) -> int {
     if (defer) {
-      Deferred d{6, sd, GemmDesc(), y, rows, 0, 0, 0, dgam};
+      Deferred d{6, sd, GemmDesc(), y, rows, in16 ? 1 : 0, 0, 0, dgam};
       d.p1 = mean; d.p2 = rstd; d.p3 = dz; d.p4 = dy; d.p5 = du; d.dst2 = dbet; d.dst3 = db2; d.dst4 = db1;
       deferred.push_back(d);
       return MIMRL_OK;
     }
-    return daxis_param_grads(S(sd), y, mean, rstd, dz, dy, du, dgam, dbet, db2, db1, rows);
+    return daxis_param_grads(S(sd), y, mean, rstd, dz, dy, du, dgam, dbet, db2, db1, rows, in16);
   };
   auto W_fork = [&](int lo, int hi) -> int { return defer ? MIMRL_OK : fork(lo, hi); };
   bool d_fused[MIMRL_MAX_BLOCKS] = {};
@@ -61,6 +61,9 @@
     const int hl = w.ax[0].hid, ol = w.ax[0].out, hk = w.ax[1].hid, ok = w.ax[1].out, hd = w.ax[2].hid, od = w.ax[2].out;
     const float* xblk = i == 0 ? cube0 : bb[i - 1].d.z;
     const float pl = cfg.dropout_mlp[0], pk = cfg.dropout_mlp[1], pd = cfg.dropout_mlp[2];
+    const bool s16 = cube_block_16bit_saves(i);
+    auto W16 = [&](GemmDesc& g, bool b_f16) { if (s16) { g.a_bf16 = 1; if (b_f16) g.b_bf16 = g.b_f16cvt = 1; } };
+    if (s16 && !(bf16 && d_fused[i])) return set_error(MIMRL_ERR_STATE, "cube_backward: block %d saved 16-bit activations but its fused D-axis backward is off", i);
     if (d_fused[i]) {
       const AxisW& a = w.ax[2];
       const long R2 = (long)B * ol * ok;
@@ -69,15 +72,15 @@
       fa.dz = gbuf[cur]; fa.y = b.d.y; fa.mean = b.d.mean; fa.rstd = b.d.rstd; fa.gamma = P(a.ln_g); fa.u = b.d.u;
       fa.w2t = wtT[i][0]; fa.w1t = wtT[i][1]; fa.wrt = wtT[i][2];
       fa.dy = gbuf[i_dy]; fa.du = gbuf[i_du]; fa.dx = gbuf[i_dx];
-      fa.R = R2; fa.act = cfg.activation;
+      fa.R = R2; fa.act = cfg.activation; fa.out16 = s16 ? 1 : 0;
       fa.dgamma = fa.dbeta = fa.db2 = fa.db1 = nullptr;
       MX(daxis_bwd_fused(stream, fa));
       MX(W_fork(1, 3));
       MX(W_dpg(2, b.d.y, b.d.mean, b.d.rstd, gbuf[cur], gbuf[i_dy], gbuf[i_du], Gm(a.ln_g), Gm(a.ln_b),
-               a.fc2.b >= 0 ? Gm(a.fc2.b) : nullptr, a.fc1.b >= 0 ? Gm(a.fc1.b) : nullptr, R2));
-      { GemmDesc g = gemm_tn(gbuf[i_dy], od, b.d.h, hd, Gm(a.fc2.w), hd, od, hd, (int)R2); g.atomic = 1; MX(W_gemm(1, g)); }
-      { GemmDesc g = gemm_tn(gbuf[i_dy], od, b.k.z, id, Gm(a.res), id, od, id, (int)R2); g.atomic = 1; MX(W_gemm(2, g)); }
-      { GemmDesc g = gemm_tn(gbuf[i_du], hd, b.k.z, id, Gm(a.fc1.w), id, hd, id, (int)R2); g.atomic = 1; MX(W_gemm(3, g)); }
+               a.fc2.b >= 0 ? Gm(a.fc2.b) : nullptr, a.fc1.b >= 0 ? Gm(a.fc1.b) : nullptr, R2, s16));
+      { GemmDesc g = gemm_tn(gbuf[i_dy], od, b.d.h, hd, Gm(a.fc2.w), hd, od, hd, (int)R2); g.atomic = 1; W16(g, true); MX(W_gemm(1, g)); }
+      { GemmDesc g = gemm_tn(gbuf[i_dy], od, b.k.z, id, Gm(a.res), id, od, id, (int)R2); g.atomic = 1; W16(g, true); MX(W_gemm(2, g)); }
+      { GemmDesc g = gemm_tn(gbuf[i_du], hd, b.k.z, id, Gm(a.fc1.w), id, hd, id, (int)R2); g.atomic = 1; W16(g, true); MX(W_gemm(3, g)); }
       MX(W_join(1, 3));
       release(cur); release(i_dy); release(i_du);
       cur = i_dx;
@@ -181,7 +184,7 @@
       fa.w2 = P(a.fc2.w); fa.w1 = P(a.fc1.w); fa.wr = P(a.res);
       fa.dy = gbuf[i_dy]; fa.du = gbuf[i_du]; fa.dx = gbuf[i_dx];
       fa.db2 = a.fc2.b >= 0 ? Gm(a.fc2.b) : nullptr; fa.db1 = a.fc1.b >= 0 ? Gm(a.fc1.b) : nullptr;
-      fa.B = B; fa.il = il; fa.hl = hl; fa.ol = ol; fa.C = (int)C; fa.act = cfg.activation;
+      fa.B = B; fa.il = il; fa.hl = hl; fa.ol = ol; fa.C = (int)C; fa.act = cfg.activation; fa.out16 = s16 ? 1 : 0;
       MX(laxis_bwd_fused(stream, fa));
       MX(W_fork(1, 3));
       MX(W_lnpar(1, b.l.y, b.l.mean, b.l.rstd, gbuf[cur], Gm(a.ln_g), Gm(a.ln_b), B, ol, (int)C));
@@ -189,19 +192,20 @@
       { GemmDesc g; g.A = gbuf[i_dy]; g.sa_m = C; g.sa_k = 1; g.sa_b = (long)ol * C;
         g.B = b.l.h; g.sb_k = 1; g.sb_n = C; g.sb_b = (long)hl * C;
         g.C = Gm(a.fc2.w); g.sc_m = hl; g.sc_n = 1; g.sc_b = 0; g.M = ol; g.N = hl; g.K = (int)C; g.batch = B; g.atomic = 1;
-        MX(W_gemm(1, g)); }
+        W16(g, true); MX(W_gemm(1, g)); }
       { GemmDesc g; g.A = gbuf[i_dy]; g.sa_m = C; g.sa_k = 1; g.sa_b = (long)ol * C;
         g.B = xblk; g.sb_k = 1; g.sb_n = C; g.sb_b = (long)il * C;
         g.C = Gm(a.res); g.sc_m = il; g.sc_n = 1; g.sc_b = 0; g.M = ol; g.N = il; g.K = (int)C; g.batch = B; g.atomic = 1;
-        MX(W_gemm(2, g)); }
+        W16(g, false); MX(W_gemm(2, g)); }
       { GemmDesc g; g.A = gbuf[i_du]; g.sa_m = C; g.sa_k = 1; g.sa_b = (long)hl * C;
         g.B = xblk; g.sb_k = 1; g.sb_n = C; g.sb_b = (long)il * C;
         g.C = Gm(a.fc1.w); g.sc_m = il; g.sc_n = 1; g.sc_b = 0; g.M = hl; g.N = il; g.K = (int)C; g.batch = B; g.atomic = 1;
-        MX(W_gemm(3, g)); }
+        W16(g, false); MX(W_gemm(3, g)); }
       MX(W_join(1, 3));
       release(i_dy); release(i_du);
       cur = i_dx;
     } else {
+      if (s16) return set_error(MIMRL_ERR_STATE, "cube_backward: block %d saved 16-bit activations but its fused L-axis backward is off", i);
       const AxisW& a = w.ax[0];
       const long C = (long)ik * id;
       const float* xmlp = cfg.ln_first ? b.l.xn : xblk;
@@ -308,9 +312,9 @@
   static const int dbg_skip_kinds = dbg_env("MIMRL_DBG_SKIP_DEFERRED") ? atoi(dbg_env("MIMRL_DBG_SKIP_DEFERRED")) : 0;
   const bool groupk = !prof_on && bf16 && !((dbg_skip_kinds >> 0) & 1) && cfg.seq_len <= 128;
   if (groupk) {
-    std::vector<GemmDesc> cls[2];
-    for (const Deferred& d : deferred) if (d.kind == 0) cls[d.g.sa_k == 1 ? 0 : 1].push_back(d.g);
-    for (int c = 0; c < 2; ++c) {
+    std::vector<GemmDesc> cls[4];
+    for (const Deferred& d : deferred) if (d.kind == 0) cls[(d.g.sa_k == 1 ? 0 : 1) + (d.g.a_bf16 ? 2 : 0)].push_back(d.g);
+    for (int c = 0; c < 4; ++c) {
       hipStream_t st = only_side > 0 ? S(only_side) : S(1 + c % wg_sides);
       for (size_t i = 0; i < cls[c].size(); i += 12) MX(gemm_group_splitk(st, cls[c].data() + i, (int)std::min<size_t>(12, cls[c].size() - i), bf16));
     }
@@ -325,7 +329,7 @@
     else if (d.kind == 1) MX(colsum(st, d.src, d.n0, (int)d.n1, (int)d.n2, d.dst));
     else if (d.kind == 2) MX(rowsum_batched(st, d.src, (int)d.n0, (int)d.n1, (int)d.n2, d.dst));
     else if (d.kind == 3) MX(colln_param_grads(st, d.src, d.p1, d.p2, d.p3, d.dst, d.dst2, (int)d.n0, (int)d.n1, (int)d.n2));
-    else if (d.kind == 6) MX(daxis_param_grads(st, d.src, d.p1, d.p2, d.p3, d.p4, d.p5, d.dst, d.dst2, d.dst3, d.dst4, d.n0));
+    else if (d.kind == 6) MX(daxis_param_grads(st, d.src, d.p1, d.p2, d.p3, d.p4, d.p5, d.dst, d.dst2, d.dst3, d.dst4, d.n0, d.n1 != 0));
     else MX(kmix_bwd_part(st, d.src, d.p3, nullptr, d.kw, d.n0, (int)d.n1, 2));
   }
   deferred.clear();
diff --git a/mimrl_amd/csrc/engine_forward.hip b/mimrl_amd/csrc/engine_forward.hip
--- a/mimrl_amd/csrc/engine_forward.hip
+++ b/mimrl_amd/csrc/engine_forward.hip
@@ -274,6 +274,19 @@
   const float pmlp[3] = {train ? cfg.dropout_mlp[0] : 0.f, train ? cfg.dropout_mlp[1] : 0.f, train ? cfg.dropout_mlp[2] : 0.f};
   return cube_fused_supported(il, w.ax[0].hid, w.ax[0].out, ik, w.ax[1].hid, w.ax[1].out, id, w.ax[2].hid, w.ax[2].out, cfg.ln_first != 0,
                               cfg.res_project[i] != 0, cfg.bias != 0, pmlp);
+}
+
+bool mimrl_handle::cube_block_16bit_saves(int i) const {
+  if (i < 0 || i >= cfg.n_blocks || !bf16_fwd() || !bf16_bwd() || !fused_cube || !fused_cube_bwd || cfg.ln_first) return false;
+  int il = cfg.time_len, ik = 3, id = cfg.d_common;
+  for (int j = 0; j < i; ++j) { il = blk[j].ax[0].out; ik = blk[j].ax[1].out; id = blk[j].ax[2].out; }
+  const BlockW& w = blk[i];
+  if (!cube_fused_supported(il, w.ax[0].hid, w.ax[0].out, ik, w.ax[1].hid, w.ax[1].out, id, w.ax[2].hid, w.ax[2].out, false, cfg.res_project[i] != 0,
+                            cfg.bias != 0, cfg.dropout_mlp))
+    return false;
+  bool d_fused[MIMRL_MAX_BLOCKS] = {};
+  daxis_fused_blocks(true, d_fused);
+  return d_fused[i] && w.ax[0].res >= 0 && laxis_bwd_supported(il, w.ax[0].hid, w.ax[0].out, ik * id);
 }
 
 int mimrl_handle::cube_forward(bool train, bool save, const CubePre* pre, const CubeHead* head) {
@@ -310,7 +323,8 @@
       fa.d_z = b.d.z;
       fa.dbg_phase = dbg_env("MIMRL_CUBE_PHASE") ? atoi(dbg_env("MIMRL_CUBE_PHASE")) : 0;
       fa.B = B; fa.il = il; fa.hl = hl; fa.ol = ol; fa.K = ik; fa.act = cfg.activation; fa.save = save ? 1 : 0;
-      if (fa.dbg_phase == 100) { fa.save = 0; fa.dbg_phase = 0; }
+      fa.save16 = save && cube_block_16bit_saves(i) ? 1 : 0;
+      if (fa.dbg_phase == 100) { fa.save = 0; fa.save16 = 0; fa.dbg_phase = 0; }
       if (pre && i == 0) { fa.pre_on = 1; fa.pre = *pre; }
       if (head && i == cfg.n_blocks - 1) { fa.head_on = 1; fa.head = *head; }
       MX(cube_block_fwd_fused(stream, fa));
@@ -419,15 +433,23 @@
   return MIMRL_OK;
 }
 
+void mimrl_handle::daxis_fused_blocks(bool bwd_bf16, bool* d_fused) const {
+  int din2 = cfg.d_common, n = 0;
+  for (int i = 0; i < cfg.n_blocks; ++i) {
+    const AxisW& a = blk[i].ax[2];
+    d_fused[i] = bwd_bf16 && fused_cube_bwd && !cfg.ln_first && cfg.dropout_mlp[2] <= 0.f && a.res >= 0 &&
+                 daxis_bwd_supported(din2, a.hid, a.out) && n + 3 <= 12;
+    din2 = cfg.d_outs[i][2];
+    if (d_fused[i]) n += 3;
+  }
+}
+
 int mimrl_handle::wt_images(hipStream_t st, bool bwd_bf16, bool launch, bool* d_fused) {
-  int din2 = cfg.d_common;
+  daxis_fused_blocks(bwd_bf16, d_fused);
   WtTransposeArgs ta;
   ta.n = 0;
   for (int i = 0; i < cfg.n_blocks; ++i) {
     const AxisW& a = blk[i].ax[2];
-    d_fused[i] = bwd_bf16 && fused_cube_bwd && !cfg.ln_first && cfg.dropout_mlp[2] <= 0.f && a.res >= 0 &&
-                 daxis_bwd_supported(din2, a.hid, a.out) && ta.n + 3 <= 12;
-    din2 = cfg.d_outs[i][2];
     if (!d_fused[i]) continue;
     const long srcs[3] = {a.fc2.w, a.fc1.w, a.res};
     for (int q = 0; q < 3; ++q) { ta.src[ta.n] = P(srcs[q]); ta.dst[ta.n] = wtT[i][q]; ++ta.n; }
diff --git a/mimrl_amd/csrc/gemm.hip b/mimrl_amd/csrc/gemm.hip
--- a/mimrl_amd/csrc/gemm.hip
+++ b/mimrl_amd/csrc/gemm.hip
@@ -515,10 +515,9 @@
 }
 
 template <int TM, int TN, bool AKC, bool BKC, bool GEN, bool ABF = false, bool BBF = false, bool F16 = false, bool BH = false>
-__device__ __forceinline__ void fast_body(const GemmDesc& d, int ksplit, int kt_per, int dbg, unsigned bx, unsigned by, unsigned bzr) {
+__device__ __forceinline__ void fast_body_lds(const GemmDesc& d, int ksplit, int kt_per, int dbg, unsigned bx, unsigned by, unsigned bzr,
+                                              __bf16 (&sA)[2][FT<TM>::ELEMS], __bf16 (&sB)[2][FT<TN>::ELEMS]) {
   constexpr int BMf = 64 * TM, BNf = 64 * TN;
-  __shared__ __attribute__((aligned(16))) __bf16 sA[2][FT<TM>::ELEMS];
-  __shared__ __attribute__((aligned(16))) __bf16 sB[2][FT<TN>::ELEMS];
   const int tid = threadIdx.x, lane = tid & 63, wave = tid >> 6;
   const int wm = wave >> 1, wn = wave & 1;
   const int bz = bzr / ksplit, ks = bzr - bz * ksplit;
@@ -631,6 +630,13 @@
       epilogue<GEN>(d, d.atomic || ksplit > 1, bz, oc, bn_pre[j], acc[i][j], m0 + wm * 32 * TM + i * 32, n0 + wn * 32 * TN + j * 32 + (lane & 31), lane);
 }
 
+template <int TM, int TN, bool AKC, bool BKC, bool GEN, bool ABF = false, bool BBF = false, bool F16 = false, bool BH = false>
+__device__ __forceinline__ void fast_body(const GemmDesc& d, int ksplit, int kt_per, int dbg, unsigned bx, unsigned by, unsigned bzr) {
+  __shared__ __attribute__((aligned(16))) __bf16 sA[2][FT<TM>::ELEMS];
+  __shared__ __attribute__((aligned(16))) __bf16 sB[2][FT<TN>::ELEMS];
+  fast_body_lds<TM, TN, AKC, BKC, GEN, ABF, BBF, F16, BH>(d, ksplit, kt_per, dbg, bx, by, bzr, sA, sB);
+}
+
 template <int TM, int TN, bool AKC, bool BKC, bool GEN>
 __global__ __launch_bounds__(256) void gemm_fast_kernel(KernelArgs ka) {
   unsigned bx, by, bzr;
@@ -656,11 +662,11 @@
   fast_body<TM, TN, AKC, BKC, false, true, BBF>(ka.d, ka.ksplit, ka.kt_per, ka.dbg, bx, by, bzr);
 }
 
-template <int TM, int TN>
+template <int TM, int TN, bool KC = false>
 __global__ __launch_bounds__(256) void gemm_fast_bfh_kernel(KernelArgs ka) {
   unsigned bx, by, bzr;
   tile_ids(ka.xcd_remap, bx, by, bzr);
-  fast_body<TM, TN, false, false, false, true, true, false, true>(ka.d, ka.ksplit, ka.kt_per, ka.dbg, bx, by, bzr);
+  fast_body<TM, TN, KC, KC, false, true, true, false, true>(ka.d, ka.ksplit, ka.kt_per, ka.dbg, bx, by, bzr);
 }
 
 struct GroupArgs {
@@ -686,13 +692,14 @@
   int M, N, K, batch;
   long sa, sa_b, sb, sb_b, sc_m, sc_b;
   int nsplit, kt_per;
+  int b_f16;
 };
 struct GroupKArgs {
   GroupKProb p[GEMM_GROUPK_MAX];
   int start[GEMM_GROUPK_MAX];
   int n;
 };
-template <bool AKC, bool BKC>
+template <bool AKC, bool BKC, bool S16 = false>
 __global__ __launch_bounds__(256) void gemm_groupk_kernel(GroupKArgs ga) {
   int p = 0;
 #pragma unroll
@@ -706,7 +713,19 @@
   d.sc_m = g.sc_m; d.sc_n = 1; d.sc_b = g.sc_b; d.atomic = 1;
   const unsigned t = blockIdx.x - ga.start[p];
   const unsigned nx = (g.N + 63) / 64, ny = (g.M + 63) / 64;
-  fast_body<1, 1, AKC, BKC, false>(d, g.nsplit, g.kt_per, 0, t % nx, (t / nx) % ny, t / (nx * ny));
+  if constexpr (S16) {
+    __shared__ __attribute__((aligned(16))) __bf16 sA[2][FT<1>::ELEMS];
+    __shared__ __attribute__((aligned(16))) __bf16 sB[2][FT<1>::ELEMS];
+    d.a_bf16 = 1;
+    if (g.b_f16) {
+      d.b_bf16 = d.b_f16cvt = 1;
+      fast_body_lds<1, 1, AKC, BKC, false, true, true, false, true>(d, g.nsplit, g.kt_per, 0, t % nx, (t / nx) % ny, t / (nx * ny), sA, sB);
+    } else {
+      fast_body_lds<1, 1, AKC, BKC, false, true, false>(d, g.nsplit, g.kt_per, 0, t % nx, (t / nx) % ny, t / (nx * ny), sA, sB);
+    }
+  } else {
+    fast_body<1, 1, AKC, BKC, false>(d, g.nsplit, g.kt_per, 0, t % nx, (t / nx) % ny, t / (nx * ny));
+  }
 }
 
 inline int fast_class(const float* P, long s_r, long s_k, long s_b, long s_bo, int R, int K, int bf = 0, int pad4 = 0) {
@@ -738,10 +757,12 @@
   if (d.A2 && (fast_class(d.A2, d.sa2_m, d.sa2_k, d.sa2_b, 0, d.M, d.K2, d.a_bf16) != ca || fast_class(d.B2, d.sb2_n, d.sb2_k, d.sb2_b, 0, d.N, d.K2, d.b_bf16) != cb))
     return false;
   if (d.a_bf16 || d.b_bf16) {
-    if (!d.a_bf16 || (ca == 1 && cb == 1 && !(d.f16 && d.b_bf16)) || d.bias_m || d.beta != 0.f || d.pre || d.gradact_u) return false;
+    const bool kk16 = ca == 1 && cb == 1 && d.a_bf16 && !d.f16 && (d.b_bf16 != 0) == (d.b_f16cvt != 0) && plain_accumulate(d) && d.M <= 64 && d.N <= 64 &&
+                      !d.a_gap_rows;
+    if (!d.a_bf16 || (ca == 1 && cb == 1 && !(d.f16 && d.b_bf16) && !kk16) || d.bias_m || d.beta != 0.f || d.pre || d.gradact_u) return false;
     if (d.f16 && !(ca == 1 && cb == 1 && d.b_bf16)) return false;
     if (d.a_gap_rows && (d.a_gap_at % 8 != 0 || d.a_gap_rows % 8 != 0)) return false;
-    if (d.b_f16cvt && !(ca == 2 && cb == 2 && d.b_bf16 && !d.A2)) return false;
+    if (d.b_f16cvt && !(((ca == 2 && cb == 2) || kk16) && d.b_bf16 && !d.A2)) return false;
   }
   const int ktiles = (d.K + FBK - 1) / FBK;
   const bool acc = plain_accumulate(d) && ktiles >= 32;
@@ -827,15 +848,18 @@
 int gemm_group_splitk(hipStream_t s, const GemmDesc* ds, int n, bool bf16) {
   bool ok = bf16 && n >= 2 && n <= GEMM_GROUPK_MAX;
   int ca = 0, cb = 0;
+  bool s16 = false;
   long tiles = 0;
   double macs = 0;
   for (int i = 0; ok && i < n; ++i) {
     const GemmDesc& d = ds[i];
     if (d.M <= 0 || d.N <= 0 || d.batch <= 0 || !d.A || !d.B || !d.C) { ok = false; break; }
-    const int a = fast_class(d.A, d.sa_m, d.sa_k, d.sa_b, d.sa_bo, d.M, d.K), b = fast_class(d.B, d.sb_n, d.sb_k, d.sb_b, d.sb_bo, d.N, d.K);
+    const int a = fast_class(d.A, d.sa_m, d.sa_k, d.sa_b, d.sa_bo, d.M, d.K, d.a_bf16), b = fast_class(d.B, d.sb_n, d.sb_k, d.sb_b, d.sb_bo, d.N, d.K, d.b_bf16);
     if (!a || !b || a != b || (i > 0 && a != ca)) { ok = false; break; }
     ca = a; cb = b;
-    if (!plain_accumulate(d) || d.alpha != 1.f || d.sc_n != 1 || d.batch_in > 0 || d.a_gap_rows || d.a_bf16 || d.b_bf16) { ok = false; break; }
+    if (!plain_accumulate(d) || d.alpha != 1.f || d.sc_n != 1 || d.batch_in > 0 || d.a_gap_rows || d.f16) { ok = false; break; }
+    if ((i > 0 && (d.a_bf16 != 0) != s16) || (d.b_bf16 != 0) != (d.b_f16cvt != 0) || (d.b_bf16 && !d.a_bf16)) { ok = false; break; }
+    s16 = d.a_bf16 != 0;
     tiles += (long)((d.M + 63) / 64) * ((d.N + 63) / 64) * d.batch;
     macs += (double)d.M * d.N * d.K * d.batch;
   }
@@ -855,7 +879,7 @@
     GroupKProb& g = ga.p[i];
     g.A = d.A; g.B = d.B; g.C = d.C; g.M = d.M; g.N = d.N; g.K = d.K; g.batch = d.batch;
     g.sa = ca == 1 ? d.sa_m : d.sa_k; g.sa_b = d.sa_b; g.sb = ca == 1 ? d.sb_n : d.sb_k; g.sb_b = d.sb_b;
-    g.sc_m = d.sc_m; g.sc_b = d.sc_b;
+    g.sc_m = d.sc_m; g.sc_b = d.sc_b; g.b_f16 = d.b_f16cvt;
     const int ktiles = (d.K + FBK - 1) / FBK;
     long ks = want < 1 ? 1 : want;
     if (ks > ktiles / 8) ks = ktiles / 8;
@@ -866,7 +890,9 @@
     acc += (long)((d.M + 63) / 64) * ((d.N + 63) / 64) * d.batch * g.nsplit;
   }
   if (acc > 0x7fffffffL) return set_error(MIMRL_ERR_ARG, "gemm_group_splitk: grid too large");
-  if (ca == 1) hipLaunchKernelGGL((gemm_groupk_kernel<true, true>), dim3((unsigned)acc), dim3(256), 0, s, ga);
+  if (s16 && ca == 1) hipLaunchKernelGGL((gemm_groupk_kernel<true, true, true>), dim3((unsigned)acc), dim3(256), 0, s, ga);
+  else if (s16) hipLaunchKernelGGL((gemm_groupk_kernel<false, false, true>), dim3((unsigned)acc), dim3(256), 0, s, ga);
+  else if (ca == 1) hipLaunchKernelGGL((gemm_groupk_kernel<true, true>), dim3((unsigned)acc), dim3(256), 0, s, ga);
   else hipLaunchKernelGGL((gemm_groupk_kernel<false, false>), dim3((unsigned)acc), dim3(256), 0, s, ga);
   LAUNCH_CHECK();
   return MIMRL_OK;
@@ -943,7 +969,13 @@
     case 14: FASTK(2, 1, true, true);
     case 15: FASTB(2, 1, true, false);
     case 16: FASTB(2, 1, false, false);
-    case 18: FASTK(1, 1, true, true);
+    case 18:
+      if (d.a_bf16 && !d.f16) {
+        if (d.b_f16cvt) hipLaunchKernelGGL((gemm_fast_bfh_kernel<1, 1, true>), grid, dim3(256), 0, s, ka);
+        else hipLaunchKernelGGL((gemm_fast_bf_kernel<1, 1, true, true, false>), grid, dim3(256), 0, s, ka);
+        break;
+      }
+      FASTK(1, 1, true, true);
     case 19: FASTB(1, 1, true, false);
     case 20: FASTB(1, 1, false, false);
     case 0: GENK(false, 32, false);
```

Result: faster. 1247, median of 6 (+1.1%).
